# SenseTime-FVG/OpenDWM

Hardware: AMD Instinct MI355X
Metric: denoise-steps/sec (6-view x16f 448x256), SD-3.5 CTSD (higher is better)
Workload: dtype bf16; 1 GPU; CTSD SD-3.5 MMDiT (24 joint blocks, 13 dual, 6 cross-view + 12 temporal VT blocks, point-wise temporal + ImageAdapter), 6 views x 16 frames x 448x256 px (latents [1,16,6,16,32,56]), CFG g=4 -> model batch 2, 154 text tokens, FlowMatch-Euler; one replica per GPU; layers=24, finite=True, residual_stream=fp32 (GEMM operands and activations bf16), variant=text+layout (ImageAdapter recomputed every step, pointwise temporal)

## Files before the change

include/dwm_hip.h:

```cpp
#ifndef DWM_HIP_H
#define DWM_HIP_H

#include <stdint.h>

#ifdef __cplusplus
extern "C" {
#endif

#define DWM_OK 0
#define DWM_EINVAL (-1)
#define DWM_EALIGN (-2)
#define DWM_EUNSUPPORTED (-3)

#define DWM_ABI_VERSION 18
int dwm_abi_version(void);
const char* dwm_source_hash(void);

enum {
    DWM_EPI_PLAIN = 0,
    DWM_EPI_GEGLU = 1,
    DWM_EPI_RESID = 2,
    DWM_EPI_RMSHEAD = 3
};
enum { DWM_ACT_NONE = 0, DWM_ACT_GELU_TANH = 1, DWM_ACT_SILU = 2, DWM_ACT_RELU = 3 };

typedef struct dwm_rowmap2d {
    int64_t rw, rh;
    int64_t rpitch, ipitch;
    int64_t origin;
    int64_t xstep;
} dwm_rowmap2d;

typedef struct dwm_gemm_args {
    const void* A;  int64_t lda;
    const void* W;
    const void* bias;
    void* C;        int64_t ldc;
    int64_t M, N, K;
    int32_t epilogue;
    int32_t act;
    const void* gate; int64_t ld_gate; int64_t rows_per_gate;
    const void* res;  int64_t ld_res;  int64_t res_mod;
    const void* blend; int64_t ld_blend;
    const float* alpha; int64_t rows_per_alpha;
    const void* rms_w; int64_t rms_ncols; float rms_eps;
    int32_t reserved;
    dwm_rowmap2d a_map;
    dwm_rowmap2d c_map;
    int32_t ntaps; int32_t k_per_tap;
    int64_t tap_shift[27];
    void* workspace; int64_t workspace_bytes; int32_t split_k;
    void* C32; int64_t ldc32;
    int32_t tile;
} dwm_gemm_args;

int dwm_gemm_bf16(const dwm_gemm_args* args, void* stream);
int64_t dwm_gemm4w_launches(void);
int64_t dwm_gemm4w_launches_general(void);

typedef struct dwm_gemm_tn_args {
    const void* A; int64_t lda;
    const void* B; int64_t ldb; int64_t b_rows;
    void* out; int64_t ldo;
    int64_t M, N, C;
    int32_t ntaps; int32_t split_k;
    int64_t tap_shift[27];
    void* workspace; int64_t workspace_bytes;
} dwm_gemm_tn_args;
int dwm_gemm_tn(const dwm_gemm_tn_args* args, void* stream);

typedef struct dwm_attn_args {
    const void *q0, *k0, *v0; int64_t ld0;
    const void *q1, *k1, *v1; int64_t ld1;
    void* o0; int64_t ldo0;
    void* o1; int64_t ldo1;
    int64_t L0, L1;
    int64_t n_problems;
    int32_t heads; int32_t head_dim;
    float scale;
    int32_t mask_mode;
    int64_t pdiv[3], pmod[3], pstride[3];
    int64_t ldiv[2], lstride[3];
    const uint8_t* mask; int64_t mask_G; int64_t group_size; int64_t p_per_mask;
    int32_t variant;
    int32_t cross;
    float* lse;
} dwm_attn_args;

int dwm_attention_fwd(const dwm_attn_args* args, void* stream);
int64_t dwm_attn_stream_launches(void);

typedef struct dwm_attn_bwd_args {
    dwm_attn_args fwd;
    const void *do0, *do1;
    void *dq0, *dk0, *dv0; int64_t ld_d0;
    void *dq1, *dk1, *dv1; int64_t ld_d1;
    float* delta;
} dwm_attn_bwd_args;
int dwm_attention_bwd(const dwm_attn_bwd_args* args, void* stream);

int dwm_debug_tr_probe(const int32_t* offs, int16_t* out, void* stream);

typedef struct dwm_layernorm_args {
    const void* x; int64_t ldx;
    void* y;       int64_t ldy;
    void* y2;      int64_t ldy2;
    void* xsum;    int64_t ldxsum;
    int64_t rows; int32_t D; float eps;
    const void* weight; const void* bias;
    const void* scale;  const void* shift;  int64_t ld_mod;  int64_t rows_per_mod;
    const void* scale2; const void* shift2;
    const void* addvec; int64_t ld_add; int64_t rows_per_add;
} dwm_layernorm_args;

int dwm_layernorm(const dwm_layernorm_args* args, void* stream);
int dwm_layernorm_x32(const dwm_layernorm_args* args, void* stream);

int dwm_rmsnorm_heads(void* x, int64_t ldx, int64_t rows, int64_t ncols,
                      const void* w, float eps, void* stream);

int dwm_silu(const void* x, void* y, int64_t n, void* stream);

int dwm_timestep_sinusoid(const float* t, int64_t n, int32_t C, void* out, void* stream);

int dwm_patchify(const void* x, int32_t x_is_f32, int64_t I, int32_t C, int32_t H, int32_t W,
                 int32_t p, void* out, int64_t ldo, void* stream);

int dwm_unpatchify(const void* x, int64_t ldx, int64_t I, int32_t C, int32_t h, int32_t w,
                   int32_t p, void* out, void* stream);

int dwm_cfg_euler_step(const void* pred, float* latents, void* model_in, int64_t n,
                       float guidance, float dsigma, void* stream);

int dwm_cfg_euler_step_grouped(const void* pred, float* latents, void* model_in, int64_t n, float guidance,
                               const float* dsigma, int64_t group_elems, void* stream);

int dwm_unshuffle_tokens(const void* x, int32_t x_is_f32, int64_t I, int32_t C, int32_t H, int32_t W,
                         int32_t r, void* out, int64_t ldo, void* stream);

int dwm_avgpool2_tokens(const void* x, int64_t I, int32_t h, int32_t w, int32_t C, void* out, void* stream);

int dwm_add_inplace(void* y, const void* x, int64_t n, void* stream);
int dwm_add_f32_inplace(void* y, const float* x, int64_t n, void* stream);
int dwm_add_f32_f32_inplace(float* y, const float* x, int64_t n, void* stream);

int dwm_groupnorm_silu(const void* x, void* y, int64_t I, int64_t P, int32_t C, int32_t G, float eps,
                       const void* gamma, const void* beta, int32_t silu, float* stats,
                       const dwm_rowmap2d* out_map, void* stream);

typedef struct dwm_gn_imgmap { int64_t iv, pn, s_ihi, s_ilo, s_phi; } dwm_gn_imgmap;
int64_t dwm_groupnorm_stats_floats(int64_t I, int64_t P, int32_t G);
int dwm_groupnorm_silu_mapped(const void* x, void* y, int64_t I, int64_t P, int32_t C, int32_t G, float eps,
                              const void* gamma, const void* beta, int32_t silu, float* stats,
                              const dwm_rowmap2d* out_map, const dwm_gn_imgmap* img_map, void* stream);

typedef struct dwm_gn_zmap {
    const void* mod; int64_t ld_mod;
    int32_t frames, videos, h, w, shift;
    int32_t zt[32];
} dwm_gn_zmap;
int dwm_groupnorm_spatial(const void* x, void* y, int64_t I, int64_t P, int32_t C, int32_t G, float eps,
                          const void* gamma, const void* beta, int32_t silu, float* stats,
                          const dwm_rowmap2d* out_map, const dwm_gn_imgmap* img_map, const dwm_gn_zmap* zmap, void* stream);
int dwm_groupnorm_spatial_f32(const float* x, float* y, int64_t I, int64_t P, int32_t C, int32_t G, float eps,
                              const float* gamma, const float* beta, int32_t silu, float* stats,
                              const dwm_rowmap2d* out_map, const dwm_gn_imgmap* img_map, const dwm_gn_zmap* zmap, void* stream);

typedef struct dwm_frame_mix { int32_t n_out; int32_t f0[64], f1[64]; float w0[64], w1[64]; } dwm_frame_mix;
int dwm_frame_mix_bf16(const void* x, void* y, int64_t frame_elems, const dwm_frame_mix* mix, void* stream);
int dwm_frame_mix_f32(const float* x, float* y, int64_t frame_elems, const dwm_frame_mix* mix, void* stream);

int dwm_upsample2_padded(const void* x, void* y, int64_t I, int32_t h, int32_t w, int32_t C, void* stream);

int dwm_pad_tokens(const void* x, void* y, int64_t rows, int32_t C, const dwm_rowmap2d* map, void* stream);

int dwm_softmax_rows(const void* x, void* y, int64_t rows, int32_t L, int64_t ld, float scale, void* stream);

typedef struct dwm_vae_attn_args {
    const void* q; const void* k; const void* v; void* out;
    int64_t ldq, ldk, ldv, ldo;
    int64_t I, P;
    int32_t C; float scale;
} dwm_vae_attn_args;
int dwm_vae_attention(const dwm_vae_attn_args* args, void* stream);
int dwm_vae_attention_f32(const dwm_vae_attn_args* args, void* stream);

int dwm_ray_features(const float* cam, int64_t I, int32_t h, int32_t w, void* out, int64_t ldo, void* stream);
int dwm_ray_features_f32(const float* cam, int64_t I, int32_t h, int32_t w, float* out, int64_t ldo, void* stream);

int dwm_frame_affine(const float* x, const float* y, const float* coef, float* out, void* out_bf16, int64_t n,
                     int64_t group_elems, void* stream);

int dwm_cfg_ddim_step(const void* pred, int32_t pred_is_f32, int32_t cfg, float* latents, void* model_in, float* x0_out,
                      const float* noise, const float* coef, int64_t n, int64_t group_elems, float guidance,
                      int32_t prediction_type, float clip_range, int32_t use_clipped_model_output, void* stream);

int dwm_cfg_ddim_step_masked(const void* pred, int32_t pred_is_f32, int32_t cfg, float* latents, void* model_in, float* x0_out,
                             const float* noise, const float* coef, int64_t n, int64_t group_elems, float guidance,
                             int32_t prediction_type, float clip_range, int32_t use_clipped_model_output, const int32_t* skip,
                             void* stream);

int dwm_cfg_multistep(const void* pred, float* latents, float* x0_prev, void* model_in, int64_t n, float guidance,
                      float kx, float ko, float A, float B, float C, void* stream);

int dwm_cfg_multistep_grouped(const void* pred, float* latents, float* x0_prev, void* model_in, int64_t n, float guidance,
                              const float* coef, int64_t coef_rows, const int32_t* keep_model_in, int64_t group_elems, void* stream);
int dwm_cfg_multistep_grouped_f32(const float* pred, float* latents, float* x0_prev, float* model_in, int64_t n, float guidance,
                                  const float* coef, int64_t coef_rows, const int32_t* keep_model_in, int64_t group_elems,
                                  void* stream);

int dwm_cast_f32_to_bf16(const float* src, void* dst, int64_t n, void* stream);

int dwm_transpose_bf16(const void* in, int64_t ld_in, int64_t rows, int64_t cols,
                       void* out, int64_t ld_out, int64_t rows_pad, void* stream);

int dwm_segsum(const void* a, int64_t lda, const void* b, int64_t ldb, int64_t rows, int64_t ncols,
               int64_t rows_per_group, float* out, int64_t ld_out, void* stream);
int dwm_segsum_diff(const void* a, int64_t lda, const void* b, int64_t ldb, const void* b2, int64_t ldb2, int64_t rows,
                    int64_t ncols, int64_t rows_per_group, float* out, int64_t ld_out, void* stream);

int dwm_act_fwd(const void* x, void* y, int64_t n, int32_t act, void* stream);
int dwm_act_bwd(const void* x, const void* dy, void* dx, int64_t n, int32_t act, void* stream);
int dwm_act_bwd_recompute(const void* x, const void* dy, void* y_out, void* dx, int64_t n, int32_t act, void* stream);

int dwm_geglu_fwd(const void* u, int64_t ldu, int64_t rows, int64_t inner, void* g, int64_t ldg, void* stream);
int dwm_geglu_bwd(const void* u, int64_t ldu, const void* dg, int64_t lddg, int64_t rows, int64_t inner,
                  void* du, int64_t lddu, void* stream);
int dwm_geglu_bwd_recompute(const void* u, int64_t ldu, const void* dg, int64_t lddg, int64_t rows, int64_t inner,
                            void* g_out, int64_t ldg, void* du, int64_t lddu, void* stream);

typedef struct dwm_rowcombine_args {
    const void* a; int64_t lda;
    const void* gate_a; int64_t ld_gate_a; int64_t rows_per_gate_a;
    const float* coef_a; int64_t rows_per_coef_a;
    const void* b; int64_t ldb;
    const float* coef_b; int64_t rows_per_coef_b;
    void* out; int64_t ldo;
    int64_t rows; int64_t ncols;
} dwm_rowcombine_args;
int dwm_rowcombine(const dwm_rowcombine_args* args, void* stream);

typedef struct dwm_layernorm_bwd_args {
    const void* x; int64_t ldx;
    const void* addvec; int64_t ld_add; int64_t rows_per_add;
    const void* dy; int64_t lddy;
    const void* dy2; int64_t lddy2;
    void* dx; int64_t lddx; int32_t accumulate;
    int64_t rows; int32_t D; float eps;
    const void* weight;
    const void* scale; const void* scale2; int64_t ld_mod; int64_t rows_per_mod;
    float* dgamma; float* dbeta; float* dgamma2; float* dbeta2; int64_t ld_grad; int32_t grad_per_group;
} dwm_layernorm_bwd_args;
int dwm_layernorm_bwd(const dwm_layernorm_bwd_args* args, void* stream);

int dwm_rmsnorm_heads_train(void* x, int64_t ldx, int64_t rows, int64_t ncols, const void* w, float eps,
                            float* rinv, void* stream);
int dwm_rmsnorm_heads_bwd(const void* y, int64_t ldy, const float* rinv, const void* w, void* dy, int64_t lddy,
                          int64_t rows, int64_t ncols, float* dw, void* stream);

int dwm_adamw(float* p, const float* g, float* m, float* v, void* p_bf16, int64_t n, float lr, float beta1,
              float beta2, float eps, float weight_decay, float bias_corr1, float bias_corr2, float grad_scale,
              void* stream);

typedef struct dwm_adamw_item {
    float* p; const float* g; float* m; float* v; void* p_bf16; int64_t n;
} dwm_adamw_item;
int dwm_adamw_multi(const dwm_adamw_item* items, const int32_t* block_item, const int64_t* block_start, int64_t n_blocks,
                    int64_t chunk, float lr, float beta1, float beta2, float eps, float weight_decay, float bias_corr1,
                    float bias_corr2, float grad_scale, void* stream);

int dwm_quantize_blockwise8(const float* x, int64_t n, const float* code, int32_t floor_positive, uint8_t* q, float* absmax,
                            void* stream);
int dwm_dequantize_blockwise8(const uint8_t* q, const float* absmax, int64_t n, const float* code, float* x, void* stream);

typedef struct dwm_adamw8_item {
    float* p; const float* g; uint8_t* m_q; float* m_absmax; uint8_t* v_q; float* v_absmax; void* p_bf16; int64_t n;
} dwm_adamw8_item;
int dwm_adamw8_multi(const dwm_adamw8_item* items, const int32_t* block_item, const int64_t* block_start, int64_t n_blocks,
                     int64_t chunk, const float* code_m, const float* code_v, float lr, float beta1, float beta2, float eps,
                     float weight_decay, float bias_corr1, float bias_corr2, float grad_scale, void* stream);

typedef struct dwm_grad_item { float* g; int64_t n; } dwm_grad_item;
int dwm_grad_sumsq_multi(const dwm_grad_item* items, const int32_t* block_item, const int64_t* block_start, int64_t n_blocks,
                         int64_t chunk, float pre_scale, float max_norm, double* partials, uint32_t* flags, float* out,
                         void* stream);
int dwm_grad_scale_multi(const dwm_grad_item* items, const int32_t* block_item, const int64_t* block_start, int64_t n_blocks,
                         int64_t chunk, float coef, void* stream);

int dwm_groupnorm_bwd(const void* x, const void* dz, void* dx, int64_t I, int64_t P, int32_t C, int32_t G, float eps,
                      const void* gamma, const void* beta, int32_t silu, int32_t accumulate, float* stats,
                      float* dgamma, float* dbeta, const dwm_rowmap2d* dz_map, const dwm_gn_imgmap* img_map, void* stream);

int64_t dwm_segsum_ordered_floats(int64_t rows, int64_t ncols, int64_t rows_per_group);
int64_t dwm_segsum_diff_ordered_floats(int64_t rows, int64_t ncols, int64_t rows_per_group);
int64_t dwm_layernorm_bwd_ordered_floats(const dwm_layernorm_bwd_args* args);
int64_t dwm_rmsnorm_heads_bwd_ordered_floats(int64_t rows, int64_t ncols);
int64_t dwm_groupnorm_bwd_ordered_floats(int64_t I, int64_t P, int32_t C);
int dwm_segsum_ordered(const void* a, int64_t lda, const void* b, int64_t ldb, int64_t rows, int64_t ncols,
                       int64_t rows_per_group, float* out, int64_t ld_out, float* workspace, int64_t workspace_floats, void* stream);
int dwm_segsum_diff_ordered(const void* a, int64_t lda, const void* b, int64_t ldb, const void* b2, int64_t ldb2, int64_t rows,
                            int64_t ncols, int64_t rows_per_group, float* out, int64_t ld_out, float* workspace,
                            int64_t workspace_floats, void* stream);
int dwm_layernorm_bwd_ordered(const dwm_layernorm_bwd_args* args, float* workspace, int64_t workspace_floats, void* stream);
int dwm_rmsnorm_heads_bwd_ordered(const void* y, int64_t ldy, const float* rinv, const void* w, void* dy, int64_t lddy,
                                  int64_t rows, int64_t ncols, float* dw, float* workspace, int64_t workspace_floats, void* stream);
int dwm_groupnorm_bwd_ordered(const void* x, const void* dz, void* dx, int64_t I, int64_t P, int32_t C, int32_t G, float eps,
                              const void* gamma, const void* beta, int32_t silu, int32_t accumulate, float* stats,
                              float* dgamma, float* dbeta, const dwm_rowmap2d* dz_map, const dwm_gn_imgmap* img_map,
                              float* workspace, int64_t workspace_floats, void* stream);

typedef struct dwm_block_permute_args {
    const void* src;
    void* dst;
    int64_t block_bytes;
    int64_t n[4];
    int64_t sstride[4];
} dwm_block_permute_args;
int dwm_block_permute(const dwm_block_permute_args* args, void* stream);

int dwm_head_exchange(const void* src, void* dst, int64_t rows, int32_t S, int32_t R, int64_t Dr, int32_t elem_size, int64_t ld,
                      int32_t dir, void* stream);

typedef struct dwm_fifo_item {
    void* buf; const void* fresh; int64_t outer; int64_t T; int64_t inner_bytes; int64_t fresh_outer; int64_t convert; int64_t n;
} dwm_fifo_item;
int dwm_fifo_slide_multi(const dwm_fifo_item* host_items, int64_t n_items, const dwm_fifo_item* items, const int32_t* block_item,
                         const int64_t* block_start, int64_t n_blocks, int64_t chunk, void* stream);

int dwm_cast_bf16_to_f32(const void* x, int64_t ldx, float* y, int64_t ldy, int64_t rows, int64_t cols,
                         int32_t accumulate, void* stream);

int dwm_gemm_f32(const dwm_gemm_args* args, void* stream);
int dwm_groupnorm_silu_f32(const float* x, float* y, int64_t I, int64_t P, int32_t C, int32_t G, float eps,
                           const float* gamma, const float* beta, int32_t silu, float* stats,
                           const dwm_rowmap2d* out_map, const dwm_gn_imgmap* img_map, void* stream);
int dwm_upsample2_padded_f32(const float* x, float* y, int64_t I, int32_t h, int32_t w, int32_t C, void* stream);
int dwm_pad_tokens_f32(const float* x, float* y, int64_t rows, int32_t C, const dwm_rowmap2d* map, void* stream);
int dwm_softmax_rows_f32(const float* x, float* y, int64_t rows, int32_t L, int64_t ld, float scale, void* stream);
int dwm_unshuffle_tokens_f32(const float* x, int64_t I, int32_t C, int32_t H, int32_t W, int32_t r, float* out, int64_t ldo,
                             void* stream);
int dwm_avgpool2_tokens_f32(const float* x, int64_t I, int32_t h, int32_t w, int32_t C, float* out, void* stream);
int dwm_cfg_multistep_f32(const float* pred, float* latents, float* x0_prev, float* model_in, int64_t n, float guidance,
                          float kx, float ko, float A, float B, float C, void* stream);
int dwm_layernorm_f32(const dwm_layernorm_args* args, void* stream);
int dwm_attention_f32(const dwm_attn_args* args, void* stream);
int dwm_silu_f32(const float* x, float* y, int64_t n, void* stream);
int dwm_timestep_sinusoid_f32(const float* t, int64_t n, int32_t C, float* out, void* stream);
int dwm_patchify_f32(const float* x, int64_t I, int32_t C, int32_t H, int32_t W, int32_t p, float* out, int64_t ldo, void* stream);
int dwm_unpatchify_f32(const float* x, int64_t ldx, int64_t I, int32_t C, int32_t h, int32_t w, int32_t p, float* out, void* stream);
int dwm_cfg_euler_step_f32(const float* pred, float* latents, float* model_in, int64_t n, float guidance, float dsigma,
                           const float* dsigma_group, int64_t group_elems, void* stream);

typedef struct dwm_text_attn_args {
    const void* q; const void* k; const void* v; int64_t ld;
    void* out; int64_t ldo;
    int64_t n_seq, L;
// ... 18 lines not shown
```

opendwm_amd/_lib.py:

```python
from __future__ import annotations

import ctypes as C
import os

HERE = os.path.dirname(os.path.abspath(__file__))
LIB_PATH = os.environ.get("DWM_HIP_LIB") or os.path.join(HERE, "libdwm_hip.so")
ABI_VERSION = 18

EPI_PLAIN, EPI_GEGLU, EPI_RESID, EPI_RMSHEAD = 0, 1, 2, 3
ACT_NONE, ACT_GELU_TANH, ACT_SILU, ACT_RELU = 0, 1, 2, 3

_i64, _i32, _f32, _vp = C.c_int64, C.c_int32, C.c_float, C.c_void_p


class RowMap2D(C.Structure):
    _fields_ = [("rw", _i64), ("rh", _i64), ("rpitch", _i64), ("ipitch", _i64), ("origin", _i64), ("xstep", _i64)]


class GemmTnArgs(C.Structure):
    _fields_ = [
        ("A", _vp), ("lda", _i64), ("B", _vp), ("ldb", _i64), ("b_rows", _i64), ("out", _vp), ("ldo", _i64),
        ("M", _i64), ("N", _i64), ("C", _i64), ("ntaps", _i32), ("split_k", _i32), ("tap_shift", _i64 * 27),
        ("workspace", _vp), ("workspace_bytes", _i64),
    ]


class GemmArgs(C.Structure):
    _fields_ = [
        ("A", _vp), ("lda", _i64), ("W", _vp), ("bias", _vp), ("C", _vp), ("ldc", _i64),
        ("M", _i64), ("N", _i64), ("K", _i64), ("epilogue", _i32), ("act", _i32),
        ("gate", _vp), ("ld_gate", _i64), ("rows_per_gate", _i64),
        ("res", _vp), ("ld_res", _i64), ("res_mod", _i64),
        ("blend", _vp), ("ld_blend", _i64), ("alpha", _vp), ("rows_per_alpha", _i64),
        ("rms_w", _vp), ("rms_ncols", _i64), ("rms_eps", _f32), ("reserved", _i32),
        ("a_map", RowMap2D), ("c_map", RowMap2D), ("ntaps", _i32), ("k_per_tap", _i32),
        ("tap_shift", _i64 * 27),
        ("workspace", _vp), ("workspace_bytes", _i64), ("split_k", _i32),
        ("C32", _vp), ("ldc32", _i64),
        ("tile", _i32),
    ]


class AttnArgs(C.Structure):
    _fields_ = [
        ("q0", _vp), ("k0", _vp), ("v0", _vp), ("ld0", _i64),
        ("q1", _vp), ("k1", _vp), ("v1", _vp), ("ld1", _i64),
        ("o0", _vp), ("ldo0", _i64), ("o1", _vp), ("ldo1", _i64),
        ("L0", _i64), ("L1", _i64), ("n_problems", _i64),
        ("heads", _i32), ("head_dim", _i32), ("scale", _f32), ("mask_mode", _i32),
        ("pdiv", _i64 * 3), ("pmod", _i64 * 3), ("pstride", _i64 * 3),
        ("ldiv", _i64 * 2), ("lstride", _i64 * 3),
        ("mask", _vp), ("mask_G", _i64), ("group_size", _i64), ("p_per_mask", _i64),
        ("variant", _i32), ("cross", _i32), ("lse", _vp),
    ]


class AttnBwdArgs(C.Structure):
    _fields_ = [
        ("fwd", AttnArgs), ("do0", _vp), ("do1", _vp),
        ("dq0", _vp), ("dk0", _vp), ("dv0", _vp), ("ld_d0", _i64),
        ("dq1", _vp), ("dk1", _vp), ("dv1", _vp), ("ld_d1", _i64), ("delta", _vp),
    ]


class LayerNormArgs(C.Structure):
    _fields_ = [
        ("x", _vp), ("ldx", _i64), ("y", _vp), ("ldy", _i64), ("y2", _vp), ("ldy2", _i64),
        ("xsum", _vp), ("ldxsum", _i64), ("rows", _i64), ("D", _i32), ("eps", _f32),
        ("weight", _vp), ("bias", _vp),
        ("scale", _vp), ("shift", _vp), ("ld_mod", _i64), ("rows_per_mod", _i64),
        ("scale2", _vp), ("shift2", _vp),
        ("addvec", _vp), ("ld_add", _i64), ("rows_per_add", _i64),
    ]


class GnImgMap(C.Structure):
    _fields_ = [("iv", _i64), ("pn", _i64), ("s_ihi", _i64), ("s_ilo", _i64), ("s_phi", _i64)]


class GnZMap(C.Structure):
    _fields_ = [("mod", _vp), ("ld_mod", _i64), ("frames", _i32), ("videos", _i32), ("h", _i32), ("w", _i32),
                ("shift", _i32), ("zt", _i32 * 32)]


class FrameMix(C.Structure):
    _fields_ = [("n_out", _i32), ("f0", _i32 * 64), ("f1", _i32 * 64), ("w0", _f32 * 64), ("w1", _f32 * 64)]


class BlockPermuteArgs(C.Structure):
    _fields_ = [("src", C.c_void_p), ("dst", C.c_void_p), ("block_bytes", C.c_int64), ("n", C.c_int64 * 4), ("sstride", C.c_int64 * 4)]


class RowCombineArgs(C.Structure):
    _fields_ = [
        ("a", _vp), ("lda", _i64), ("gate_a", _vp), ("ld_gate_a", _i64), ("rows_per_gate_a", _i64),
        ("coef_a", _vp), ("rows_per_coef_a", _i64), ("b", _vp), ("ldb", _i64),
        ("coef_b", _vp), ("rows_per_coef_b", _i64), ("out", _vp), ("ldo", _i64), ("rows", _i64), ("ncols", _i64),
    ]


class LayerNormBwdArgs(C.Structure):
    _fields_ = [
        ("x", _vp), ("ldx", _i64), ("addvec", _vp), ("ld_add", _i64), ("rows_per_add", _i64),
        ("dy", _vp), ("lddy", _i64), ("dy2", _vp), ("lddy2", _i64),
        ("dx", _vp), ("lddx", _i64), ("accumulate", _i32),
        ("rows", _i64), ("D", _i32), ("eps", _f32), ("weight", _vp),
        ("scale", _vp), ("scale2", _vp), ("ld_mod", _i64), ("rows_per_mod", _i64),
        ("dgamma", _vp), ("dbeta", _vp), ("dgamma2", _vp), ("dbeta2", _vp), ("ld_grad", _i64), ("grad_per_group", _i32),
    ]


class AdamW8Item(C.Structure):
    _fields_ = [("p", _vp), ("g", _vp), ("m_q", _vp), ("m_absmax", _vp), ("v_q", _vp), ("v_absmax", _vp), ("p_bf16", _vp), ("n", _i64)]


class FifoItem(C.Structure):
    _fields_ = [("buf", _vp), ("fresh", _vp), ("outer", _i64), ("T", _i64), ("inner_bytes", _i64), ("fresh_outer", _i64),
                ("convert", _i64), ("n", _i64)]


class VaeAttnArgs(C.Structure):
    _fields_ = [("q", _vp), ("k", _vp), ("v", _vp), ("out", _vp), ("ldq", _i64), ("ldk", _i64), ("ldv", _i64), ("ldo", _i64),
                ("I", _i64), ("P", _i64), ("C", _i32), ("scale", _f32)]


class TextAttnArgs(C.Structure):
    _fields_ = [("q", _vp), ("k", _vp), ("v", _vp), ("ld", _i64), ("out", _vp), ("ldo", _i64), ("n_seq", _i64), ("L", _i64),
                ("heads", _i32), ("scale", _f32), ("causal", _i32), ("bias", _vp)]


SIGNATURES = {
    "dwm_abi_version": (_i32, []),
    "dwm_source_hash": (C.c_char_p, []),
    "dwm_gemm_bf16": (_i32, [C.POINTER(GemmArgs), _vp]),
    "dwm_gemm4w_launches": (_i64, []),
    "dwm_gemm4w_launches_general": (_i64, []),
    "dwm_attn_stream_launches": (_i64, []),
    "dwm_gemm_tn": (_i32, [C.POINTER(GemmTnArgs), _vp]),
    "dwm_attention_fwd": (_i32, [C.POINTER(AttnArgs), _vp]),
    "dwm_attention_bwd": (_i32, [C.POINTER(AttnBwdArgs), _vp]),
    "dwm_debug_tr_probe": (_i32, [_vp, _vp, _vp]),
    "dwm_layernorm": (_i32, [C.POINTER(LayerNormArgs), _vp]),
    "dwm_layernorm_x32": (_i32, [C.POINTER(LayerNormArgs), _vp]),
    "dwm_rmsnorm_heads": (_i32, [_vp, _i64, _i64, _i64, _vp, _f32, _vp]),
    "dwm_silu": (_i32, [_vp, _vp, _i64, _vp]),
    "dwm_timestep_sinusoid": (_i32, [_vp, _i64, _i32, _vp, _vp]),
    "dwm_patchify": (_i32, [_vp, _i32, _i64, _i32, _i32, _i32, _i32, _vp, _i64, _vp]),
    "dwm_unpatchify": (_i32, [_vp, _i64, _i64, _i32, _i32, _i32, _i32, _vp, _vp]),
    "dwm_cfg_euler_step": (_i32, [_vp, _vp, _vp, _i64, _f32, _f32, _vp]),
    "dwm_cfg_euler_step_grouped": (_i32, [_vp, _vp, _vp, _i64, _f32, _vp, _i64, _vp]),
    "dwm_cast_f32_to_bf16": (_i32, [_vp, _vp, _i64, _vp]),
    "dwm_gemm_f32": (_i32, [C.POINTER(GemmArgs), _vp]),
    "dwm_layernorm_f32": (_i32, [C.POINTER(LayerNormArgs), _vp]),
    "dwm_groupnorm_silu_f32": (_i32, [_vp, _vp, _i64, _i64, _i32, _i32, _f32, _vp, _vp, _i32, _vp, C.POINTER(RowMap2D), C.POINTER(GnImgMap), _vp]),
    "dwm_upsample2_padded_f32": (_i32, [_vp, _vp, _i64, _i32, _i32, _i32, _vp]),
    "dwm_pad_tokens_f32": (_i32, [_vp, _vp, _i64, _i32, C.POINTER(RowMap2D), _vp]),
    "dwm_softmax_rows_f32": (_i32, [_vp, _vp, _i64, _i32, _i64, _f32, _vp]),
    "dwm_unshuffle_tokens_f32": (_i32, [_vp, _i64, _i32, _i32, _i32, _i32, _vp, _i64, _vp]),
    "dwm_avgpool2_tokens_f32": (_i32, [_vp, _i64, _i32, _i32, _i32, _vp, _vp]),
    "dwm_cfg_multistep_f32": (_i32, [_vp, _vp, _vp, _vp, _i64, _f32, _f32, _f32, _f32, _f32, _f32, _vp]),
    "dwm_attention_f32": (_i32, [C.POINTER(AttnArgs), _vp]),
    "dwm_silu_f32": (_i32, [_vp, _vp, _i64, _vp]),
    "dwm_timestep_sinusoid_f32": (_i32, [_vp, _i64, _i32, _vp, _vp]),
    "dwm_patchify_f32": (_i32, [_vp, _i64, _i32, _i32, _i32, _i32, _vp, _i64, _vp]),
    "dwm_unpatchify_f32": (_i32, [_vp, _i64, _i64, _i32, _i32, _i32, _i32, _vp, _vp]),
    "dwm_cfg_euler_step_f32": (_i32, [_vp, _vp, _vp, _i64, _f32, _f32, _vp, _i64, _vp]),
    "dwm_ray_features": (_i32, [_vp, _i64, _i32, _i32, _vp, _i64, _vp]),
    "dwm_ray_features_f32": (_i32, [_vp, _i64, _i32, _i32, _vp, _i64, _vp]),
    "dwm_frame_affine": (_i32, [_vp, _vp, _vp, _vp, _vp, _i64, _i64, _vp]),
    "dwm_cfg_ddim_step": (_i32, [_vp, _i32, _i32, _vp, _vp, _vp, _vp, _vp, _i64, _i64, _f32, _i32, _f32, _i32, _vp]),
    "dwm_cfg_multistep": (_i32, [_vp, _vp, _vp, _vp, _i64, _f32, _f32, _f32, _f32, _f32, _f32, _vp]),
    "dwm_cfg_ddim_step_masked": (_i32, [_vp, _i32, _i32, _vp, _vp, _vp, _vp, _vp, _i64, _i64, _f32, _i32, _f32, _i32, _vp, _vp]),
    "dwm_cfg_multistep_grouped": (_i32, [_vp, _vp, _vp, _vp, _i64, _f32, _vp, _i64, _vp, _i64, _vp]),
    "dwm_cfg_multistep_grouped_f32": (_i32, [_vp, _vp, _vp, _vp, _i64, _f32, _vp, _i64, _vp, _i64, _vp]),
    "dwm_unshuffle_tokens": (_i32, [_vp, _i32, _i64, _i32, _i32, _i32, _i32, _vp, _i64, _vp]),
    "dwm_avgpool2_tokens": (_i32, [_vp, _i64, _i32, _i32, _i32, _vp, _vp]),
    "dwm_add_inplace": (_i32, [_vp, _vp, _i64, _vp]),
    "dwm_add_f32_inplace": (_i32, [_vp, _vp, _i64, _vp]),
    "dwm_add_f32_f32_inplace": (_i32, [_vp, _vp, _i64, _vp]),
    "dwm_groupnorm_silu": (_i32, [_vp, _vp, _i64, _i64, _i32, _i32, _f32, _vp, _vp, _i32, _vp, C.POINTER(RowMap2D), _vp]),
    "dwm_groupnorm_silu_mapped": (_i32, [_vp, _vp, _i64, _i64, _i32, _i32, _f32, _vp, _vp, _i32, _vp, C.POINTER(RowMap2D), C.POINTER(GnImgMap), _vp]),
    "dwm_upsample2_padded": (_i32, [_vp, _vp, _i64, _i32, _i32, _i32, _vp]),
    "dwm_pad_tokens": (_i32, [_vp, _vp, _i64, _i32, C.POINTER(RowMap2D), _vp]),
    "dwm_groupnorm_stats_floats": (_i64, [_i64, _i64, _i32]),
    "dwm_groupnorm_spatial": (_i32, [_vp, _vp, _i64, _i64, _i32, _i32, _f32, _vp, _vp, _i32, _vp, C.POINTER(RowMap2D),
                                     C.POINTER(GnImgMap), C.POINTER(GnZMap), _vp]),
    "dwm_frame_mix_bf16": (_i32, [_vp, _vp, _i64, C.POINTER(FrameMix), _vp]),
    "dwm_frame_mix_f32": (_i32, [_vp, _vp, _i64, C.POINTER(FrameMix), _vp]),
    "dwm_groupnorm_spatial_f32": (_i32, [_vp, _vp, _i64, _i64, _i32, _i32, _f32, _vp, _vp, _i32, _vp, C.POINTER(RowMap2D),
                                         C.POINTER(GnImgMap), C.POINTER(GnZMap), _vp]),
    "dwm_softmax_rows": (_i32, [_vp, _vp, _i64, _i32, _i64, _f32, _vp]),
    "dwm_vae_attention": (_i32, [C.POINTER(VaeAttnArgs), _vp]),
    "dwm_vae_attention_f32": (_i32, [C.POINTER(VaeAttnArgs), _vp]),
    "dwm_transpose_bf16": (_i32, [_vp, _i64, _i64, _i64, _vp, _i64, _i64, _vp]),
    "dwm_segsum": (_i32, [_vp, _i64, _vp, _i64, _i64, _i64, _i64, _vp, _i64, _vp]),
    "dwm_segsum_diff": (_i32, [_vp, _i64, _vp, _i64, _vp, _i64, _i64, _i64, _i64, _vp, _i64, _vp]),
    "dwm_act_fwd": (_i32, [_vp, _vp, _i64, _i32, _vp]),
    "dwm_act_bwd": (_i32, [_vp, _vp, _vp, _i64, _i32, _vp]),
    "dwm_geglu_fwd": (_i32, [_vp, _i64, _i64, _i64, _vp, _i64, _vp]),
    "dwm_geglu_bwd": (_i32, [_vp, _i64, _vp, _i64, _i64, _i64, _vp, _i64, _vp]),
    "dwm_act_bwd_recompute": (_i32, [_vp, _vp, _vp, _vp, _i64, _i32, _vp]),
    "dwm_geglu_bwd_recompute": (_i32, [_vp, _i64, _vp, _i64, _i64, _i64, _vp, _i64, _vp, _i64, _vp]),
    "dwm_rowcombine": (_i32, [C.POINTER(RowCombineArgs), _vp]),
    "dwm_layernorm_bwd": (_i32, [C.POINTER(LayerNormBwdArgs), _vp]),
    "dwm_rmsnorm_heads_train": (_i32, [_vp, _i64, _i64, _i64, _vp, _f32, _vp, _vp]),
    "dwm_rmsnorm_heads_bwd": (_i32, [_vp, _i64, _vp, _vp, _vp, _i64, _i64, _i64, _vp, _vp]),
    "dwm_adamw": (_i32, [_vp, _vp, _vp, _vp, _vp, _i64, _f32, _f32, _f32, _f32, _f32, _f32, _f32, _f32, _vp]),
    "dwm_adamw_multi": (_i32, [_vp, _vp, _vp, _i64, _i64, _f32, _f32, _f32, _f32, _f32, _f32, _f32, _f32, _vp]),
    "dwm_quantize_blockwise8": (_i32, [_vp, _i64, _vp, _i32, _vp, _vp, _vp]),
    "dwm_dequantize_blockwise8": (_i32, [_vp, _vp, _i64, _vp, _vp, _vp]),
    "dwm_adamw8_multi": (_i32, [_vp, _vp, _vp, _i64, _i64, _vp, _vp, _f32, _f32, _f32, _f32, _f32, _f32, _f32, _f32, _vp]),
    "dwm_grad_sumsq_multi": (_i32, [_vp, _vp, _vp, _i64, _i64, _f32, _f32, _vp, _vp, _vp, _vp]),
    "dwm_grad_scale_multi": (_i32, [_vp, _vp, _vp, _i64, _i64, _f32, _vp]),
    "dwm_block_permute": (_i32, [C.POINTER(BlockPermuteArgs), _vp]),
    "dwm_head_exchange": (_i32, [_vp, _vp, _i64, _i32, _i32, _i64, _i32, _i64, _i32, _vp]),
    "dwm_fifo_slide_multi": (_i32, [C.POINTER(FifoItem), _i64, _vp, _vp, _vp, _i64, _i64, _vp]),
    "dwm_cast_bf16_to_f32": (_i32, [_vp, _i64, _vp, _i64, _i64, _i64, _i32, _vp]),
    "dwm_groupnorm_bwd": (_i32, [_vp, _vp, _vp, _i64, _i64, _i32, _i32, _f32, _vp, _vp, _i32, _i32, _vp, _vp, _vp,
                                 C.POINTER(RowMap2D), C.POINTER(GnImgMap), _vp]),
    "dwm_segsum_ordered": (_i32, [_vp, _i64, _vp, _i64, _i64, _i64, _i64, _vp, _i64, _vp, _i64, _vp]),
    "dwm_segsum_diff_ordered": (_i32, [_vp, _i64, _vp, _i64, _vp, _i64, _i64, _i64, _i64, _vp, _i64, _vp, _i64, _vp]),
    "dwm_layernorm_bwd_ordered": (_i32, [C.POINTER(LayerNormBwdArgs), _vp, _i64, _vp]),
    "dwm_rmsnorm_heads_bwd_ordered": (_i32, [_vp, _i64, _vp, _vp, _vp, _i64, _i64, _i64, _vp, _vp, _i64, _vp]),
    "dwm_groupnorm_bwd_ordered": (_i32, [_vp, _vp, _vp, _i64, _i64, _i32, _i32, _f32, _vp, _vp, _i32, _i32, _vp, _vp, _vp,
                                         C.POINTER(RowMap2D), C.POINTER(GnImgMap), _vp, _i64, _vp]),
    "dwm_segsum_ordered_floats": (_i64, [_i64, _i64, _i64]),
    "dwm_segsum_diff_ordered_floats": (_i64, [_i64, _i64, _i64]),
    "dwm_layernorm_bwd_ordered_floats": (_i64, [C.POINTER(LayerNormBwdArgs)]),
    "dwm_rmsnorm_heads_bwd_ordered_floats": (_i64, [_i64, _i64]),
    "dwm_groupnorm_bwd_ordered_floats": (_i64, [_i64, _i64, _i32]),
    "dwm_text_attention": (_i32, [C.POINTER(TextAttnArgs), _vp]),
    "dwm_rmsnorm_rows": (_i32, [_vp, _i64, _i64, _i64, _vp, _f32, _vp, _i64, _vp]),
    "dwm_text_embed": (_i32, [_vp, _i64, _vp, _i64, _i64, _vp, _i64, _vp, _i64, _vp]),
    "dwm_text_act": (_i32, [_vp, _i64, _i64, _i64, _i32, _i32, _vp, _i64, _vp]),
}

_ERR = {-1: "DWM_EINVAL (bad shape / null pointer)", -2: "DWM_EALIGN (alignment)",
        -3: "DWM_EUNSUPPORTED (shape not supported by the kernel)"}

_lib = None


def load():
    global _lib
    if _lib is not None:
        return _lib
    import torch
    if torch.cuda.is_available():
        torch.cuda.init()
    if not os.path.exists(LIB_PATH):
        raise RuntimeError(
            f"{LIB_PATH} is missing: build it with `python -m opendwm_amd.build` "
            "(there is no CPU / PyTorch fallback for the HIP path)")
    lib = C.CDLL(LIB_PATH)
    for name, (res, args) in SIGNATURES.items():
        fn = getattr(lib, name)
        fn.restype = res
        fn.argtypes = args
    v = lib.dwm_abi_version()
    if v != ABI_VERSION:
        raise RuntimeError(f"libdwm_hip.so ABI {v} != binding ABI {ABI_VERSION}; rebuild")
    if os.environ.get("DWM_SKIP_SOURCE_HASH") != "1":
        from .build import source_hash
        try:
            want = source_hash()
        except OSError:
            want = None
        have = (lib.dwm_source_hash() or b"").decode()
        if want is not None and have != want:
            msg = (f"{LIB_PATH} was built from other sources (hash {have[:12]}..., tree {want[:12]}...): "
                   "run `python -m opendwm_amd.build`")
            if os.environ.get("DWM_HIP_LIB"):
                import warnings
                warnings.warn(msg)
            else:
                raise RuntimeError(msg)
    _lib = lib
    return lib


def check(rc: int, what: str) -> None:
    if rc != 0:
        msg = _ERR.get(rc, f"hipError_t {rc}" if rc > 0 else f"error {rc}")
        raise RuntimeError(f"{what} failed: {msg}")
```

opendwm_amd/blocks.py:

```python
from __future__ import annotations

from typing import Optional

import torch
from torch import nn

from . import ops
from .ops import ACT_GELU_TANH, ACT_SILU, EPI_GEGLU, EPI_RESID, EPI_RMSHEAD

bf16 = torch.bfloat16


class ParamStore:

    def __init__(self):
        self.step = 0
        self._shadow = {}
        self._derived = {}
        self.precision = bf16

    def set_precision(self, dtype: torch.dtype) -> None:
        if dtype not in (bf16, torch.float32):
            raise ValueError("compute dtype must be torch.bfloat16 or torch.float32")
        self.precision = dtype

    def cached(self, owner, make):
        slot = getattr(owner, "_pk", None)
        if not isinstance(slot, dict) or "_by_precision" not in slot:
            slot = {"_by_precision": {}}
            owner._pk = slot
        hit = slot["_by_precision"].get(self.precision)
        if hit is None or hit[0] != self.step:
            hit = (self.step, make())
            slot["_by_precision"][self.precision] = hit
        return hit[1]

    def bf(self, t: torch.Tensor) -> torch.Tensor:
        if self.precision == torch.float32:
            d = t.detach()
            if d.dtype == torch.float32:
                return d if d.is_contiguous() else d.contiguous()
            key = (t.data_ptr(), t._version, tuple(t.shape), "f32")
            hit = self._shadow.get(id(t))
            if hit is None or hit[0] != key:
                hit = (key, d.float().contiguous())
                self._shadow[id(t)] = hit
            return hit[1]
        if t.dtype == bf16:
            d = t.detach()
            return d if d.is_contiguous() else d.contiguous()
        key = (t.data_ptr(), t._version, tuple(t.shape))
        hit = self._shadow.get(id(t))
        if hit is None or hit[0] != key:
            d = t.detach()
            if d.is_cuda and d.dtype == torch.float32 and d.is_contiguous() and d.numel() % 4 == 0:
                sh = ops.cast_bf16(d)
            else:
                sh = d.to(bf16).contiguous()
            hit = (key, sh)
            self._shadow[id(t)] = hit
        return hit[1]

    def derived(self, t: torch.Tensor, tag: str, make):
        k = (id(t), tag, self.precision)
        hit = self._derived.get(k)
        if hit is None or hit[0] != (self.step, t.data_ptr(), t._version):
            hit = ((self.step, t.data_ptr(), t._version), make())
            self._derived[k] = hit
        return hit[1]

    def bump(self, keep_shadows: bool = False) -> None:
        self.step += 1
        self._derived.clear()
        ops.clear_split_weights()
        if not keep_shadows:
            self._shadow.clear()


STORE = ParamStore()
PRESCALE_Q = True
ATTN_VARIANT = 0


def _bf(t: Optional[torch.Tensor]) -> Optional[torch.Tensor]:
    return None if t is None else STORE.bf(t)


def stream32(h: torch.Tensor) -> bool:
    return h.dtype == torch.float32 and STORE.precision == bf16


def _act_like(h: torch.Tensor) -> torch.Tensor:
    return torch.empty(h.shape, dtype=bf16 if stream32(h) else h.dtype, device=h.device)


def _resid_into(stream: torch.Tensor, a: torch.Tensor, w: torch.Tensor, b: Optional[torch.Tensor], **kw) -> torch.Tensor:
    if stream32(stream):
        return ops.gemm(a, w, b, epilogue=EPI_RESID, res=stream, out32=stream, mirror=False, **kw)
    return ops.gemm(a, w, b, epilogue=EPI_RESID, res=stream, out=stream, **kw)


def geglu_pack(w: torch.Tensor) -> torch.Tensor:
    n2 = w.shape[0] // 2
    if n2 % 32 != 0:
        raise RuntimeError("GEGLU inner dim must be a multiple of 32")
    tail = w.shape[1:]
    v = w[:n2].reshape(n2 // 32, 32, *tail)
    g = w[n2:].reshape(n2 // 32, 32, *tail)
    return torch.stack([v, g], dim=1).reshape(w.shape).contiguous()


class RMSNorm(nn.Module):

    def __init__(self, dim: int, eps: float):
        super().__init__()
        self.eps = eps
        self.weight = nn.Parameter(torch.ones(dim))


class _ActProj(nn.Module):

    def __init__(self, dim_in: int, dim_out: int):
        super().__init__()
        self.proj = nn.Linear(dim_in, dim_out)


class FeedForward(nn.Module):

    def __init__(self, dim: int, dim_out: Optional[int] = None, activation_fn: str = "geglu"):
        super().__init__()
        inner = dim * 4
        self.activation_fn = activation_fn
        proj_out = inner * 2 if activation_fn == "geglu" else inner
        self.net = nn.ModuleList([_ActProj(dim, proj_out), nn.Identity(), nn.Linear(inner, dim_out or dim)])


class TimestepEmbedding(nn.Module):

    def __init__(self, in_channels: int, time_embed_dim: int, out_dim: Optional[int] = None):
        super().__init__()
        self.linear_1 = nn.Linear(in_channels, time_embed_dim)
        self.linear_2 = nn.Linear(time_embed_dim, out_dim or time_embed_dim)

    def run(self, x: torch.Tensor, res: Optional[torch.Tensor] = None) -> torch.Tensor:
        h = ops.gemm(x, _bf(self.linear_1.weight), _bf(self.linear_1.bias), act=ACT_SILU)
        if res is None:
            return ops.gemm(h, _bf(self.linear_2.weight), _bf(self.linear_2.bias))
        return ops.gemm(h, _bf(self.linear_2.weight), _bf(self.linear_2.bias), epilogue=EPI_RESID, res=res)


class CombinedTimestepTextProjEmbeddings(nn.Module):

    def __init__(self, embedding_dim: int, pooled_projection_dim: int):
        super().__init__()
        self.timestep_embedder = TimestepEmbedding(256, embedding_dim)
        self.text_embedder = TimestepEmbedding(pooled_projection_dim, embedding_dim)

    def run(self, timestep: torch.Tensor, pooled: torch.Tensor) -> torch.Tensor:
        t_emb = self.timestep_embedder.run(ops.timestep_sinusoid(timestep, 256, dtype=STORE.precision))
        return self.text_embedder.run(pooled, res=t_emb)


class _AdaNorm(nn.Module):

    def __init__(self, dim: int, chunks: int):
        super().__init__()
        self.linear = nn.Linear(dim, chunks * dim)


class Attention(nn.Module):

    def __init__(self, dim: int, heads: int, dim_head: int, bias: bool, out_bias: bool = True,
                 added_kv: bool = False, context_pre_only: Optional[bool] = None,
                 qk_norm: Optional[str] = None, eps: float = 1e-5):
        super().__init__()
        self.heads, self.dim_head, self.eps = heads, dim_head, eps
        inner = heads * dim_head
        self.to_q = nn.Linear(dim, inner, bias=bias)
        self.to_k = nn.Linear(dim, inner, bias=bias)
        self.to_v = nn.Linear(dim, inner, bias=bias)
        self.to_out = nn.ModuleList([nn.Linear(inner, dim, bias=out_bias), nn.Identity()])
        self.has_qk_norm = qk_norm == "rms_norm"
        if self.has_qk_norm:
            self.norm_q = RMSNorm(dim_head, eps)
            self.norm_k = RMSNorm(dim_head, eps)
        self.added_kv = added_kv
        if added_kv:
            self.add_q_proj = nn.Linear(dim, inner, bias=True)
            self.add_k_proj = nn.Linear(dim, inner, bias=True)
            self.add_v_proj = nn.Linear(dim, inner, bias=True)
            if not context_pre_only:
                self.to_add_out = nn.Linear(inner, dim, bias=True)
            if self.has_qk_norm:
                self.norm_added_q = RMSNorm(dim_head, eps)
                self.norm_added_k = RMSNorm(dim_head, eps)
        self._pk = None
        self._pk_step = -1

    def packed(self) -> dict:
        def make():
            def fuse(q, k, v):
                w = torch.cat([_bf(q.weight), _bf(k.weight), _bf(v.weight)], 0).contiguous()
                b = None if q.bias is None else torch.cat([_bf(q.bias), _bf(k.bias), _bf(v.bias)]).contiguous()
                return w, b
            pk = {}
            pk["wqkv"], pk["bqkv"] = fuse(self.to_q, self.to_k, self.to_v)
            def rms_cols(nq, nk, fold):
                wq = _bf(nq.weight)
                if fold:
                    wq = (nq.weight.detach().float() * (self.dim_head ** -0.5 * 1.4426950408889634)).to(wq.dtype)
                return torch.cat([wq.repeat(self.heads), _bf(nk.weight).repeat(self.heads)]).contiguous()
            if self.has_qk_norm:
                pk["rms"] = rms_cols(self.norm_q, self.norm_k, False)
                pk["rms_ps"] = rms_cols(self.norm_q, self.norm_k, True)
            if self.added_kv:
                pk["wadd"], pk["badd"] = fuse(self.add_q_proj, self.add_k_proj, self.add_v_proj)
                if self.has_qk_norm:
                    pk["rms_add"] = rms_cols(self.norm_added_q, self.norm_added_k, False)
                    pk["rms_add_ps"] = rms_cols(self.norm_added_q, self.norm_added_k, True)
            return pk
        return STORE.cached(self, make)

    @property
    def attn_variant(self) -> int:
        return ops.ATTN_Q_PRESCALED if (self.has_qk_norm and PRESCALE_Q) else 0

    def project_qkv(self, x: torch.Tensor, added: bool = False, out: Optional[torch.Tensor] = None) -> torch.Tensor:
        pk = self.packed()
        ps = "_ps" if self.attn_variant else ""
        w, b, rms = (pk["wadd"], pk["badd"], pk.get("rms_add" + ps)) if added else (pk["wqkv"], pk["bqkv"], pk.get("rms" + ps))
        if rms is None:
            return ops.gemm(x, w, b, out=out)
        if self.dim_head != 64:
            raise RuntimeError("qk RMSNorm is implemented for head_dim 64 only")
        return ops.gemm(x, w, b, epilogue=EPI_RMSHEAD, rms_w=rms, rms_ncols=rms.numel(), rms_eps=self.eps, out=out)


class JointTransformerBlock(nn.Module):

    def __init__(self, dim: int, num_attention_heads: int, attention_head_dim: int,
                 context_pre_only: bool = False, qk_norm: Optional[str] = None,
                 use_dual_attention: bool = False):
        super().__init__()
        self.dim, self.heads = dim, num_attention_heads
        self.context_pre_only = context_pre_only
        self.use_dual_attention = use_dual_attention
        self.norm1 = _AdaNorm(dim, 9 if use_dual_attention else 6)
        self.norm1_context = _AdaNorm(dim, 2 if context_pre_only else 6)
        self.attn = Attention(dim, num_attention_heads, attention_head_dim, bias=True, added_kv=True,
                              context_pre_only=context_pre_only, qk_norm=qk_norm, eps=1e-6)
        if use_dual_attention:
            self.attn2 = Attention(dim, num_attention_heads, attention_head_dim, bias=True,
                                   qk_norm=qk_norm, eps=1e-6)
        self.ff = FeedForward(dim, dim, activation_fn="gelu-approximate")
        if not context_pre_only:
            self.ff_context = FeedForward(dim, dim, activation_fn="gelu-approximate")

    def run(self, h: torch.Tensor, c: torch.Tensor, silu_temb: torch.Tensor, n_img: int, mod=None, cmod=None):
        D = self.dim
        N, Lc = h.shape[0] // n_img, c.shape[0] // n_img
        x32 = stream32(h)
        if mod is None:
            mod = ops.gemm(silu_temb, _bf(self.norm1.linear.weight), _bf(self.norm1.linear.bias))
        if cmod is None:
            cmod = ops.gemm(silu_temb, _bf(self.norm1_context.linear.weight), _bf(self.norm1_context.linear.bias))
        sl = lambda m, i: m[:, i * D:(i + 1) * D]
        nh2 = _act_like(h) if self.use_dual_attention else None
        nh = ops.layernorm(h, eps=1e-6, scale=sl(mod, 1), shift=sl(mod, 0), rows_per_mod=N,
                           scale2=sl(mod, 7) if nh2 is not None else None,
                           shift2=sl(mod, 6) if nh2 is not None else None, out2=nh2, x32=x32)
        if self.context_pre_only:
            nc = ops.layernorm(c, eps=1e-6, scale=sl(cmod, 0), shift=sl(cmod, 1), rows_per_mod=Lc, x32=x32)
        else:
            nc = ops.layernorm(c, eps=1e-6, scale=sl(cmod, 1), shift=sl(cmod, 0), rows_per_mod=Lc, x32=x32)

        rows_h, rows_c = nh.shape[0], nc.shape[0]
        both = torch.empty(rows_h + rows_c, 3 * D, dtype=nh.dtype, device=nh.device)
        qkv = self.attn.project_qkv(nh, out=both[:rows_h])
        cqkv = self.attn.project_qkv(nc, added=True, out=both[rows_h:])
        ao_both = torch.empty(rows_h + rows_c, D, dtype=nh.dtype, device=nh.device)
        ao, cao = ao_both[:rows_h], ao_both[rows_h:]
        ops.attention(qkv[:, :D], qkv[:, D:2 * D], qkv[:, 2 * D:], ao, ops.rowmap_identity(n_img, N), self.heads,
                      q1=cqkv[:, :D], k1=cqkv[:, D:2 * D], v1=cqkv[:, 2 * D:], out1=cao, variant=self.attn.attn_variant | ATTN_VARIANT)
        to_out = self.attn.to_out[0]
        _resid_into(h, ao, _bf(to_out.weight), _bf(to_out.bias), gate=sl(mod, 2), rows_per_gate=N)
        if self.use_dual_attention:
            qkv2 = self.attn2.project_qkv(nh2)
            ops.attention(qkv2[:, :D], qkv2[:, D:2 * D], qkv2[:, 2 * D:], ao, ops.rowmap_identity(n_img, N), self.heads,
                          variant=self.attn2.attn_variant | ATTN_VARIANT)
            to_out2 = self.attn2.to_out[0]
            _resid_into(h, ao, _bf(to_out2.weight), _bf(to_out2.bias), gate=sl(mod, 8), rows_per_gate=N)
        nh = ops.layernorm(h, eps=1e-6, scale=sl(mod, 4), shift=sl(mod, 3), rows_per_mod=N, out=nh, x32=x32)
        f1, f2 = self.ff.net[0].proj, self.ff.net[2]
        ffh = ops.gemm(nh, _bf(f1.weight), _bf(f1.bias), act=ACT_GELU_TANH)
        _resid_into(h, ffh, _bf(f2.weight), _bf(f2.bias), gate=sl(mod, 5), rows_per_gate=N)

        if self.context_pre_only:
            return None, h
        ta = self.attn.to_add_out
        _resid_into(c, cao, _bf(ta.weight), _bf(ta.bias), gate=sl(cmod, 2), rows_per_gate=Lc)
        nc = ops.layernorm(c, eps=1e-6, scale=sl(cmod, 4), shift=sl(cmod, 3), rows_per_mod=Lc, out=nc, x32=x32)
        c1, c2 = self.ff_context.net[0].proj, self.ff_context.net[2]
        cff = ops.gemm(nc, _bf(c1.weight), _bf(c1.bias), act=ACT_GELU_TANH)
        _resid_into(c, cff, _bf(c2.weight), _bf(c2.bias), gate=sl(cmod, 5), rows_per_gate=Lc)
        return c, h


class AlphaBlender(nn.Module):

    strategies = ["fixed", "learned", "learned_with_images"]

    def __init__(self, alpha: float, merge_strategy: str = "learned_with_images"):
        super().__init__()
        if merge_strategy not in AlphaBlender.strategies:
            raise ValueError("merge_strategy needs to be in {}".format(AlphaBlender.strategies))
        self.merge_strategy = merge_strategy
        if merge_strategy == "fixed":
            self.register_buffer("mix_factor", torch.tensor([float(alpha)]))
        else:
            self.register_parameter("mix_factor", nn.Parameter(torch.tensor([float(alpha)])))

    def get_alpha(self, image_only_indicator: Optional[torch.Tensor], batch: int) -> torch.Tensor:
        mfp, ind = self.mix_factor, image_only_indicator
        if mfp.is_cuda and torch.cuda.is_current_stream_capturing():
            return self._alpha(ind, batch)
        key = (mfp.data_ptr(), mfp._version, STORE.step, batch, None if ind is None else ind._version)
        c = getattr(self, "_alpha_cache", None)
        if c is not None and c[0] == key and c[1] is ind:
            return c[2]
        a = self._alpha(ind, batch)
        self._alpha_cache = (key, ind, a)
        return a

    def _alpha(self, image_only_indicator: Optional[torch.Tensor], batch: int) -> torch.Tensor:
        mf = self.mix_factor.detach().float()
        if self.merge_strategy == "fixed":
            return mf.expand(batch).contiguous()
        if self.merge_strategy == "learned":
            return torch.sigmoid(mf).expand(batch).contiguous()
        if image_only_indicator is None:
            raise ValueError("Please provide image_only_indicator to use learned_with_images merge strategy")
        flag = image_only_indicator.reshape(batch).to(device=mf.device, dtype=torch.bool)
        return torch.where(flag, torch.ones((), device=mf.device), torch.sigmoid(mf)).contiguous()


class VTSelfAttentionBlock(nn.Module):

    def __init__(self, dim: int, time_mix_inner_dim: int, num_attention_heads: int,
                 attention_head_dim: int, qk_norm=None):
        super().__init__()
        if dim != time_mix_inner_dim:
            raise NotImplementedError("VTSelfAttentionBlock: dim != time_mix_inner_dim is never used by the reference")
        self.dim, self.heads = dim, num_attention_heads
        self.is_res = True
        self.norm_in = nn.LayerNorm(dim)
        self.ff_in = FeedForward(dim, dim_out=time_mix_inner_dim, activation_fn="geglu")
        self.norm1 = nn.LayerNorm(time_mix_inner_dim)
        self.attn1 = Attention(time_mix_inner_dim, num_attention_heads, attention_head_dim, bias=False,
                               qk_norm=qk_norm, eps=1e-5)
        self.norm3 = nn.LayerNorm(time_mix_inner_dim)
        self.ff = FeedForward(time_mix_inner_dim, activation_fn="geglu")
        self._pk = None
        self._pk_step = -1

    def packed(self) -> dict:
        def make():
            pk = {}
            for name, ff in (("ff_in", self.ff_in), ("ff", self.ff)):
                pk[name + "_w"] = geglu_pack(_bf(ff.net[0].proj.weight))
                pk[name + "_b"] = geglu_pack(_bf(ff.net[0].proj.bias))
            return pk
        return STORE.cached(self, make)

    def run(self, h: torch.Tensor, rowmap: ops.RowMap, *, emb: Optional[torch.Tensor] = None,
            rows_per_emb: int = 1, group_mask: Optional[torch.Tensor] = None,
            dense_mask: Optional[torch.Tensor] = None,
            blend_alpha: Optional[torch.Tensor] = None, rows_per_alpha: int = 1,
            blend_into: Optional[torch.Tensor] = None, head_exchange=None) -> torch.Tensor:
        D = self.dim
        pk = self.packed()
        x32 = stream32(h)
        ln = lambda x, n, **kw: ops.layernorm(x, eps=1e-5, weight=_bf(n.weight), bias=_bf(n.bias), x32=stream32(x), **kw)
        if emb is not None:
            xs = torch.empty_like(h)
            y = ln(h, self.norm_in, addvec=emb, rows_per_add=rows_per_emb, xsum=xs)
        else:
            xs = h.clone()
            y = ln(h, self.norm_in)
        g = ops.gemm(y, pk["ff_in_w"], pk["ff_in_b"], epilogue=EPI_GEGLU)
        l2 = self.ff_in.net[2]
        _resid_into(xs, g, _bf(l2.weight), _bf(l2.bias))

        y = ln(xs, self.norm1, out=y)
        qkv = self.attn1.project_qkv(y)
        ao = y
        if head_exchange is None:
            ops.attention(qkv[:, :D], qkv[:, D:2 * D], qkv[:, 2 * D:], ao, rowmap, self.heads,
                          group_mask=group_mask, dense_mask=dense_mask, variant=self.attn1.attn_variant | ATTN_VARIANT)
        else:
            fs, rows = head_exchange, qkv.shape[0]
            if group_mask is not None or dense_mask is not None or self.heads % fs.size:
                raise RuntimeError("VTSelfAttentionBlock.run: the head exchange takes no mask and needs heads % ranks == 0")
            Dr = D // fs.size
            rx = fs.heads_gather(qkv, rows, 3)
            ox = torch.empty(fs.size * rows, Dr, dtype=rx.dtype, device=rx.device)
            ops.attention(rx[:, :Dr], rx[:, Dr:2 * Dr], rx[:, 2 * Dr:], ox, rowmap, self.heads // fs.size,
                          variant=self.attn1.attn_variant | ATTN_VARIANT)
            fs.heads_scatter(ox, rows, out=ao)
        to_out = self.attn1.to_out[0]
        _resid_into(xs, ao, _bf(to_out.weight), _bf(to_out.bias))

        y = ln(xs, self.norm3, out=y)
        g = ops.gemm(y, pk["ff_w"], pk["ff_b"], epilogue=EPI_GEGLU, out=g)
        l2 = self.ff.net[2]
        if blend_alpha is None:
            return _resid_into(xs, g, _bf(l2.weight), _bf(l2.bias))
        if x32:
            if not stream32(blend_into):
                raise RuntimeError("VTSelfAttentionBlock.run: an fp32 stream blends into an fp32 stream")
            ops.gemm(g, _bf(l2.weight), _bf(l2.bias), epilogue=EPI_RESID, res=xs, blend=blend_into,
                     alpha=blend_alpha, rows_per_alpha=rows_per_alpha, out32=blend_into, mirror=False)
            return blend_into
        ops.gemm(g, _bf(l2.weight), _bf(l2.bias), epilogue=EPI_RESID, res=xs, blend=blend_into,
                 alpha=blend_alpha, rows_per_alpha=rows_per_alpha, out=blend_into)
        return blend_into

    def forward(self, hidden_states: torch.Tensor, self_attention_mask: Optional[torch.Tensor] = None):
        with torch.no_grad():
            bp, L, c = hidden_states.shape
            h = ops.cast_bf16(hidden_states.reshape(bp * L, c).contiguous()) \
                if hidden_states.dtype != bf16 else hidden_states.reshape(bp * L, c).contiguous()
            out = self.run(h, ops.rowmap_identity(bp, L), dense_mask=self_attention_mask)
            return out.view(bp, L, c)
```

opendwm_amd/build.py:

```python
from __future__ import annotations

import os
import shutil
import subprocess
import sys
from concurrent.futures import ThreadPoolExecutor

HERE = os.path.dirname(os.path.abspath(__file__))
CSRC = os.path.join(HERE, "csrc")
INCLUDE = os.path.join(os.path.dirname(HERE), "include")
LIB = os.path.join(HERE, "libdwm_hip.so")
SOURCES = ["gemm_bf16.hip", "gemm_bf16_4w.hip", "gemm_tn.hip", "attention.hip", "attention_stream.hip", "attention_bwd.hip", "norm.hip",
           "elementwise.hip", "vae.hip", "vae_attention.hip", "train.hip", "fp32path.hip", "gradnorm.hip", "fifo.hip", "text.hip"]
AGPR_SOURCES: set = {"gemm_bf16_4w.hip", "attention_stream.hip"}
FILE_FLAGS: dict = {"attention_stream.hip": ["-fno-slp-vectorize"]}
VGPR_FORM = ["-mllvm", "-amdgpu-mfma-vgpr-form"]
ARCH = "gfx950"


def _hipcc() -> str:
    for c in (os.environ.get("HIPCC"), "/opt/rocm/bin/hipcc", shutil.which("hipcc")):
        if c and os.path.exists(c):
            return c
    raise RuntimeError("hipcc not found (need ROCm to build libdwm_hip.so)")


def _stale(target: str, deps) -> bool:
    if not os.path.exists(target):
        return True
    t = os.path.getmtime(target)
    return any(os.path.getmtime(d) > t for d in deps)


def source_hash() -> str:
    import hashlib
    h = hashlib.sha256()
    files = sorted(os.path.join(CSRC, f) for f in os.listdir(CSRC) if f.endswith((".hip", ".h"))) + [os.path.join(INCLUDE, "dwm_hip.h")]
    for f in files:
        h.update(os.path.basename(f).encode())
        h.update(open(f, "rb").read())
    return h.hexdigest()


def build(force: bool = False, verbose: bool = False) -> str:
    hipcc = _hipcc()
    headers = [os.path.join(CSRC, "common.h"), os.path.join(CSRC, "attention_common.h"), os.path.join(CSRC, "gemm_common.h"),
               os.path.join(INCLUDE, "dwm_hip.h")]
    shash = source_hash()
    stamp = os.path.join(CSRC, "build", ".source_hash")
    objdir = os.path.join(CSRC, "build")
    os.makedirs(objdir, exist_ok=True)
    base = [f"--offload-arch={ARCH}", "-O3", "-std=c++17", "-fPIC", "-fno-gpu-rdc", f"-I{INCLUDE}", f"-I{CSRC}"]
    user = os.environ.get("DWM_EXTRA_FLAGS", "").split()
    jobs = []
    extra = " ".join(os.environ.get("DWM_EXTRA_FLAGS", "").split())
    old_hash, old_extra = "", ""
    if os.path.exists(stamp):
        lines = open(stamp).read().split("\n")
        old_hash, old_extra = lines[0].strip(), (lines[1].strip() if len(lines) > 1 else "")
    force = force or old_extra != extra
    for src in SOURCES:
        s = os.path.join(CSRC, src)
        o = os.path.join(objdir, src.replace(".hip", ".o"))
        if force or _stale(o, [s] + headers) or (src == "elementwise.hip" and old_hash != shash):
            jobs.append((s, o))

    def compile_one(job):
        s, o = job
        name = os.path.basename(s)
        fl = base + ([] if name in AGPR_SOURCES else VGPR_FORM) + FILE_FLAGS.get(name, []) + user
        if name == "elementwise.hip":
            fl = fl + [f'-DDWM_SOURCE_HASH="{shash}"']
        cmd = [hipcc] + fl + ["-c", s, "-o", o]
        r = subprocess.run(cmd, capture_output=True, text=True)
        if r.returncode != 0:
            raise RuntimeError(f"hipcc failed for {s}:\n{r.stderr}")
        if verbose and r.stderr:
            print(r.stderr, file=sys.stderr)
        return o

    if jobs:
        with ThreadPoolExecutor(max_workers=len(jobs)) as ex:
            list(ex.map(compile_one, jobs))
    objs = [os.path.join(objdir, s.replace(".hip", ".o")) for s in SOURCES]
    if force or jobs or _stale(LIB, objs):
        cmd = [hipcc, f"--offload-arch={ARCH}", "-shared", "-fPIC", "-o", LIB] + objs
        r = subprocess.run(cmd, capture_output=True, text=True)
        if r.returncode != 0:
            raise RuntimeError(f"link failed:\n{r.stderr}")
    with open(stamp, "w") as f:
        f.write(shash + "\n" + extra)
    return LIB


def ensure_built() -> str:
    if os.path.exists(LIB):
        return LIB
    import fcntl
    with open(os.path.join(HERE, ".build.lock"), "w") as lk:
        fcntl.flock(lk, fcntl.LOCK_EX)
        try:
            if not os.path.exists(LIB):
                build()
        finally:
            fcntl.flock(lk, fcntl.LOCK_UN)
    return LIB


if __name__ == "__main__":
    print(build(force="--force" in sys.argv, verbose=True))
```

opendwm_amd/csrc/gemm_bf16.hip:

```cpp
#include <cstdlib>
#include <type_traits>

#include "gemm_common.h"

namespace {

using namespace dwm_gemm;

#ifdef DWM_DEV_HOOKS
#define DWM_RESERVED(x_) (x_)
#define DWM_DEV_LDS_PAD 16384
#else
#define DWM_RESERVED(x_) 0
#define DWM_DEV_LDS_PAD 0
#endif

constexpr int BM = 256, BN = 256, BK = 64;
constexpr int TILE_BYTES = BM * BK * 2;
constexpr int A_STAGES = 3, W_STAGES = 2;
constexpr int W_BASE = A_STAGES * TILE_BYTES;
constexpr int LDS_BYTES = (A_STAGES + W_STAGES) * TILE_BYTES;

template <int TC> struct TileCfg;
template <> struct TileCfg<0> { static constexpr int bm = 256, bn = 256, bk = 64, nwn = 4, nwaves = 8, ast = A_STAGES, wst = W_STAGES; };
// ... 606 lines not shown
    float t[8];
    if (p.bias) {
        unpack8(*(const uint4*)((const bf16_t*)p.bias + n), t);
#pragma unroll
        for (int j = 0; j < 8; ++j) v[j] += t[j];
    }
    if (p.act != DWM_ACT_NONE) {
#pragma unroll
        for (int j = 0; j < 8; j += 2) {
            const f32x2 x = {v[j], v[j + 1]};
            const f32x2 y = p.act == DWM_ACT_GELU_TANH ? gelu_tanh2(x) : p.act == DWM_ACT_SILU ? silu2(x) : relu2(x);
            v[j] = y[0]; v[j + 1] = y[1];
        }
    }
    const int64_t mr = map_row(cp.c, m);
    if (p.epilogue == DWM_EPI_RESID) {
        if (p.gate) {
            unpack8(*(const uint4*)((const bf16_t*)p.gate + (int64_t)fdiv((uint32_t)m, cp.fd_rpg) * p.ld_gate + n), t);
#pragma unroll
            for (int j = 0; j < 8; ++j) v[j] *= t[j];
        }
        if (p.res) {
            const int64_t rr = p.res_mod > 0 ? (int64_t)fmod_u((uint32_t)m, cp.fd_rmod) : p.res_mod < 0 ? (int64_t)fdiv((uint32_t)m, cp.fd_rmod) : mr;
            unpack8(*(const uint4*)((const bf16_t*)p.res + rr * p.ld_res + n), t);
#pragma unroll
            for (int j = 0; j < 8; ++j) v[j] += t[j];
        }
        if (p.blend) {
            unpack8(*(const uint4*)((const bf16_t*)p.blend + mr * p.ld_blend + n), t);
            const float al = p.alpha[fdiv((uint32_t)m, cp.fd_rpa)];
#pragma unroll
            for (int j = 0; j < 8; ++j) v[j] = al * t[j] + (1.f - al) * v[j];
        }
    }
    *(uint4*)((bf16_t*)p.C + mr * p.ldc + n) = pack8(v);
}

__global__ void __launch_bounds__(256)
split_planes_kernel(const float* __restrict__ x, int64_t ldx, int64_t M, int64_t K, bf16_t* __restrict__ planes) {
    const int64_t k8 = K >> 3;
    const int64_t i = (int64_t)blockIdx.x * 256 + threadIdx.x;
    if (i >= M * k8) return;
    const int64_t m = i / k8, k = (i - m * k8) << 3;
    const float4 a = *(const float4*)(x + m * ldx + k), b = *(const float4*)(x + m * ldx + k + 4);
    const float v[8] = {a.x, a.y, a.z, a.w, b.x, b.y, b.z, b.w};
    float hi[8], lo[8];
    const uint4 ph = pack8(v);
    unpack8(ph, hi);
#pragma unroll
    for (int j = 0; j < 8; ++j) lo[j] = v[j] - hi[j];
    *(uint4*)(planes + m * K + k) = ph;
    *(uint4*)(planes + (M + m) * K + k) = pack8(lo);
}

DWM_DEVINL float act_f32(float x, int act) {
    if (act == DWM_ACT_GELU_TANH) return 0.5f * x * (1.f + tanhf(0.7978845608028654f * (x + 0.044715f * x * x * x)));
    if (act == DWM_ACT_SILU) return x / (1.f + expf(-x));
    if (act == DWM_ACT_RELU) return fmaxf(x, 0.f);
    return x;
}

template <int EPI>
__global__ void __launch_bounds__(256)
f32_finish_kernel(const dwm_gemm_args p, const ConvParams cp) {
    constexpr bool kGeglu = EPI == DWM_EPI_GEGLU;
    const int64_t Nout = kGeglu ? (p.N >> 1) : p.N;
    const int64_t n8 = Nout >> 3;
    const int64_t i = (int64_t)blockIdx.x * 256 + threadIdx.x;
    const bool live = i < p.M * n8;
    const int64_t m = live ? i / n8 : 0, n = live ? (i - m * n8) << 3 : 0;
    const int64_t nv = kGeglu ? ((n >> 5) << 6) + (n & 31) : n;
    auto load8 = [&](int64_t col, float* v) {
#pragma unroll
        for (int j = 0; j < 8; ++j) v[j] = 0.f;
        const float* w = cp.ws + m * p.N + col;
        for (int s = 0; s < cp.ksplit; ++s) {
            const float4 a = *(const float4*)(w + s * cp.ws_slice), b = *(const float4*)(w + s * cp.ws_slice + 4);
            v[0] += a.x; v[1] += a.y; v[2] += a.z; v[3] += a.w;
            v[4] += b.x; v[5] += b.y; v[6] += b.z; v[7] += b.w;
        }
        if (p.bias) {
            const float* bp = (const float*)p.bias + col;
#pragma unroll
            for (int j = 0; j < 8; ++j) v[j] += bp[j];
        }
    };
    float v[8];
    load8(nv, v);
    if constexpr (kGeglu) {
        float g[8];
        load8(nv + 32, g);
#pragma unroll
        for (int j = 0; j < 8; ++j) v[j] *= 0.5f * g[j] * (1.f + erff(g[j] * 0.7071067811865476f));
    } else if constexpr (EPI == DWM_EPI_RMSHEAD) {
        float ss = 0.f;
#pragma unroll
        for (int j = 0; j < 8; ++j) ss += v[j] * v[j];
        ss += __shfl_xor(ss, 1, 64);
        ss += __shfl_xor(ss, 2, 64);
        ss += __shfl_xor(ss, 4, 64);
        if (n < p.rms_ncols) {
            const float rinv = 1.f / sqrtf(ss * (1.f / 64.f) + p.rms_eps);
            const float* rw = (const float*)p.rms_w + n;
#pragma unroll
            for (int j = 0; j < 8; ++j) v[j] = v[j] * rinv * rw[j];
        }
    } else {
#pragma unroll
        for (int j = 0; j < 8; ++j) v[j] = act_f32(v[j], p.act);
    }
    if (!live) return;
    const int64_t mr = map_row(cp.c, m);
    if constexpr (EPI == DWM_EPI_RESID) {
        if (p.gate) {
            const float* t = (const float*)p.gate + (int64_t)fdiv((uint32_t)m, cp.fd_rpg) * p.ld_gate + n;
#pragma unroll
            for (int j = 0; j < 8; ++j) v[j] *= t[j];
        }
        if (p.res) {
            const int64_t rr = p.res_mod > 0 ? (int64_t)fmod_u((uint32_t)m, cp.fd_rmod) : p.res_mod < 0 ? (int64_t)fdiv((uint32_t)m, cp.fd_rmod) : mr;
            const float* t = (const float*)p.res + rr * p.ld_res + n;
#pragma unroll
            for (int j = 0; j < 8; ++j) v[j] += t[j];
        }
        if (p.blend) {
            const float* t = (const float*)p.blend + mr * p.ld_blend + n;
            const float al = p.alpha[fdiv((uint32_t)m, cp.fd_rpa)];
#pragma unroll
            for (int j = 0; j < 8; ++j) v[j] = al * t[j] + (1.f - al) * v[j];
        }
    }
    float* o = (float*)p.C + mr * p.ldc + n;
    *(float4*)o = make_float4(v[0], v[1], v[2], v[3]);
    *(float4*)(o + 4) = make_float4(v[4], v[5], v[6], v[7]);
}


struct GemmFlavor {
    int quantum;
    int64_t m_limit;
    int too_many_taps;
    bool fp32;
};
constexpr GemmFlavor kBf16 = {8, 1ll << 31, DWM_EINVAL, false};
constexpr GemmFlavor kFp32 = {4, 1ll << 30, DWM_EUNSUPPORTED, true};

int check_sizes(const dwm_gemm_args& a, const GemmFlavor& fl) {
    if (a.M <= 0 || a.N <= 0 || a.K <= 0 || a.M >= fl.m_limit || a.N >= (1ll << 31)) return DWM_EINVAL;
    if (a.K % BK != 0 || a.N % 8 != 0) return DWM_EUNSUPPORTED;
    return DWM_OK;
}
int check_epilogue(const dwm_gemm_args& a, const GemmFlavor& fl) {
    const int q = fl.quantum, q_stream = a.C32 ? 4 : q;
    switch (a.epilogue) {
        case DWM_EPI_PLAIN: return DWM_OK;
        case DWM_EPI_GEGLU: return a.N % 64 != 0 ? DWM_EUNSUPPORTED : DWM_OK;
        case DWM_EPI_RESID:
            if (a.gate && (a.rows_per_gate <= 0 || a.ld_gate % q != 0 || !dwm_aligned16(a.gate))) return DWM_EINVAL;
            if (a.res && (a.ld_res % q_stream != 0 || !dwm_aligned16(a.res))) return DWM_EALIGN;
            if (a.blend && (a.alpha == nullptr || a.rows_per_alpha <= 0 || a.ld_blend % q_stream != 0 || !dwm_aligned16(a.blend))) return DWM_EINVAL;
            if (a.gate && a.blend) return DWM_EUNSUPPORTED;
            if (!fl.fp32 && a.C32 != nullptr && (a.ldc32 % 4 != 0 || a.ldc32 < a.N || !dwm_aligned16(a.C32) || a.res_mod != 0 || a.split_k > 1))
                return DWM_EINVAL;
            return DWM_OK;
        case DWM_EPI_RMSHEAD: return a.rms_w == nullptr || a.rms_ncols % 64 != 0 || a.N % 64 != 0 ? DWM_EINVAL : DWM_OK;
        default: return DWM_EINVAL;
    }
}
int check_taps(const dwm_gemm_args& a, const GemmFlavor& fl) {
    const int ntaps = gemm_ntaps(a);
    if (ntaps > 27) return fl.too_many_taps;
    const int64_t kpt = gemm_k_per_tap(a);
    return kpt <= 0 || kpt % BK != 0 || kpt * ntaps != a.K ? DWM_EINVAL : DWM_OK;
}
int check_row_divisors(const dwm_gemm_args& a) {
    return a.rows_per_gate > (1ll << 30) || a.res_mod > (1ll << 30) || a.res_mod < -(1ll << 30) || a.rows_per_alpha > (1ll << 30) ? DWM_EINVAL : DWM_OK;
}
bool valid_rowmaps(const dwm_gemm_args& a) {
    DevRowMap d;
    return make_dev_rowmap(a.a_map, d) && make_dev_rowmap(a.c_map, d);
}

int plan_gemm(const dwm_gemm_args& a, int tile_asked, GemmPlan& plan) {
    const int knobs = DWM_RESERVED(a.reserved);
    if ((tile_asked == 3 || tile_asked == 4) && !knobs && a.lda % 64 == 0 && dwm_gemm4w_covers(a, tile_asked == 4, plan)) return DWM_OK;

    if (!valid_rowmaps(a)) return DWM_EINVAL;
    int rc = check_taps(a, kBf16);
    if (rc == DWM_OK) rc = check_row_divisors(a);
    if (rc != DWM_OK) return rc;
    if (a.lda < gemm_k_per_tap(a)) return DWM_EINVAL;
    if (a.tile < 0 || a.tile > 2) return DWM_EINVAL;

    plan = GemmPlan();
    plan.epi = a.epilogue;
    plan.ntm = (int)((a.M + BM - 1) / BM); plan.ntn = (int)((a.N + BN - 1) / BN);
    plan.block = 512; plan.lds = LDS_BYTES;
    plan.gm = (knobs >> 4) & 31;
    if (plan.gm == 0) plan.gm = raster_group_height(a.K);

    const int64_t tiles = (int64_t)plan.ntm * plan.ntn, nk = a.K / BK;
    const bool ws_usable = dwm_aligned16(a.workspace) && !(knobs & 3);
    int ksplit = 1;
    if (a.split_k > 1) {
        if (!((a.epilogue == DWM_EPI_PLAIN || a.epilogue == DWM_EPI_RESID) && a.workspace != nullptr && a.C32 == nullptr && ws_usable))
            return DWM_EUNSUPPORTED;
        ksplit = a.split_k;
    } else if (auto_splitk(a, tiles) && ws_usable) {
        ksplit = (int)(256 / tiles);
    }
    if (ksplit > 1) {
        ksplit = clamp_ksplit(ksplit, nk, 32, a.M * a.N * 4, a.workspace_bytes);
        if (ksplit < 2) {
            if (a.split_k > 1) return DWM_EUNSUPPORTED;
            ksplit = 1;
        }
    }
    plan.ksplit = ksplit;
    if (ksplit > 1) {
        plan.family = GemmFamily::W8_SPLITK;
        plan.epi = EPI_SPLITK;
        plan.grid = (unsigned)(plan.ntm * plan.ntn * ksplit);
        return DWM_OK;
    }

    plan.tc = a.tile == 2 ? 1 : 0;
    if (a.tile == 0 && a.C32 == nullptr) {
        const int64_t c256 = (a.N + 255) / 256 * 256, c128 = (a.N + 127) / 128 * 128;
        if (c128 < c256 && a.K <= 640) plan.tc = 1;
    }
    if (knobs & 0x200) plan.tc = 1;
    if (plan.tc == 1) {
        if (a.C32 != nullptr) return DWM_EUNSUPPORTED;
        plan.ntn = (int)((a.N + TileCfg<1>::bn - 1) / TileCfg<1>::bn);
        plan.block = TileCfg<1>::nwaves * 64;
        plan.lds = tile_lds_bytes<1>() + ((knobs & 0x400) ? DWM_DEV_LDS_PAD : 0);
    }
    plan.grid = (unsigned)(plan.ntm * plan.ntn);

    const int64_t lim = 1ll << 31;
    const int rs16 = (a.gate ? 1 : 0) | (a.res ? 2 : 0) | (a.blend ? 4 : 0) | ((a.res && a.res_mod < 0) ? 16 : 0);
    plan.fast = a.c_map.rw <= 0 && a.ldc < lim && !(knobs & 4);
    if (a.epilogue == DWM_EPI_RESID)
        plan.fast = plan.fast && (a.res_mod == 0 || (rs16 == 18 && a.C32 == nullptr)) && a.act == DWM_ACT_NONE &&
                    (a.gate == nullptr || a.ld_gate < lim) && (a.res == nullptr || a.ld_res < lim) && (a.blend == nullptr || a.ld_blend < lim);
    if (a.C32 != nullptr) {
        plan.family = GemmFamily::W8_C32;
        plan.rf32 = true;
        plan.fast = plan.fast && a.ldc32 < lim;
        const int rs = rs16 | (a.C ? 8 : 0);
        plan.rs = plan.fast && (rs == 2 || rs == 3 || rs == 6) ? rs : 0;
        return DWM_OK;
    }
    plan.family = plan.tc == 1 ? GemmFamily::W8_128 : GemmFamily::W8_256;
    plan.rs = a.epilogue == DWM_EPI_RESID && plan.fast && (rs16 == 2 || rs16 == 3 || rs16 == 6 || rs16 == 18) ? rs16 : 0;
    return DWM_OK;
}

void fill_conv_params(const dwm_gemm_args& a, const GemmPlan& pl, ConvParams& cp) {
    make_dev_rowmap(a.a_map, cp.a);
    make_dev_rowmap(a.c_map, cp.c);
    cp.steps_per_tap = (int)(gemm_k_per_tap(a) / (pl.tc == 1 ? TileCfg<1>::bk : BK));
    cp.fd_steps = make_fastdiv((uint32_t)cp.steps_per_tap);
    cp.fd_rpg = make_fastdiv((uint32_t)(a.rows_per_gate > 0 ? a.rows_per_gate : 1));
    cp.fd_rmod = make_fastdiv((uint32_t)(a.res_mod > 0 ? a.res_mod : a.res_mod < 0 ? -a.res_mod : 1));
    cp.fd_rpa = make_fastdiv((uint32_t)(a.rows_per_alpha > 0 ? a.rows_per_alpha : 1));
    for (int t = 0; t < 27; ++t) cp.tap_shift[t] = t < a.ntaps ? a.tap_shift[t] : 0;
    cp.ksplit = pl.ksplit;
    cp.ws = (float*)a.workspace;
    cp.ws_slice = a.M * a.N;
    cp.gm = pl.gm;
    cp.fd_pergroup = make_fastdiv((uint32_t)(pl.gm * pl.ntn));
    cp.fd_gm = make_fastdiv((uint32_t)pl.gm);
}

template <int EPI, bool FAST, bool RF32, int TC, int RS>
hipError_t allow8w() {
    return dwm_allow_dynamic_lds<gemm_bf16_kernel<EPI, FAST, RF32, TC, RS>>(tile_lds_bytes<TC>() + (TC ? DWM_DEV_LDS_PAD : 0));
}
template <int EPI, bool FAST, bool RF32, int TC, int RS>
void enqueue8w(const dwm_gemm_args& a, const ConvParams& cp, const GemmPlan& pl, hipStream_t s) {
    hipLaunchKernelGGL((gemm_bf16_kernel<EPI, FAST, RF32, TC, RS>), dim3(pl.grid), dim3(pl.block), pl.lds, s, a, cp, pl.ntm, pl.ntn);
}
template <int EPI, bool FAST, bool RF32, int TC, int RS>
int launch8w(const dwm_gemm_args& a, const ConvParams& cp, const GemmPlan& pl, hipStream_t s) {
    const hipError_t e = allow8w<EPI, FAST, RF32, TC, RS>();
    if (e != hipSuccess) return (int)e;
    enqueue8w<EPI, FAST, RF32, TC, RS>(a, cp, pl, s);
    return dwm_launch_status();
}

int launch_splitk(const dwm_gemm_args& a, const ConvParams& cp, const GemmPlan& pl, hipStream_t s) {
    const hipError_t e = allow8w<EPI_SPLITK, false, false, 0, 0>();
    if (e != hipSuccess) return (int)e;
    enqueue8w<EPI_SPLITK, false, false, 0, 0>(a, cp, pl, s);
    const int64_t nthr = a.M * (a.N >> 3);
    hipLaunchKernelGGL(splitk_finish_kernel, dim3((unsigned)((nthr + 255) / 256)), dim3(256), 0, s, a, cp);
    return dwm_launch_status();
}
}

extern "C" int dwm_gemm_f32(const dwm_gemm_args* a, void* stream) {
    if (a == nullptr || a->A == nullptr || a->W == nullptr || a->C == nullptr || a->workspace == nullptr) return DWM_EINVAL;
    int rc = check_sizes(*a, kFp32);
    if (rc != DWM_OK) return rc;
    rc = check_taps(*a, kFp32);
    if (rc != DWM_OK) return rc;
    const int ctaps = gemm_ntaps(*a), ngroups = (ctaps + 8) / 9;
    const int64_t kpt = gemm_k_per_tap(*a);
    int64_t a_rows = a->M;
    if (a->a_map.rw > 0) {
        const int64_t ppi = a->a_map.rw * a->a_map.rh;
        if (a->a_map.rh <= 0 || a->M % ppi != 0) return DWM_EINVAL;
        int64_t reach = 0;
        for (int t = 0; t < a->ntaps; ++t) reach = a->tap_shift[t] > reach ? a->tap_shift[t] : reach;
        a_rows = a->a_map.origin + (a->M / ppi - 1) * a->a_map.ipitch + (a->a_map.rh - 1) * a->a_map.rpitch +
                 (a->a_map.rw - 1) * (a->a_map.xstep > 0 ? a->a_map.xstep : 1) + reach + 1;
        if (a_rows <= 0) return DWM_EINVAL;
    } else if (a->ntaps > 0) return DWM_EUNSUPPORTED;
    if (a->lda % 4 != 0 || a->ldc % 4 != 0 || !dwm_aligned16(a->A) || !dwm_aligned16(a->W) || !dwm_aligned16(a->C) ||
        !dwm_aligned16(a->workspace)) return DWM_EALIGN;
    const int64_t nout = gemm_nout(*a);
    if (a->ldc < nout || a->lda < kpt) return DWM_EINVAL;
    rc = check_epilogue(*a, kFp32);
    if (rc == DWM_OK) rc = check_row_divisors(*a);
    if (rc != DWM_OK) return rc;
    if (!valid_rowmaps(*a)) return DWM_EINVAL;
    GemmPlan pl = GemmPlan();
    pl.family = GemmFamily::W8_SPLITK; pl.epi = EPI_SPLITK;
    pl.ntm = (int)((a->M + BM - 1) / BM); pl.ntn = (int)((a->N + BN - 1) / BN);
    const int64_t plane_bytes = ((2 * a_rows * kpt * 2 + 255) / 256) * 256;
    const int last_taps = ctaps - 9 * (ngroups - 1);
    const int64_t tiles = (int64_t)pl.ntm * pl.ntn, nk = 3 * kpt * last_taps / BK, slice_bytes = a->M * a->N * 4;
    pl.ksplit = 1;
    if (splitk_pays(tiles * ngroups, nk))
        pl.ksplit = clamp_ksplit((int)(256 / (tiles * ngroups)), nk, 32 / ngroups, ngroups * slice_bytes, a->workspace_bytes - plane_bytes);
    if (pl.ksplit < 1) pl.ksplit = 1;
    if (plane_bytes + (int64_t)ngroups * slice_bytes > a->workspace_bytes) return DWM_EINVAL;
    pl.grid = (unsigned)(pl.ntm * pl.ntn * pl.ksplit); pl.block = 512; pl.lds = LDS_BYTES;

    const hipError_t e = allow8w<EPI_SPLITK, false, false, 0, 0>();
    if (e != hipSuccess) return (int)e;
    hipStream_t s = (hipStream_t)stream;
    bf16_t* planes = (bf16_t*)a->workspace;
    {
        const int64_t nthr = a_rows * (kpt >> 3);
        hipLaunchKernelGGL(split_planes_kernel, dim3((unsigned)((nthr + 255) / 256)), dim3(256), 0, s, (const float*)a->A, a->lda, a_rows,
                           kpt, planes);
    }
    dwm_gemm_args g = *a;
    g.A = planes; g.lda = kpt;
    g.reserved = 0;
    float* const ws_base = (float*)((char*)a->workspace + plane_bytes);
    ConvParams cp;
    for (int gi = 0; gi < ngroups; ++gi) {
        const int tg = gi + 1 < ngroups ? 9 : last_taps;
        g.K = 3 * kpt * tg;
        g.W = (const bf16_t*)a->W + (int64_t)a->N * (3 * kpt * 9) * gi;
        pl.gm = raster_group_height(g.K);
        fill_conv_params(*a, pl, cp);
        for (int t = 0; t < 27; ++t) cp.tap_shift[t] = 0;
        for (int t = 0; t < tg; ++t) {
            const int64_t sh = a->ntaps > 0 ? a->tap_shift[9 * gi + t] : 0;
            cp.tap_shift[3 * t] = sh; cp.tap_shift[3 * t + 1] = sh; cp.tap_shift[3 * t + 2] = sh + a_rows;
        }
        cp.ws = ws_base + (int64_t)gi * pl.ksplit * cp.ws_slice;
        enqueue8w<EPI_SPLITK, false, false, 0, 0>(g, cp, pl, s);
    }
    cp.ws = ws_base;
    cp.ksplit = ngroups * pl.ksplit;
    const int64_t nthr = a->M * (nout >> 3);
    const dim3 fg((unsigned)((nthr + 255) / 256));
    switch (a->epilogue) {
        case DWM_EPI_PLAIN: hipLaunchKernelGGL(f32_finish_kernel<DWM_EPI_PLAIN>, fg, dim3(256), 0, s, *a, cp); break;
        case DWM_EPI_GEGLU: hipLaunchKernelGGL(f32_finish_kernel<DWM_EPI_GEGLU>, fg, dim3(256), 0, s, *a, cp); break;
        case DWM_EPI_RESID: hipLaunchKernelGGL(f32_finish_kernel<DWM_EPI_RESID>, fg, dim3(256), 0, s, *a, cp); break;
        default: hipLaunchKernelGGL(f32_finish_kernel<DWM_EPI_RMSHEAD>, fg, dim3(256), 0, s, *a, cp); break;
    }
    return dwm_launch_status();
}

namespace {

int launch_c32(const dwm_gemm_args& a, const ConvParams& cp, const GemmPlan& pl, hipStream_t s) {
    if (!pl.fast) return launch8w<DWM_EPI_RESID, false, true, 0, 0>(a, cp, pl, s);
    switch (pl.rs) {
        case 0: return launch8w<DWM_EPI_RESID, true, true, 0, 0>(a, cp, pl, s);
        case 3: return launch8w<DWM_EPI_RESID, true, true, 0, 3>(a, cp, pl, s);
        case 2: return launch8w<DWM_EPI_RESID, true, true, 0, 2>(a, cp, pl, s);
        default: return launch8w<DWM_EPI_RESID, true, true, 0, 6>(a, cp, pl, s);
    }
}
template <int TC>
int launch_resid_rs(const dwm_gemm_args& a, const ConvParams& cp, const GemmPlan& pl, hipStream_t s) {
    switch (pl.rs) {
        case 2: return launch8w<DWM_EPI_RESID, true, false, TC, 2>(a, cp, pl, s);
        case 3: return launch8w<DWM_EPI_RESID, true, false, TC, 3>(a, cp, pl, s);
        case 6: return launch8w<DWM_EPI_RESID, true, false, TC, 6>(a, cp, pl, s);
        default: return launch8w<DWM_EPI_RESID, true, false, TC, 18>(a, cp, pl, s);
    }
}
template <int EPI>
int launch_epi(const dwm_gemm_args& a, const ConvParams& cp, const GemmPlan& pl, hipStream_t s) {
    if (pl.fast) return pl.tc == 1 ? launch8w<EPI, true, false, 1, 0>(a, cp, pl, s) : launch8w<EPI, true, false, 0, 0>(a, cp, pl, s);
    return pl.tc == 1 ? launch8w<EPI, false, false, 1, 0>(a, cp, pl, s) : launch8w<EPI, false, false, 0, 0>(a, cp, pl, s);
}
int launch_tile(const dwm_gemm_args& a, const ConvParams& cp, const GemmPlan& pl, hipStream_t s) {
    if (pl.rs != 0) return pl.tc == 1 ? launch_resid_rs<1>(a, cp, pl, s) : launch_resid_rs<0>(a, cp, pl, s);
    switch (pl.epi) {
        case DWM_EPI_PLAIN: return launch_epi<DWM_EPI_PLAIN>(a, cp, pl, s);
        case DWM_EPI_GEGLU: return launch_epi<DWM_EPI_GEGLU>(a, cp, pl, s);
        case DWM_EPI_RESID: return launch_epi<DWM_EPI_RESID>(a, cp, pl, s);
        default: return launch_epi<DWM_EPI_RMSHEAD>(a, cp, pl, s);
    }
}

}

extern "C" int dwm_gemm_bf16(const dwm_gemm_args* a_in, void* stream) {
    if (a_in == nullptr) return DWM_EINVAL;
    const int tile_asked = a_in->tile;
    dwm_gemm_args a_copy;
    if (tile_asked == 3 || tile_asked == 4) { a_copy = *a_in; a_copy.tile = 0; }
    const dwm_gemm_args& a = tile_asked == 3 || tile_asked == 4 ? a_copy : *a_in;

    if (a.A == nullptr || a.W == nullptr || (a.C == nullptr && a.C32 == nullptr)) return DWM_EINVAL;
    int rc = check_sizes(a, kBf16);
    if (rc != DWM_OK) return rc;
    if (a.lda % 8 != 0 || (a.C != nullptr && a.ldc % 8 != 0)) return DWM_EALIGN;
    if (!dwm_aligned16(a.A) || !dwm_aligned16(a.W) || !dwm_aligned16(a.C)) return DWM_EALIGN;
    if (a.bias && (((uintptr_t)a.bias) & 7u)) return DWM_EALIGN;
    if (a.C != nullptr && a.ldc < gemm_nout(a)) return DWM_EINVAL;
    rc = check_epilogue(a, kBf16);
    if (rc != DWM_OK) return rc;
    if (a.C32 != nullptr && a.epilogue != DWM_EPI_RESID) return DWM_EUNSUPPORTED;

    GemmPlan plan;
    rc = plan_gemm(a, tile_asked, plan);
    if (rc != DWM_OK) return rc;
    hipStream_t s = (hipStream_t)stream;
    if (plan.family == GemmFamily::W4_FAST || plan.family == GemmFamily::W4_GENERAL) return dwm_gemm4w_launch(a, plan, s);
    ConvParams cp;
    fill_conv_params(a, plan, cp);
    switch (plan.family) {
        case GemmFamily::W8_SPLITK: return launch_splitk(a, cp, plan, s);
        case GemmFamily::W8_C32: return launch_c32(a, cp, plan, s);
        default: return launch_tile(a, cp, plan, s);
    }
}
```

opendwm_amd/csrc/gemm_bf16_4w.hip:

```cpp
#include <atomic>

#include "gemm_common.h"

namespace {

using namespace dwm_gemm;

typedef __attribute__((ext_vector_type(8))) __bf16 hbf16x8;
typedef __attribute__((ext_vector_type(4))) int i32x4;

constexpr int BM = 256, BN = 256, BK = 64;
constexpr int TILE = BM * BK * 2;
constexpr int AST = 3, WST = 2;
constexpr int W_BASE = AST * TILE;
constexpr int LDS_BYTES = (AST + WST) * TILE;
constexpr int NJ = TILE / (4 * 1024);

struct G4Params {
    int ntm, ntn, gm;
    FastDiv fd_rpg, fd_rpa;
    FastDiv fd_rmod;
    DevRowMap amap;
    int steps_per_tap;
    int64_t a_base_rows;
    uint32_t tap_off[27];
};

template <int EPI, bool RF32, int RS, bool GEN = false>
__global__ void __launch_bounds__(256, 1)
gemm4w_kernel(const dwm_gemm_args p, const G4Params gp) {
    static_assert(EPI == DWM_EPI_RESID || (!RF32 && RS == 0), "RF32 / RS belong to RESID");
    static_assert(EPI != DWM_EPI_RESID || RS == 2 || RS == 3 || RS == 6 || (GEN && !RF32 && RS == 18),
                  "RESID: residual / gate + residual / residual + blend / (general form) residual row per image");
    extern __shared__ __attribute__((aligned(16))) char smem[];
    const int tid = threadIdx.x, lane = tid & 63;
    const int wave = __builtin_amdgcn_readfirstlane(tid >> 6);
    const int wm = wave >> 1, wn = wave & 1;
    const int l15 = lane & 15, lg = lane >> 4;
    const int64_t M = p.M, N = p.N, K = p.K;
    uint32_t tapv = 0;
    if constexpr (GEN) tapv = gp.tap_off[lane < 27 ? lane : 0];

    const int ntm = gp.ntm, ntn = gp.ntn, gm = gp.gm;
    const int id = xcd_remap(blockIdx.x, ntm * ntn);
    const int per_group = gm * ntn;
    const int grp = id / per_group, in_grp = id - grp * per_group;
    const int first_m = grp * gm;
    const int gsize = ntm - first_m < gm ? ntm - first_m : gm;
    const int tn = in_grp / gsize, tm = first_m + in_grp % gsize;
    const int64_t m0 = (int64_t)tm * BM, n0 = (int64_t)tn * BN;

    const bf16_t* __restrict__ Ap = (const bf16_t*)p.A;
    const bf16_t* __restrict__ Wp = (const bf16_t*)p.W;
    auto make_rsrc = [](const void* ptr) {
        const uint64_t a = (uint64_t)ptr;
        i32x4 r;
        r[0] = __builtin_amdgcn_readfirstlane((int)(uint32_t)a);
        r[1] = __builtin_amdgcn_readfirstlane((int)(uint32_t)((a >> 32) & 0xffffu));
        r[2] = -1;
        r[3] = 0x00020000;
        return r;
    };
    const i32x4 rs_a = make_rsrc(GEN ? Ap + gp.a_base_rows * p.lda : Ap + m0 * p.lda), rs_w = make_rsrc(GEN ? Wp : Wp + n0 * K);
    const int row0 = wave * (NJ * 8) + (lane >> 3);
    const uint32_t ch0 = (uint32_t)((lane & 7) ^ ((row0 >> 1) & 7)) * 16u;
    const uint32_t voff_a = (uint32_t)row0 * (uint32_t)(p.lda * 2) + ch0, voff_w = (uint32_t)row0 * (uint32_t)(K * 2) + ch0;
    const uint32_t step_a = 8u * (uint32_t)(p.lda * 2), step_w = 8u * (uint32_t)(K * 2);
    uint32_t va[NJ], vw[NJ];
    if constexpr (GEN) {
#pragma unroll
        for (int j = 0; j < NJ; ++j) {
            const int row = row0 + j * 8;
            const uint32_t ch = (uint32_t)((lane & 7) ^ ((row >> 1) & 7)) * 16u;
            int64_t gmr = m0 + row; gmr = gmr < M ? gmr : M - 1;
            int64_t gnr = n0 + row; gnr = gnr < N ? gnr : N - 1;
            va[j] = (uint32_t)map_row(gp.amap, gmr) * (uint32_t)(p.lda * 2) + ch;
            vw[j] = (uint32_t)gnr * (uint32_t)(K * 2) + ch;
        }
        asm volatile("" : "+v"(tapv));
    }
    int walk_left = 0, walk_tap = 0;
    uint32_t walk_a = 0;
    auto walk_next = [&]() {
        if (--walk_left == 0) {
            ++walk_tap;
            walk_left = gp.steps_per_tap;
            walk_a = (uint32_t)__builtin_amdgcn_readlane((int)tapv, walk_tap);
        } else {
            walk_a += BK * 2;
        }
    };
    const uint32_t lds0 = (uint32_t)(uintptr_t)(const __attribute__((address_space(3))) char*)smem;
    auto bufld = [&](const i32x4& rs, uint32_t vo, uint32_t so) {
        asm volatile("buffer_load_dwordx4 %0, %1, %2 offen lds\n\ts_add_u32 m0, m0, 0x400" ::"v"(vo), "s"(rs), "s"(so) : "memory", "m0");
    };
    auto set_m0 = [&](uint32_t lds_off) { asm volatile("s_mov_b32 m0, %0\n\ts_nop 0" ::"s"(lds0 + lds_off) : "memory", "m0"); };
    auto stage_a = [&](int buf, int kt, int j, uint32_t wa) {
        if (j == 0) set_m0((uint32_t)(buf * TILE + wave * NJ * 1024));
        if constexpr (GEN) bufld(rs_a, va[j], wa);
        else bufld(rs_a, (j & 1) ? (voff_a ^ 64u) : voff_a, (uint32_t)kt * (BK * 2) + (uint32_t)j * step_a);
    };
    auto stage_w = [&](int buf, int kt, int j) {
        if (j == 0) set_m0((uint32_t)(W_BASE + buf * TILE + wave * NJ * 1024));
        if constexpr (GEN) bufld(rs_w, vw[j], (uint32_t)kt * (BK * 2));
        else bufld(rs_w, (j & 1) ? (voff_w ^ 64u) : voff_w, (uint32_t)kt * (BK * 2) + (uint32_t)j * step_w);
    };

    const int swz = (l15 >> 1) & 7;
    const int a_row = (wm * 128 + l15) * 128, w_row = (wn * 128 + l15) * 128;
    int coff[2];
#pragma unroll
    for (int kh = 0; kh < 2; ++kh) coff[kh] = ((4 * kh + lg) ^ swz) << 4;

    f32x4 acc[8][8];
#pragma unroll
    for (int i = 0; i < 8; ++i)
#pragma unroll
        for (int j = 0; j < 8; ++j) acc[i][j] = (f32x4){0.f, 0.f, 0.f, 0.f};

    const int nk = (int)(K / BK);
    hbf16x8 af[2][8], wf[2][8];
    if constexpr (GEN) {
        walk_left = gp.steps_per_tap;
        walk_a = gp.tap_off[0];
    }
#pragma unroll
    for (int j = 0; j < NJ; ++j) stage_a(0, 0, j, walk_a);
#pragma unroll
    for (int j = 0; j < NJ; ++j) stage_w(0, 0, j);
    if (nk > 1) {
        if constexpr (GEN) walk_next();
#pragma unroll
        for (int j = 0; j < NJ; ++j) stage_a(1, 1, j, walk_a);
#pragma unroll
        for (int j = 0; j < NJ; ++j) stage_w(1, 1, j);
    }
#pragma unroll
    for (int i = 0; i < 8; ++i)
#pragma unroll
        for (int j = 0; j < 8; ++j) asm volatile("" : "+a"(acc[i][j]));
    if (nk > 1) asm volatile("s_waitcnt vmcnt(%0)" ::"n"(2 * NJ) : "memory");
    else asm volatile("s_waitcnt vmcnt(0)" ::: "memory");
    __builtin_amdgcn_s_barrier();
    asm volatile("" ::: "memory");
#pragma unroll
    for (int f = 0; f < 8; ++f) {
        af[0][f] = *(const hbf16x8*)(smem + a_row + f * 2048 + coff[0]);
        wf[0][f] = *(const hbf16x8*)(smem + W_BASE + w_row + f * 2048 + coff[0]);
    }

    int sa = 0, kt = 0;
    auto k_step = [&](auto mode_tag) {
        constexpr int MODE = decltype(mode_tag)::value;
        const int sa1 = sa == AST - 1 ? 0 : sa + 1, sa2 = sa1 == AST - 1 ? 0 : sa1 + 1;
        const char* la = smem + sa * TILE;
        const char* lw = smem + W_BASE + (kt & 1) * TILE;
        const char* lan = smem + sa1 * TILE;
        const char* lwn = smem + W_BASE + ((kt + 1) & 1) * TILE;
        if constexpr (GEN && MODE == 0) walk_next();
        const uint32_t wa2 = walk_a;
#pragma unroll
        for (int kh = 0; kh < 2; ++kh) {
            if (kh == 1 && MODE != 2) {
                if constexpr (MODE == 0) asm volatile("s_waitcnt vmcnt(%0) lgkmcnt(0)" ::"n"(NJ) : "memory");
                else asm volatile("s_waitcnt vmcnt(0) lgkmcnt(0)" ::: "memory");
                __builtin_amdgcn_s_barrier();
                asm volatile("" ::: "memory");
            }
#pragma unroll
            for (int i = 0; i < 8; ++i) {
#pragma unroll
                for (int j = 0; j < 8; ++j) {
                    acc[i][j] = __builtin_amdgcn_mfma_f32_16x16x32_bf16(wf[kh][j], af[kh][i], acc[i][j], 0, 0, 0);
                    const int idx = i * 8 + j;
                    if (!(MODE == 2 && kh == 1)) {
                        const char* fa = kh == 0 ? la : lan;
                        const char* fw = kh == 0 ? lw : lwn;
                        const int khn = kh ^ 1;
                        if (idx >= 8 && idx < 24 && ((idx & 1) == 0)) {
                            const int f = (idx - 8) >> 1;
                            wf[khn][f] = *(const hbf16x8*)(fw + w_row + f * 2048 + coff[khn]);
                        }
                        if (idx >= 9 && idx < 25 && ((idx & 1) == 1)) {
                            const int f = (idx - 9) >> 1;
                            af[khn][f] = *(const hbf16x8*)(fa + a_row + f * 2048 + coff[khn]);
                        }
                    }
                    if (MODE == 0 && idx >= 28 && idx < 28 + 4 * NJ && ((idx - 28) & 3) == 0) {
                        const int r = (idx - 28) >> 2;
                        if (kh == 0) stage_a(sa2, kt + 2, r, wa2);
                        else stage_w(kt & 1, kt + 2, r);
                    }
                    __builtin_amdgcn_sched_barrier(0);
                }
            }
        }
        sa = sa1;
        ++kt;
    };
    while (kt + 2 < nk) k_step(std::integral_constant<int, 0>{});
    if (nk > 1) k_step(std::integral_constant<int, 1>{});
    k_step(std::integral_constant<int, 2>{});

    constexpr bool kGeglu = EPI == DWM_EPI_GEGLU, kResid = EPI == DWM_EPI_RESID;
    constexpr int OW = kGeglu ? 64 : 128;
    constexpr int ESZ = kResid ? 4 : 2;
    constexpr int RB = OW * ESZ;
    constexpr int NCH = RB / 16;
    constexpr int LPR = OW / 8;
    constexpr int RPS = 64 / LPR;
    constexpr int NST = 16 / RPS;
    const int64_t Nout = kGeglu ? (N >> 1) : N;
    const int64_t ocol0 = (kGeglu ? (n0 >> 1) + wn * 64 : n0 + wn * 128);
    float bv[8][4];
    float rw[8][4];
    bool do_norm[2] = {false, false};
    if constexpr (!kResid) {
        const bf16_t* __restrict__ bias = (const bf16_t*)p.bias;
#pragma unroll
        for (int j = 0; j < 8; ++j) {
            int64_t n = n0 + wn * 128 + j * 16 + lg * 4;
            if constexpr (GEN) n = n < N ? n : 0;
            if (bias != nullptr) unpack4(*(const uint2*)(bias + n), bv[j]);
            else { bv[j][0] = bv[j][1] = bv[j][2] = bv[j][3] = 0.f; }
        }
        if constexpr (EPI == DWM_EPI_RMSHEAD) {
#pragma unroll
            for (int s = 0; s < 2; ++s) do_norm[s] = n0 + wn * 128 + s * 64 < p.rms_ncols;
#pragma unroll
            for (int j = 0; j < 8; ++j) {
                int64_t n = n0 + wn * 128 + j * 16 + lg * 4;
                if constexpr (GEN) n = n < N ? n : 0;
                if (do_norm[j >> 2]) unpack4(*(const uint2*)((const bf16_t*)p.rms_w + n), rw[j]);
                else { rw[j][0] = rw[j][1] = rw[j][2] = rw[j][3] = 1.f; }
            }
        }
    }
    const int rrow = lane / LPR, rc8 = lane % LPR;
    const int64_t ocol_raw = ocol0 + rc8 * 8;
    const bool nok = !GEN || ocol_raw < Nout;
    const int64_t ocol = nok ? ocol_raw : 0;
    float b8[8] = {0.f, 0.f, 0.f, 0.f, 0.f, 0.f, 0.f, 0.f};
    if constexpr (kResid) {
        if (p.bias != nullptr) unpack8(*(const uint4*)((const bf16_t*)p.bias + ocol), b8);
    }
    constexpr bool f_gate = (RS & 1) != 0, f_blend = (RS & 4) != 0;
    constexpr bool f_rowdiv = (RS & 16) != 0;

    asm volatile("s_waitcnt vmcnt(0)" ::: "memory");
    __syncthreads();
    char* const scr = smem + wave * 8192;

    uint4 gA[NST], rA[NST], rB[NST], blA[NST], blB[NST];
    float alA[NST];
    auto issue_resid = [&](int i) {
        if constexpr (kResid) {
#pragma unroll
            for (int st = 0; st < NST; ++st) {
                uint32_t m = (uint32_t)(m0 + wm * 128 + i * 16 + st * RPS + rrow);
                if constexpr (GEN) m = m < (uint32_t)M ? m : (uint32_t)(M - 1);
                if constexpr (f_gate) gA[st] = *(const uint4*)((const bf16_t*)p.gate + ((uint64_t)fdiv(m, gp.fd_rpg) * (uint32_t)p.ld_gate + (uint32_t)ocol));
                if constexpr (RF32) {
                    const float* rp = (const float*)p.res + ((uint64_t)m * (uint32_t)p.ld_res + (uint32_t)ocol);
                    rA[st] = *(const uint4*)rp;
                    rB[st] = *(const uint4*)(rp + 4);
                    if constexpr (f_blend) {
                        const float* bp = (const float*)p.blend + ((uint64_t)m * (uint32_t)p.ld_blend + (uint32_t)ocol);
                        blA[st] = *(const uint4*)bp;
                        blB[st] = *(const uint4*)(bp + 4);
                    }
                } else {
                    rA[st] = *(const uint4*)((const bf16_t*)p.res + ((uint64_t)(f_rowdiv ? fdiv(m, gp.fd_rmod) : m) * (uint32_t)p.ld_res + (uint32_t)ocol));
                    if constexpr (f_blend) blA[st] = *(const uint4*)((const bf16_t*)p.blend + ((uint64_t)m * (uint32_t)p.ld_blend + (uint32_t)ocol));
                }
                if constexpr (f_blend) alA[st] = p.alpha[fdiv(m, gp.fd_rpa)];
            }
        }
    };
    issue_resid(0);

#pragma unroll
    for (int i = 0; i < 8; ++i) {
        if constexpr (kGeglu) {
#pragma unroll
            for (int s = 0; s < 2; ++s)
#pragma unroll
                for (int jj = 0; jj < 2; ++jj) {
                    const int jv = 4 * s + jj, jg = jv + 2;
                    float y[4];
#pragma unroll
                    for (int r = 0; r < 4; r += 2) {
                        const f32x2 hv = (f32x2){acc[i][jv][r], acc[i][jv][r + 1]} + (f32x2){bv[jv][r], bv[jv][r + 1]};
                        const f32x2 x = hv * gelu_erf2((f32x2){acc[i][jg][r], acc[i][jg][r + 1]} + (f32x2){bv[jg][r], bv[jg][r + 1]});
                        y[r] = x[0]; y[r + 1] = x[1];
                    }
                    const int b = 2 * s + jj;
                    *(uint2*)(scr + l15 * RB + (((2 * b + (lg >> 1)) ^ (l15 & (NCH - 1))) << 4) + (lg & 1) * 8) = pack4(y);
                }
        } else if constexpr (EPI == DWM_EPI_RMSHEAD) {
#pragma unroll
            for (int s = 0; s < 2; ++s) {
                float x[4][4];
                f32x2 ss2 = {0.f, 0.f};
#pragma unroll
                for (int jj = 0; jj < 4; ++jj)
#pragma unroll
                    for (int r = 0; r < 4; r += 2) {
                        const f32x2 v = (f32x2){acc[i][4 * s + jj][r], acc[i][4 * s + jj][r + 1]} + (f32x2){bv[4 * s + jj][r], bv[4 * s + jj][r + 1]};
                        x[jj][r] = v[0]; x[jj][r + 1] = v[1];
                        ss2 += v * v;
                    }
                float ss = ss2[0] + ss2[1];
                ss += __shfl_xor(ss, 16, 64);
                ss += __shfl_xor(ss, 32, 64);
                const float rinv = do_norm[s] ? rsqrtf(ss * (1.f / 64.f) + p.rms_eps) : 1.f;
#pragma unroll
                for (int jj = 0; jj < 4; ++jj) {
                    float y[4];
#pragma unroll
                    for (int r = 0; r < 4; ++r) y[r] = x[jj][r] * rinv * rw[4 * s + jj][r];
                    const int b = 4 * s + jj;
                    *(uint2*)(scr + l15 * RB + (((2 * b + (lg >> 1)) ^ (l15 & (NCH - 1))) << 4) + (lg & 1) * 8) = pack4(y);
                }
            }
        } else if constexpr (kResid) {
#pragma unroll
            for (int j = 0; j < 8; ++j)
                *(float4*)(scr + l15 * RB + (((4 * j + lg) ^ l15) << 4)) = make_float4(acc[i][j][0], acc[i][j][1], acc[i][j][2], acc[i][j][3]);
        } else {
#define DWM4_ACT_PASS(FN_)                                                                                         \
            _Pragma("unroll") for (int j = 0; j < 8; ++j) {                                                        \
                float y[4];                                                                                        \
                _Pragma("unroll") for (int r = 0; r < 4; r += 2) {                                                 \
                    const f32x2 x = FN_((f32x2){acc[i][j][r], acc[i][j][r + 1]} + (f32x2){bv[j][r], bv[j][r + 1]}); \
                    y[r] = x[0]; y[r + 1] = x[1];                                                                  \
                }                                                                                                  \
                *(uint2*)(scr + l15 * RB + (((2 * j + (lg >> 1)) ^ (l15 & (NCH - 1))) << 4) + (lg & 1) * 8) = pack4(y); \
            }
            if (p.act == DWM_ACT_GELU_TANH) { DWM4_ACT_PASS(gelu_tanh2) }
            else if (p.act == DWM_ACT_SILU) { DWM4_ACT_PASS(silu2) }
            else if (p.act == DWM_ACT_RELU) { DWM4_ACT_PASS(relu2) }
            else { DWM4_ACT_PASS() }
#undef DWM4_ACT_PASS
        }
#pragma unroll
        for (int st = 0; st < NST; ++st) {
            const int r = st * RPS + rrow;
            const int64_t m = m0 + wm * 128 + i * 16 + r;
            if constexpr (!kResid) {
                const uint4 o = *(const uint4*)(scr + r * RB + ((rc8 ^ (r & (NCH - 1))) << 4));
                if (!GEN || (m < M && nok)) *(uint4*)((bf16_t*)p.C + ((uint64_t)(uint32_t)m * (uint32_t)p.ldc + (uint32_t)ocol)) = o;
            } else {
                const float4 x0 = *(const float4*)(scr + r * RB + (((2 * rc8) ^ r) << 4));
                const float4 x1 = *(const float4*)(scr + r * RB + (((2 * rc8 + 1) ^ r) << 4));
                float v[8] = {x0.x, x0.y, x0.z, x0.w, x1.x, x1.y, x1.z, x1.w};
                float t[8];
#pragma unroll
                for (int c = 0; c < 8; ++c) v[c] += b8[c];
                if constexpr (f_gate) {
                    unpack8(gA[st], t);
#pragma unroll
                    for (int c = 0; c < 8; ++c) v[c] *= t[c];
                }
                if constexpr (RF32) {
                    const float4 ta = *reinterpret_cast<const float4*>(&rA[st]), tb = *reinterpret_cast<const float4*>(&rB[st]);
                    t[0] = ta.x; t[1] = ta.y; t[2] = ta.z; t[3] = ta.w; t[4] = tb.x; t[5] = tb.y; t[6] = tb.z; t[7] = tb.w;
                } else {
                    unpack8(rA[st], t);
                }
#pragma unroll
                for (int c = 0; c < 8; ++c) v[c] += t[c];
                if constexpr (f_blend) {
                    if constexpr (RF32) {
                        const float4 ta = *reinterpret_cast<const float4*>(&blA[st]), tb = *reinterpret_cast<const float4*>(&blB[st]);
                        t[0] = ta.x; t[1] = ta.y; t[2] = ta.z; t[3] = ta.w; t[4] = tb.x; t[5] = tb.y; t[6] = tb.z; t[7] = tb.w;
                    } else {
                        unpack8(blA[st], t);
                    }
                    const float al = alA[st];
#pragma unroll
                    for (int c = 0; c < 8; ++c) v[c] = al * t[c] + (1.f - al) * v[c];
                }
                if (!GEN || (m < M && nok)) {
                    if constexpr (RF32) {
                        float* o32 = (float*)p.C32 + ((uint64_t)(uint32_t)m * (uint32_t)p.ldc32 + (uint32_t)ocol);
                        *(float4*)o32 = make_float4(v[0], v[1], v[2], v[3]);
                        *(float4*)(o32 + 4) = make_float4(v[4], v[5], v[6], v[7]);
                    } else {
                        *(uint4*)((bf16_t*)p.C + ((uint64_t)(uint32_t)m * (uint32_t)p.ldc + (uint32_t)ocol)) = pack8(v);
                    }
                }
            }
        }
        if (i + 1 < 8) issue_resid(i + 1);
    }
}

std::atomic<int64_t> g_launches{0};
std::atomic<int64_t> g_launches_gen{0};

template <int EPI, bool RF32, int RS, bool GEN = false>
int launch4w(const dwm_gemm_args& a, const G4Params& gp, hipStream_t s) {
    const hipError_t e = dwm_allow_dynamic_lds<gemm4w_kernel<EPI, RF32, RS, GEN>>(LDS_BYTES);
    if (e != hipSuccess) return (int)e;
    hipLaunchKernelGGL((gemm4w_kernel<EPI, RF32, RS, GEN>), dim3((unsigned)(gp.ntm * gp.ntn)), dim3(256), LDS_BYTES, s, a, gp);
    g_launches.fetch_add(1, std::memory_order_relaxed);
    if (GEN) g_launches_gen.fetch_add(1, std::memory_order_relaxed);
    return dwm_launch_status();
}
template <int EPI, bool RF32, int RS>
int launch4w_form(const dwm_gemm_args& a, const G4Params& gp, bool gen, hipStream_t s) {
    return gen ? launch4w<EPI, RF32, RS, true>(a, gp, s) : launch4w<EPI, RF32, RS, false>(a, gp, s);
}

void tap_span(const dwm_gemm_args& a, int64_t& smin, int64_t& smax) {
    smin = smax = 0;
    for (int t = 0; t < a.ntaps; ++t) {
        smin = a.tap_shift[t] < smin ? a.tap_shift[t] : smin;
        smax = a.tap_shift[t] > smax ? a.tap_shift[t] : smax;
    }
}

void fill_g4(const dwm_gemm_args& a, const GemmPlan& plan, G4Params& gp) {
    gp.ntm = plan.ntm; gp.ntn = plan.ntn;
    gp.gm = plan.gm;
    gp.fd_rpg = make_fastdiv((uint32_t)(a.rows_per_gate > 0 ? a.rows_per_gate : 1));
    gp.fd_rpa = make_fastdiv((uint32_t)(a.rows_per_alpha > 0 ? a.rows_per_alpha : 1));
    gp.fd_rmod = make_fastdiv((uint32_t)(a.res_mod < 0 ? -a.res_mod : 1));
    const dwm_rowmap2d identity = {};
    make_dev_rowmap(a.a_map.rw > 0 ? a.a_map : identity, gp.amap);
    gp.steps_per_tap = (int)(a.K / BK);
    gp.a_base_rows = 0;
    for (int t = 0; t < 27; ++t) gp.tap_off[t] = 0;
    if (plan.family != GemmFamily::W4_GENERAL) return;
    gp.steps_per_tap = (int)(gemm_k_per_tap(a) / BK);
    int64_t smin, smax;
    tap_span(a, smin, smax);
    gp.a_base_rows = smin;
    for (int t = 0; t < a.ntaps; ++t) gp.tap_off[t] = (uint32_t)((a.tap_shift[t] - smin) * a.lda * 2);
}

}

bool dwm_gemm4w_covers(const dwm_gemm_args& a, bool fast_only, GemmPlan& plan) {
    const int64_t lim = 1ll << 31;
    if (a.c_map.rw > 0 || a.split_k > 1 || a.K < 2 * BK) return false;
    const bool row_div = a.epilogue == DWM_EPI_RESID && a.res_mod < 0;
    const bool gen = a.a_map.rw > 0 || a.ntaps > 0 || a.M % BM != 0 || a.N % BN != 0 || row_div;
    if (gen && fast_only) return false;
    if (a.ldc >= lim || a.ldc32 >= lim || a.ld_res >= lim || a.ld_blend >= lim || a.ld_gate >= lim) return false;
    const int ntm = (int)((a.M + BM - 1) / BM), ntn = (int)((a.N + BN - 1) / BN);
    if (auto_splitk(a, (int64_t)ntm * ntn)) return false;
    int rs = 0;
    if (a.epilogue == DWM_EPI_RESID) {
        if (a.res_mod > 0 || a.act != DWM_ACT_NONE || a.res == nullptr) return false;
        rs = (a.gate ? 1 : 0) | 2 | (a.blend ? 4 : 0) | (row_div ? 16 : 0);
        if (a.C32 != nullptr && (a.C != nullptr || row_div)) return false;
        if (rs != 2 && rs != 3 && rs != 6 && !(rs == 18 && a.C32 == nullptr)) return false;
    } else if (a.C32 != nullptr) {
        return false;
    }
    if (!gen) {
        if (a.lda * 2 * BM >= lim || a.K * 2 * BN >= lim || a.lda * 2 >= (1ll << 28)) return false;
    } else {
        if (a.M >= (1ll << 30) || a.res_mod < -(1ll << 30) || a.rows_per_gate > (1ll << 30) || a.rows_per_alpha > (1ll << 30)) return false;
        const int ntaps = gemm_ntaps(a);
        const int64_t kpt = gemm_k_per_tap(a);
        if (ntaps > 27 || kpt <= 0 || kpt % BK != 0 || kpt * ntaps != a.K || a.lda < kpt) return false;
        DevRowMap amap;
        if (!make_dev_rowmap(a.a_map, amap)) return false;
        int64_t smin, smax;
        tap_span(a, smin, smax);
        int64_t last = a.M - 1;
        if (a.a_map.rw > 0) {
            const dwm_rowmap2d& r = a.a_map;
            const int64_t q = last / r.rw, x = last % r.rw, img = q / r.rh, y = q % r.rh;
            last = img * r.ipitch + y * r.rpitch + x * (r.xstep > 0 ? r.xstep : 1) + r.origin;
        }
        if (last < 0 || (last + smax - smin + 1) * a.lda * 2 + a.K * 2 >= lim || a.N * a.K * 2 >= lim) return false;
    }
    plan.family = gen ? GemmFamily::W4_GENERAL : GemmFamily::W4_FAST;
    plan.epi = a.epilogue; plan.rs = rs;
    plan.fast = !gen; plan.rf32 = a.C32 != nullptr;
    plan.tc = 0;
    plan.ntm = ntm; plan.ntn = ntn;
    plan.grid = (unsigned)(ntm * ntn); plan.block = 256; plan.lds = LDS_BYTES;
    plan.ksplit = 1;
    plan.gm = raster_group_height(a.K);
    return true;
}

int dwm_gemm4w_launch(const dwm_gemm_args& a, const GemmPlan& plan, hipStream_t s) {
    G4Params gp;
    fill_g4(a, plan, gp);
    const bool gen = plan.family == GemmFamily::W4_GENERAL;
    switch (plan.epi) {
        case DWM_EPI_PLAIN: return launch4w_form<DWM_EPI_PLAIN, false, 0>(a, gp, gen, s);
        case DWM_EPI_GEGLU: return launch4w_form<DWM_EPI_GEGLU, false, 0>(a, gp, gen, s);
        case DWM_EPI_RMSHEAD: return launch4w_form<DWM_EPI_RMSHEAD, false, 0>(a, gp, gen, s);
        default: break;
    }
    if (plan.rf32) {
        if (plan.rs == 2) return launch4w_form<DWM_EPI_RESID, true, 2>(a, gp, gen, s);
        if (plan.rs == 3) return launch4w_form<DWM_EPI_RESID, true, 3>(a, gp, gen, s);
        return launch4w_form<DWM_EPI_RESID, true, 6>(a, gp, gen, s);
    }
    if (plan.rs == 2) return launch4w_form<DWM_EPI_RESID, false, 2>(a, gp, gen, s);
    if (plan.rs == 3) return launch4w_form<DWM_EPI_RESID, false, 3>(a, gp, gen, s);
    if (plan.rs == 6) return launch4w_form<DWM_EPI_RESID, false, 6>(a, gp, gen, s);
    return launch4w<DWM_EPI_RESID, false, 18, true>(a, gp, s);
}

extern "C" int64_t dwm_gemm4w_launches(void) { return g_launches.load(std::memory_order_relaxed); }
extern "C" int64_t dwm_gemm4w_launches_general(void) { return g_launches_gen.load(std::memory_order_relaxed); }
```

opendwm_amd/csrc/gemm_common.h:

```cpp
#pragma once
#include "common.h"
#include "dwm_hip.h"

namespace dwm_gemm {

struct DevRowMap {
    FastDiv rw, rh;
    int64_t rpitch, ipitch, origin;
    int enabled, xstep;
};
static inline bool make_dev_rowmap(const dwm_rowmap2d& r, DevRowMap& d) {
    d.enabled = r.rw > 0;
    d.xstep = r.xstep > 0 ? (int)r.xstep : 1;
    if (!d.enabled) { d.rw = make_fastdiv(1); d.rh = make_fastdiv(1); d.rpitch = d.ipitch = d.origin = 0; return true; }
    if (r.rh <= 0 || r.rw >= (1ll << 30) || r.rh >= (1ll << 30)) return false;
    d.rw = make_fastdiv((uint32_t)r.rw); d.rh = make_fastdiv((uint32_t)r.rh);
    d.rpitch = r.rpitch; d.ipitch = r.ipitch; d.origin = r.origin;
    return true;
}
DWM_DEVINL int64_t map_row(const DevRowMap& rm, int64_t m) {
    if (!rm.enabled) return m;
    const uint32_t q = fdiv((uint32_t)m, rm.rw), x = (uint32_t)m - q * rm.rw.d;
    const uint32_t i = fdiv(q, rm.rh), y = q - i * rm.rh.d;
    return (int64_t)i * rm.ipitch + (int64_t)y * rm.rpitch + (int64_t)x * rm.xstep + rm.origin;
}

enum class GemmFamily {
    W4_FAST,
    W4_GENERAL,
    W8_SPLITK,
    W8_256,
    W8_128,
    W8_C32
};
struct GemmPlan {
    GemmFamily family;
    int epi, rs;
    bool fast, rf32;
    int tc;
    int ntm, ntn;
    unsigned grid, block;
    int lds;
    int ksplit;
    int gm;
};

static inline int raster_group_height(int64_t K) { return K >= 4096 ? 4 : 8; }

static inline int64_t gemm_nout(const dwm_gemm_args& a) { return a.epilogue == DWM_EPI_GEGLU ? a.N / 2 : a.N; }
static inline int gemm_ntaps(const dwm_gemm_args& a) { return a.ntaps > 0 ? a.ntaps : 1; }
static inline int64_t gemm_k_per_tap(const dwm_gemm_args& a) { return a.ntaps > 0 ? a.k_per_tap : a.K; }

static inline bool splitk_pays(int64_t tiles, int64_t nk) { return tiles <= 128 && nk >= 16; }
static inline bool auto_splitk(const dwm_gemm_args& a, int64_t tiles) {
    return (a.epilogue == DWM_EPI_PLAIN || a.epilogue == DWM_EPI_RESID) && a.workspace != nullptr && a.split_k == 0 &&
           a.C32 == nullptr && splitk_pays(tiles, a.K / 64);
}
static inline int clamp_ksplit(int ksplit, int64_t nk, int max_ranges, int64_t range_bytes, int64_t avail) {
    if (ksplit > nk / 8) ksplit = (int)(nk / 8);
    if (ksplit > max_ranges) ksplit = max_ranges;
    if ((int64_t)ksplit * range_bytes > avail) ksplit = (int)(avail / range_bytes);
    return ksplit;
}

}

bool dwm_gemm4w_covers(const dwm_gemm_args& a, bool fast_only, dwm_gemm::GemmPlan& plan);
int dwm_gemm4w_launch(const dwm_gemm_args& a, const dwm_gemm::GemmPlan& plan, hipStream_t s);
```

opendwm_amd/ops.py:

```python
from __future__ import annotations

import contextlib
import ctypes as C
import functools
import os
import threading
from dataclasses import dataclass
from typing import Optional, Sequence

import torch

from . import _lib
from ._lib import (ACT_GELU_TANH, ACT_NONE, ACT_RELU, ACT_SILU, EPI_GEGLU, EPI_PLAIN, EPI_RESID,
                   EPI_RMSHEAD)

BIG = 1 << 30
bf16 = torch.bfloat16
f32 = torch.float32


def _stream() -> int:
    return torch.cuda.current_stream().cuda_stream


def _call(name: str, *args) -> None:
    _lib.check(getattr(_lib.load(), name)(*args, _stream()), name)


def _dt(t: torch.Tensor):
    return f32 if t.dtype == f32 else bf16


def _p(t: Optional[torch.Tensor]):
    return None if t is None else t.data_ptr()


def _chk2d(t: torch.Tensor, name: str, dtype=bf16):
    if not t.is_cuda:
        raise RuntimeError(f"{name}: expected a device tensor (the HIP path has no CPU fallback)")
    if t.dtype != dtype:
        raise RuntimeError(f"{name}: expected {dtype}, got {t.dtype}")
    if t.dim() != 2 or t.stride(1) != 1:
        raise RuntimeError(f"{name}: expected a 2-D tensor with contiguous rows, got {tuple(t.shape)} strides {t.stride()}")


def _chkvec(t: Optional[torch.Tensor], name: str, dtype=bf16):
    if t is None:
        return
    if not t.is_cuda or t.dtype != dtype or not t.is_contiguous():
        raise RuntimeError(f"{name}: expected a contiguous {dtype} device tensor")


@dataclass
class PaddedGrid:
    I: int
    h: int
    w: int

    @property
    def rows(self) -> int:
        return self.I * (self.h + 2) * (self.w + 2)

    @property
    def pixels(self) -> int:
        return self.I * self.h * self.w

    def fill(self, m: "_lib.RowMap2D") -> None:
        m.rw, m.rh = self.w, self.h
        m.rpitch, m.ipitch = self.w + 2, (self.h + 2) * (self.w + 2)
        m.origin = self.w + 2 + 1

    def tap_shifts(self):
        return [(dy - 1) * (self.w + 2) + (dx - 1) for dy in range(3) for dx in range(3)]

    def fill_stride2(self, m: "_lib.RowMap2D") -> None:
        m.rw, m.rh = self.w // 2, self.h // 2
        m.rpitch, m.ipitch = 2 * (self.w + 2), (self.h + 2) * (self.w + 2)
        m.origin = self.w + 2 + 1
        m.xstep = 2

    def tap_shifts_stride2(self):
        return [dy * (self.w + 2) + dx for dy in range(3) for dx in range(3)]

    def fill_stride2_sym(self, m: "_lib.RowMap2D") -> None:
        self.fill_stride2(m)
        m.origin = 0

    def interior_index(self) -> torch.Tensor:
        i = torch.arange(self.I)[:, None, None]
        y = torch.arange(self.h)[None, :, None]
        x = torch.arange(self.w)[None, None, :]
        return (i * (self.h + 2) * (self.w + 2) + (y + 1) * (self.w + 2) + x + 1).reshape(-1)


@dataclass
class TimeGrid:
    B: int
    T: int
    vn: int

    @property
    def rows(self) -> int:
        return self.B * (self.T + 2) * self.vn

    @property
    def pixels(self) -> int:
        return self.B * self.T * self.vn

    def fill(self, m: "_lib.RowMap2D") -> None:
        m.rw, m.rh = self.vn, self.T
        m.rpitch, m.ipitch = self.vn, (self.T + 2) * self.vn
        m.origin = self.vn

    def tap_shifts(self):
        return [-self.vn, 0, self.vn]


@dataclass
class Grid3D:
    T: int
    B: int
    h: int
    w: int

    @property
    def frame_rows(self) -> int:
        return self.B * (self.h + 2) * (self.w + 2)

    @property
    def rows(self) -> int:
        return (self.T + 2) * self.frame_rows

    @property
    def pixels(self) -> int:
        return self.T * self.B * self.h * self.w

    def fill(self, m: "_lib.RowMap2D") -> None:
        m.rw, m.rh = self.w, self.h
        m.rpitch, m.ipitch = self.w + 2, (self.h + 2) * (self.w + 2)
        m.origin = 2 * self.frame_rows + self.w + 2 + 1

    def tap_shifts(self):
        return [(dt - 2) * self.frame_rows + (dy - 1) * (self.w + 2) + (dx - 1)
                for dt in range(3) for dy in range(3) for dx in range(3)]


def _overlaps(a: torch.Tensor, b: torch.Tensor) -> bool:
    def span(t):
        lo = t.data_ptr()
        return lo, lo + ((t.shape[0] - 1) * t.stride(0) + t.shape[1]) * t.element_size() if t.numel() else lo
    (a0, a1), (b0, b1) = span(a), span(b)
    return a0 < b1 and b0 < a1


def _gemm_dims(a, w, dt, rows, epilogue, a_grid, conv3x3, stride2, conv_taps, c_grid, fp32_checks):
    _chk2d(a, "a", dt)
    _chk2d(w, "w", dt)
    if not w.is_contiguous():
        raise RuntimeError("w must be contiguous [N, K]")
    N, K = w.shape
    taps = 9 if conv3x3 else len(conv_taps) if conv_taps is not None else 1
    if fp32_checks and taps > 27:
        raise NotImplementedError("gemm (fp32): at most 27 taps (three groups of 9, each tap walked as three plane products)")
    if a_grid is not None:
        if a.shape[0] != a_grid.rows or a.shape[1] * taps != K or (fp32_checks and not a.is_contiguous()):
            raise RuntimeError(f"gemm: padded A {tuple(a.shape)} does not match grid / weight {tuple(w.shape)}")
        if stride2 and (not conv3x3 or a_grid.h % 2 or a_grid.w % 2):
            raise RuntimeError("gemm: stride2 needs conv3x3 on an even-sized grid")
        M = a_grid.pixels // 4 if stride2 else a_grid.pixels
    else:
        if fp32_checks and (conv3x3 or conv_taps is not None or stride2):
            raise RuntimeError("gemm: convolution taps need a_grid")
        M = a.shape[0] if rows is None else rows
        if a.shape[1] != K:
            raise RuntimeError(f"gemm: K mismatch {a.shape} x {w.shape}")
    if c_grid is not None and c_grid.pixels != M:
        raise RuntimeError("gemm: c_grid pixel count != M")
    return M, N, K, taps, N // 2 if epilogue == EPI_GEGLU else N, c_grid.rows if c_grid is not None else M


def _gemm_out(out, shape, dt, device, padded):
    if out is None:
        out = (torch.zeros if padded else torch.empty)(shape, dtype=dt, device=device)
    _chk2d(out, "out", dt)
    if out.shape != shape:
        raise RuntimeError(f"gemm: out shape {tuple(out.shape)} != {shape}")
    return out


def _gemm_operands(g, dt, stream_dt, gate, rows_per_gate, res, res_mod, blend, alpha, rows_per_alpha, rms_w, rms_ncols, rms_eps):
    if gate is not None:
        _chk2d(gate, "gate", dt)
        g.gate, g.ld_gate, g.rows_per_gate = gate.data_ptr(), gate.stride(0), rows_per_gate
    if res is not None:
        _chk2d(res, "res", stream_dt)
        g.res, g.ld_res, g.res_mod = res.data_ptr(), res.stride(0), res_mod
    if blend is not None:
        _chk2d(blend, "blend", stream_dt)
        _chkvec(alpha, "alpha", f32)
        g.blend, g.ld_blend, g.alpha, g.rows_per_alpha = blend.data_ptr(), blend.stride(0), alpha.data_ptr(), rows_per_alpha
    if rms_w is not None:
        _chkvec(rms_w, "rms_w", dt)
        g.rms_w, g.rms_ncols, g.rms_eps = rms_w.data_ptr(), rms_ncols, rms_eps


def _gemm_maps(g, a, a_grid, conv3x3, stride2, conv_taps, c_grid, res, blend):
    if a_grid is not None:
        if stride2:
            (a_grid.fill_stride2_sym if stride2 == "sym" else a_grid.fill_stride2)(g.a_map)
        else:
            a_grid.fill(g.a_map)
        shifts = conv_taps
        if conv3x3:
            shifts = a_grid.tap_shifts_stride2() if stride2 else a_grid.tap_shifts()
        if shifts is not None:
            g.ntaps, g.k_per_tap = len(shifts), a.shape[1]
            for t, sh in enumerate(shifts):
                g.tap_shift[t] = sh
    if c_grid is not None:
        c_grid.fill(g.c_map)
        for name, t in (("res", res), ("blend", blend)):
            if t is not None and t.shape[0] != c_grid.rows:
                raise RuntimeError(f"gemm: {name} must be a padded grid when c_grid is given")


def gemm(a: torch.Tensor, w: torch.Tensor, bias: Optional[torch.Tensor] = None, *,
         out: Optional[torch.Tensor] = None, epilogue: int = EPI_PLAIN, act: int = ACT_NONE,
         gate: Optional[torch.Tensor] = None, rows_per_gate: int = 1,
         res: Optional[torch.Tensor] = None, res_mod: int = 0,
         blend: Optional[torch.Tensor] = None, alpha: Optional[torch.Tensor] = None,
         rows_per_alpha: int = 1,
         rms_w: Optional[torch.Tensor] = None, rms_ncols: int = 0, rms_eps: float = 1e-6,
         a_grid=None, conv3x3: bool = False, stride2=False, conv_taps: Optional[list] = None,
         c_grid=None, out32: Optional[torch.Tensor] = None, mirror: bool = True, w_is_activation: bool = False,
         rows: Optional[int] = None, split_k: int = 0, tile: int = 0, _debug: int = 0) -> torch.Tensor:
    if a.dtype == f32:
        return _gemm_f32(a, w, bias, out, rows, epilogue, act, gate, rows_per_gate, res, res_mod, blend, alpha, rows_per_alpha, rms_w,
                         rms_ncols, rms_eps, a_grid, conv3x3, stride2, conv_taps, c_grid, not w_is_activation)
    M, N, K, _, nout, orow = _gemm_dims(a, w, bf16, rows, epilogue, a_grid, conv3x3, stride2, conv_taps, c_grid, False)
    if not mirror:
        if out32 is None or out is not None:
            raise RuntimeError("gemm: mirror=False needs out32 and no `out`")
    else:
        out = _gemm_out(out, (orow, nout), bf16, a.device, c_grid is not None)
        if _overlaps(a, out):
            raise RuntimeError("gemm: `out` overlaps the A operand (a tile's output would overwrite rows other tiles still read)")
    _chkvec(bias, "bias")
    g = _lib.GemmArgs()
    g.A, g.lda, g.W, g.bias = a.data_ptr(), a.stride(0), w.data_ptr(), _p(bias)
    if out is not None:
        g.C, g.ldc = out.data_ptr(), out.stride(0)
    g.M, g.N, g.K, g.epilogue, g.act = M, N, K, epilogue, act
    if out32 is not None:
        if epilogue != EPI_RESID or res_mod != 0:
            raise RuntimeError("gemm: out32 needs the RESID epilogue (res_mod = 0; `res`, if any, in fp32)")
        _chk2d(out32, "out32", f32)
        if out32.shape != (orow, nout):
            raise RuntimeError("gemm: out32 must have the shape of the output")
        if res is not None and res.shape != out32.shape:
            raise RuntimeError("gemm: the fp32 res must have the shape of the output")
        g.C32, g.ldc32 = out32.data_ptr(), out32.stride(0)
        split_k = 1
    _gemm_operands(g, bf16, f32 if out32 is not None else bf16, gate, rows_per_gate, res, res_mod, blend, alpha, rows_per_alpha,
                   rms_w, rms_ncols, rms_eps)
    _gemm_maps(g, a, a_grid, conv3x3, stride2, conv_taps, c_grid, res, blend)
    g.reserved = _debug
    g.split_k = split_k
    g.tile = _gemm_tile_request(tile)
    if split_k != 1 and epilogue in (EPI_PLAIN, EPI_RESID) and ((M + 255) // 256) * ((N + 255) // 256) <= 128 and K >= 1024:
        ws = _gemm_workspace(a.device)
        g.workspace, g.workspace_bytes = ws.data_ptr(), ws.numel() * 4
    _call("dwm_gemm_bf16", C.byref(g))
    return out if mirror else out32


_G4W = threading.local()
_G4W_ENV = os.environ.get("DWM_GEMM4W", "")


def block_permute(src: torch.Tensor, dst: torch.Tensor, dims, src_strides, block_elems: int) -> torch.Tensor:
    if not (src.is_cuda and dst.is_cuda and src.is_contiguous() and dst.is_contiguous() and src.dtype == dst.dtype):
        raise RuntimeError("block_permute: contiguous device tensors of one dtype expected")
    a = _lib.BlockPermuteArgs()
    a.src, a.dst = src.data_ptr(), dst.data_ptr()
    a.block_bytes = block_elems * src.element_size()
    n = 1
    for i in range(4):
        a.n[i], a.sstride[i] = dims[i], src_strides[i]
        n *= dims[i]
    if n * block_elems != src.numel() or dst.numel() != src.numel():
        raise RuntimeError("block_permute: dims x block size do not cover the tensors")
    _call("dwm_block_permute", C.byref(a))
    return dst


def head_exchange(src: torch.Tensor, dst: torch.Tensor, rows: int, S: int, R: int, Dr: int, merge: bool = False) -> torch.Tensor:
    wide, dense = (dst, src) if merge else (src, dst)
    if not (src.is_cuda and dst.is_cuda and src.dtype == dst.dtype and src.element_size() in (2, 4)):
        raise RuntimeError("head_exchange: device tensors of one 2- or 4-byte dtype expected")
    if min(rows, S, R, Dr) <= 0:
        raise RuntimeError("head_exchange: rows, S, R and Dr must be positive")
    if wide.dim() != 2 or wide.stride(1) != 1 or tuple(wide.shape) != (rows, S * R * Dr) or (rows > 1 and wide.stride(0) < S * R * Dr):
        raise RuntimeError(f"head_exchange: the row-major side must be [rows, S * R * Dr] = [{rows}, {S * R * Dr}] with contiguous rows, "
                           f"got {tuple(wide.shape)} strides {wide.stride()}")
    if not dense.is_contiguous() or dense.numel() != rows * S * R * Dr:
        raise RuntimeError("head_exchange: the dense side must be contiguous with rows * S * R * Dr elements")
    ld = wide.stride(0) if rows > 1 else max(wide.stride(0), S * R * Dr)
    _call("dwm_head_exchange", src.data_ptr(), dst.data_ptr(), rows, S, R, Dr, src.element_size(), ld, 1 if merge else 0)
    return dst


FIFO_CHUNK = 1024


class FifoSlide:

    def __init__(self, pairs, chunk: int = FIFO_CHUNK):
        pairs = list(pairs)
        if not pairs:
            raise RuntimeError("fifo_slide: an empty list")
        self.chunk, self.tensors, rows = chunk, pairs, []
        dev = pairs[0][0].device
        for buf, fresh, outer, T in pairs:
            if not (torch.is_tensor(buf) and torch.is_tensor(fresh) and buf.is_cuda and fresh.is_cuda):
                raise RuntimeError("fifo_slide: expected device tensors (the HIP path has no CPU fallback)")
            if buf.device != dev or fresh.device != dev or not buf.is_contiguous() or not fresh.is_contiguous():
                raise RuntimeError("fifo_slide: contiguous tensors on one device expected")
            convert = buf.dtype == bf16 and fresh.dtype == f32
            if fresh.dtype != buf.dtype and not convert:
                raise RuntimeError(f"fifo_slide: fresh is {fresh.dtype}, the buffer {buf.dtype} (only fp32 -> bf16 is converted)")
            if outer <= 0 or T <= 0 or buf.numel() == 0 or buf.numel() % (outer * T) != 0:
                raise RuntimeError(f"fifo_slide: a buffer of {buf.numel()} elements is not [outer = {outer}][T = {T}][inner]")
            inner = buf.numel() // (outer * T)
            inner_bytes = inner * buf.element_size()
            if inner_bytes % 2 != 0:
                raise RuntimeError(f"fifo_slide: rows of {inner_bytes} bytes (a multiple of 2 is needed)")
            if fresh.numel() == 0 or fresh.numel() % inner != 0 or outer % (fresh.numel() // inner) != 0:
                raise RuntimeError(f"fifo_slide: fresh has {fresh.numel()} elements: not a number of rows of {inner} that divides outer = {outer}")
            b0, f0 = buf.data_ptr(), fresh.data_ptr()
            if f0 < b0 + buf.numel() * buf.element_size() and b0 < f0 + fresh.numel() * fresh.element_size():
                raise RuntimeError("fifo_slide: fresh overlaps the buffer it is shifted into")
            a = b0 | f0 | inner_bytes
            piece = 16 if a % 16 == 0 else 4 if a % 4 == 0 else 2
            rows.append((b0, f0, outer, T, inner_bytes, fresh.numel() // inner, int(convert), outer * (inner_bytes // piece)))
        self.bytes_moved = sum((2 * r[3] - 1) * r[2] * r[4] for r in rows)
        self.host_items = (_lib.FifoItem * len(rows))(*[_lib.FifoItem(*r) for r in rows])
        self.items = torch.tensor(rows, dtype=torch.int64).to(dev)
        bi, bs = [], []
        for i, r in enumerate(rows):
            nb = (r[-1] + chunk - 1) // chunk
            bi.append(torch.full((nb,), i, dtype=torch.int32))
            bs.append(torch.arange(nb, dtype=torch.int64) * chunk)
        self.block_item, self.block_start = torch.cat(bi).to(dev), torch.cat(bs).to(dev)

    def run(self) -> None:
        _call("dwm_fifo_slide_multi", self.host_items, len(self.host_items), _p(self.items), _p(self.block_item), _p(self.block_start),
              self.block_item.numel(), self.chunk)


def fifo_slide(bufs: Sequence[torch.Tensor], freshes: Sequence[torch.Tensor]) -> None:
    if len(bufs) != len(freshes):
        raise RuntimeError("fifo_slide: one fresh tensor per buffer")
    for b in bufs:
        if not torch.is_tensor(b) or b.dim() < 2:
            raise RuntimeError("fifo_slide: buffers are tensors [outer, T, ...]")
    FifoSlide([(b, f, b.shape[0], b.shape[1]) for b, f in zip(bufs, freshes)]).run()


ATTN_Q_PRESCALED = 1 << 15
ATTN_STREAM = 1 << 12
ATTN_RES12 = 1 << 13

_ATTN_ENV_VARIANT = int(os.environ.get("DWM_ATTN_VARIANT", "0") or "0", 0) | \
    {"1": 1 << 12, "2": (1 << 12) | (1 << 13)}.get(os.environ.get("DWM_ATTN_RES4", "")[:1], 0)


def _gemm_tile_request(tile: int) -> int:
    if tile != 0:
        return tile
    env = _G4W_ENV[:1]
    on = getattr(_G4W, "on", False)
    if env == "0":
        return 0
    if env == "f":
        return 4 if on else 0
    if env not in ("", "0"):
        return 3
    return 3 if on else 0


def gemm_4wave_enabled() -> bool:
    return bool(getattr(_G4W, "on", False))


@contextlib.contextmanager
def gemm_4wave_scope(on: bool):
    prev = gemm_4wave_enabled()
    _G4W.on = bool(on)
    try:
        yield
    finally:
        _G4W.on = prev


_ORD = threading.local()


def ordered_reductions_enabled() -> bool:
    return bool(getattr(_ORD, "on", False))


@contextlib.contextmanager
def ordered_reductions(on: bool):
    prev = ordered_reductions_enabled()
    _ORD.on = bool(on)
    try:
        yield
    finally:
        _ORD.on = prev


def opens_ordered_scope(fn):
    @functools.wraps(fn)
    def wrapped(model, *args, **kwargs):
        with ordered_reductions(getattr(model, "ordered_reductions", False)):
            return fn(model, *args, **kwargs)
    return wrapped


def carries_ordered_scope(cls):
    fwd, bwd = cls.forward, cls.backward

    def forward(ctx, *args, **kwargs):
        ctx._ordered_reductions = ordered_reductions_enabled()
        return fwd(ctx, *args, **kwargs)

    def backward(ctx, *grads):
        with ordered_reductions(getattr(ctx, "_ordered_reductions", False)):
            return bwd(ctx, *grads)

    cls.forward, cls.backward = staticmethod(forward), staticmethod(backward)
    return cls


def carries_gemm_scope(cls):
    fwd, bwd = cls.forward, cls.backward

    def forward(ctx, *args, **kwargs):
        ctx._gemm_4wave = gemm_4wave_enabled()
        return fwd(ctx, *args, **kwargs)

    def backward(ctx, *grads):
        with gemm_4wave_scope(getattr(ctx, "_gemm_4wave", False)):
            return bwd(ctx, *grads)

    cls.forward, cls.backward = staticmethod(forward), staticmethod(backward)
    return carries_ordered_scope(cls)


_SPLIT_WEIGHTS: dict = {}
SPLIT_WEIGHT_CACHE_MAX = 2048


def split_weight(w: torch.Tensor, taps: int = 1, cache: bool = True) -> torch.Tensor:
    key = (w.data_ptr(), w._version, tuple(w.shape), taps)
    hit = _SPLIT_WEIGHTS.pop(key, None) if cache else None
    if hit is None:
        hi = w.to(bf16)
        lo = (w - hi.float()).to(bf16)
        if taps > 1:
            N, K = w.shape
            h3, l3 = hi.view(N, taps, K // taps), lo.view(N, taps, K // taps)
            ws = torch.stack([h3, l3, h3], 2)
            if taps > 9:
                ws = torch.cat([ws[:, t0:t0 + 9].reshape(-1) for t0 in range(0, taps, 9)]).view(N, 3 * K)
            else:
                ws = ws.reshape(N, 3 * K).contiguous()
        else:
            ws = torch.cat([hi, lo, hi], 1).contiguous()
        hit = (ws, w)
    if not cache:
        return hit[0]
    _SPLIT_WEIGHTS[key] = hit
    while len(_SPLIT_WEIGHTS) > SPLIT_WEIGHT_CACHE_MAX:
        _SPLIT_WEIGHTS.pop(next(iter(_SPLIT_WEIGHTS)))
    return hit[0]


def clear_split_weights() -> None:
    _SPLIT_WEIGHTS.clear()


def _gemm_f32(a, w, bias, out, rows, epilogue, act, gate, rows_per_gate, res, res_mod, blend, alpha, rows_per_alpha, rms_w, rms_ncols,
              rms_eps, a_grid, conv3x3, stride2, conv_taps, c_grid, cache_w):
    M, N, K, taps, nout, orow = _gemm_dims(a, w, f32, rows, epilogue, a_grid, conv3x3, stride2, conv_taps, c_grid, True)
    out = _gemm_out(out, (orow, nout), f32, a.device, c_grid is not None)
    _chkvec(bias, "bias", f32)
    ws = split_weight(w, taps, cache=cache_w)
    g = _lib.GemmArgs()
    g.A, g.lda, g.W, g.bias, g.C, g.ldc = a.data_ptr(), a.stride(0), ws.data_ptr(), _p(bias), out.data_ptr(), out.stride(0)
    g.M, g.N, g.K, g.epilogue, g.act = M, N, K, epilogue, act
    _gemm_operands(g, f32, f32, gate, rows_per_gate, res, res_mod, blend, alpha, rows_per_alpha, rms_w, rms_ncols, rms_eps)
    _gemm_maps(g, a, a_grid, conv3x3, stride2, conv_taps, c_grid, res, blend)
    a_rows = a_grid.rows if a_grid is not None else M
    groups = (taps + 8) // 9
    need = 4 * a_rows * (K // taps) + 256 + 4 * M * N * groups
    tiles = ((M + 255) // 256) * ((N + 255) // 256)
    if tiles * groups <= 128:
        need += 4 * M * N * min(32, 256 // tiles)
    wsb = _f32_workspace(a.device, need)
    g.workspace, g.workspace_bytes = wsb.data_ptr(), wsb.numel() * 4
    _call("dwm_gemm_f32", C.byref(g))
    return out


_WORKSPACES: dict = {}
_F32_WORKSPACES: dict = {}
GEMM_WORKSPACE_BYTES = 1 << 30


def _workspace(cache: dict, device: torch.device, nbytes: int, slack: int = 0) -> torch.Tensor:
    key = (device.index, torch.cuda.current_stream(device).cuda_stream)
    ws = cache.get(key)
    if ws is None or ws.numel() * 4 < nbytes:
        ws = cache[key] = torch.empty((nbytes + slack) // 4, dtype=f32, device=device)
    return ws


def _f32_workspace(device: torch.device, nbytes: int) -> torch.Tensor:
    return _workspace(_F32_WORKSPACES, device, nbytes, 64 << 20)


def _gemm_workspace(device: torch.device) -> torch.Tensor:
    return _workspace(_WORKSPACES, device, GEMM_WORKSPACE_BYTES)


@dataclass
class RowMap:
    L0: int
    n_problems: int
    pdiv: Sequence[int] = (1, 1, 1)
    pmod: Sequence[int] = (BIG, 1, 1)
    pstride: Sequence[int] = (0, 0, 0)
    ldiv: Sequence[int] = (BIG, BIG)
    lstride: Sequence[int] = (1, 0, 0)
    p_per_mask: int = 1
    group_size: int = 1

    def rows(self) -> torch.Tensor:
        p = torch.arange(self.n_problems)[:, None]
        l = torch.arange(self.L0)[None, :]
        r = torch.zeros(self.n_problems, self.L0, dtype=torch.int64)
        for d, m, s in zip(self.pdiv, self.pmod, self.pstride):
            r = r + ((p // d) % m) * s
        r = r + (l % self.ldiv[0]) * self.lstride[0] + ((l // self.ldiv[0]) % self.ldiv[1]) * self.lstride[1] \
            + (l // (self.ldiv[0] * self.ldiv[1])) * self.lstride[2]
        return r


def rowmap_identity(n_problems: int, L0: int) -> RowMap:
    return RowMap(L0=L0, n_problems=n_problems, pstride=(L0, 0, 0))


def rowmap_crossview_rowwise(B: int, T: int, V: int, h: int, w: int) -> RowMap:
    return RowMap(L0=V * w, n_problems=B * T * h,
                  pdiv=(h, 1, 1), pmod=(BIG, h, 1), pstride=(V * h * w, w, 0),
                  ldiv=(w, BIG), lstride=(1, h * w, 0), p_per_mask=T * h, group_size=w)


def rowmap_crossview_full(B: int, T: int, V: int, h: int, w: int) -> RowMap:
    return RowMap(L0=h * V * w, n_problems=B * T,
                  pstride=(V * h * w, 0, 0),
# ... 668 lines not shown
```

Measured before the change: 2.553 denoise-steps/s.

## Pair image and context GEMMs of joint blocks into one two-segment launch

Adds a two-segment GEMM mode in which rows below seg_rows use W/bias/gate/res, and the remaining rows use a second weight set, gate and residual. In the joint blocks this fuses the image and context QKV projections, the attention out-projections and the FF2 residual GEMMs into single launches over a shared A buffer. A paired 4-wave kernel variant (W4_PAIR) handles both segments in one grid when a pair plan exists; otherwise the two segments still run as back-to-back launches. The aim is to cut launch count and fill the GPU better on the small context segment. The cost is more kernel template complexity and row buffers padded to multiples of 256. FF1 pairing is left off.

```diff
diff --git a/include/dwm_hip.h b/include/dwm_hip.h
--- a/include/dwm_hip.h
+++ b/include/dwm_hip.h
@@ -52,6 +52,12 @@
     void* workspace; int64_t workspace_bytes; int32_t split_k;
     void* C32; int64_t ldc32;
     int32_t tile;
+    int64_t seg_rows, a_rows;
+    const void* W1; const void* bias1; const void* rms_w1;
+    const void* gate1; int64_t ld_gate1; int64_t rows_per_gate1;
+    const void* res1; int64_t ld_res1;
+    void* C1; int64_t ldc1;
+    void* C32_1; int64_t ldc32_1;
 } dwm_gemm_args;
 
 int dwm_gemm_bf16(const dwm_gemm_args* args, void* stream);
diff --git a/opendwm_amd/_lib.py b/opendwm_amd/_lib.py
--- a/opendwm_amd/_lib.py
+++ b/opendwm_amd/_lib.py
@@ -38,6 +38,9 @@
         ("workspace", _vp), ("workspace_bytes", _i64), ("split_k", _i32),
         ("C32", _vp), ("ldc32", _i64),
         ("tile", _i32),
+        ("seg_rows", _i64), ("a_rows", _i64), ("W1", _vp), ("bias1", _vp), ("rms_w1", _vp),
+        ("gate1", _vp), ("ld_gate1", _i64), ("rows_per_gate1", _i64), ("res1", _vp), ("ld_res1", _i64),
+        ("C1", _vp), ("ldc1", _i64), ("C32_1", _vp), ("ldc32_1", _i64),
     ]
 
 
diff --git a/opendwm_amd/blocks.py b/opendwm_amd/blocks.py
--- a/opendwm_amd/blocks.py
+++ b/opendwm_amd/blocks.py
@@ -100,6 +100,25 @@
     return ops.gemm(a, w, b, epilogue=EPI_RESID, res=stream, out=stream, **kw)
 
 
+PAIR_GEMMS = True
+PAIR_FF1 = False
+
+
+def _pair_rows(rows: int, cols: int, dtype: torch.dtype, device) -> torch.Tensor:
+    return torch.empty((rows + 255) // 256 * 256, cols, dtype=dtype, device=device)[:rows]
+
+
+def _resid_pair_into(s0: torch.Tensor, s1: torch.Tensor, a: torch.Tensor, w0, b0, w1, b1, gate0, rows_per_gate0: int, gate1,
+                     rows_per_gate1: int) -> None:
+    on32 = stream32(s0)
+    seg = ops.GemmSegment(s0.shape[0], w1, b1, gate=gate1, rows_per_gate=rows_per_gate1, res=s1,
+                          out32=s1 if on32 else None, out=None if on32 else s1)
+    if on32:
+        ops.gemm(a, w0, b0, epilogue=EPI_RESID, res=s0, out32=s0, mirror=False, gate=gate0, rows_per_gate=rows_per_gate0, seg1=seg)
+    else:
+        ops.gemm(a, w0, b0, epilogue=EPI_RESID, res=s0, out=s0, gate=gate0, rows_per_gate=rows_per_gate0, seg1=seg)
+
+
 def geglu_pack(w: torch.Tensor) -> torch.Tensor:
     n2 = w.shape[0] // 2
     if n2 % 32 != 0:
@@ -225,15 +244,17 @@
     def attn_variant(self) -> int:
         return ops.ATTN_Q_PRESCALED if (self.has_qk_norm and PRESCALE_Q) else 0
 
-    def project_qkv(self, x: torch.Tensor, added: bool = False, out: Optional[torch.Tensor] = None) -> torch.Tensor:
+    def project_qkv(self, x: torch.Tensor, added: bool = False, out: Optional[torch.Tensor] = None,
+                    rows0: Optional[int] = None) -> torch.Tensor:
         pk = self.packed()
         ps = "_ps" if self.attn_variant else ""
         w, b, rms = (pk["wadd"], pk["badd"], pk.get("rms_add" + ps)) if added else (pk["wqkv"], pk["bqkv"], pk.get("rms" + ps))
+        seg = None if rows0 is None else ops.GemmSegment(rows0, pk["wadd"], pk["badd"], rms_w=pk.get("rms_add" + ps))
         if rms is None:
-            return ops.gemm(x, w, b, out=out)
+            return ops.gemm(x, w, b, out=out, seg1=seg)
         if self.dim_head != 64:
             raise RuntimeError("qk RMSNorm is implemented for head_dim 64 only")
-        return ops.gemm(x, w, b, epilogue=EPI_RMSHEAD, rms_w=rms, rms_ncols=rms.numel(), rms_eps=self.eps, out=out)
+        return ops.gemm(x, w, b, epilogue=EPI_RMSHEAD, rms_w=rms, rms_ncols=rms.numel(), rms_eps=self.eps, out=out, seg1=seg)
 
 
 class JointTransformerBlock(nn.Module):
@@ -266,40 +287,65 @@
             cmod = ops.gemm(silu_temb, _bf(self.norm1_context.linear.weight), _bf(self.norm1_context.linear.bias))
         sl = lambda m, i: m[:, i * D:(i + 1) * D]
         nh2 = _act_like(h) if self.use_dual_attention else None
-        nh = ops.layernorm(h, eps=1e-6, scale=sl(mod, 1), shift=sl(mod, 0), rows_per_mod=N,
-                           scale2=sl(mod, 7) if nh2 is not None else None,
-                           shift2=sl(mod, 6) if nh2 is not None else None, out2=nh2, x32=x32)
+        rows_h, rows_c = h.shape[0], c.shape[0]
+        rows = rows_h + rows_c
+        pair = PAIR_GEMMS
+        adt = bf16 if stream32(h) else h.dtype
+        nhc = _pair_rows(rows, D, adt, h.device)
+        nh, nc = nhc[:rows_h], nhc[rows_h:]
+        ops.layernorm(h, eps=1e-6, scale=sl(mod, 1), shift=sl(mod, 0), rows_per_mod=N, out=nh,
+                      scale2=sl(mod, 7) if nh2 is not None else None,
+                      shift2=sl(mod, 6) if nh2 is not None else None, out2=nh2, x32=x32)
         if self.context_pre_only:
-            nc = ops.layernorm(c, eps=1e-6, scale=sl(cmod, 0), shift=sl(cmod, 1), rows_per_mod=Lc, x32=x32)
-        else:
-            nc = ops.layernorm(c, eps=1e-6, scale=sl(cmod, 1), shift=sl(cmod, 0), rows_per_mod=Lc, x32=x32)
-
-        rows_h, rows_c = nh.shape[0], nc.shape[0]
-        both = torch.empty(rows_h + rows_c, 3 * D, dtype=nh.dtype, device=nh.device)
-        qkv = self.attn.project_qkv(nh, out=both[:rows_h])
-        cqkv = self.attn.project_qkv(nc, added=True, out=both[rows_h:])
-        ao_both = torch.empty(rows_h + rows_c, D, dtype=nh.dtype, device=nh.device)
+            ops.layernorm(c, eps=1e-6, scale=sl(cmod, 0), shift=sl(cmod, 1), rows_per_mod=Lc, out=nc, x32=x32)
+        else:
+            ops.layernorm(c, eps=1e-6, scale=sl(cmod, 1), shift=sl(cmod, 0), rows_per_mod=Lc, out=nc, x32=x32)
+
+        both = torch.empty(rows, 3 * D, dtype=nh.dtype, device=nh.device)
+        qkv, cqkv = both[:rows_h], both[rows_h:]
+        if pair:
+            self.attn.project_qkv(nhc, out=both, rows0=rows_h)
+        else:
+            self.attn.project_qkv(nh, out=qkv)
+            self.attn.project_qkv(nc, added=True, out=cqkv)
+        ao_both = _pair_rows(rows, D, adt, h.device)
         ao, cao = ao_both[:rows_h], ao_both[rows_h:]
         ops.attention(qkv[:, :D], qkv[:, D:2 * D], qkv[:, 2 * D:], ao, ops.rowmap_identity(n_img, N), self.heads,
                       q1=cqkv[:, :D], k1=cqkv[:, D:2 * D], v1=cqkv[:, 2 * D:], out1=cao, variant=self.attn.attn_variant | ATTN_VARIANT)
-        to_out = self.attn.to_out[0]
-        _resid_into(h, ao, _bf(to_out.weight), _bf(to_out.bias), gate=sl(mod, 2), rows_per_gate=N)
+        pair = pair and not self.context_pre_only
+        to_out, ta = self.attn.to_out[0], None if self.context_pre_only else self.attn.to_add_out
+        if pair:
+            _resid_pair_into(h, c, ao_both, _bf(to_out.weight), _bf(to_out.bias), _bf(ta.weight), _bf(ta.bias),
+                             sl(mod, 2), N, sl(cmod, 2), Lc)
+        else:
+            _resid_into(h, ao, _bf(to_out.weight), _bf(to_out.bias), gate=sl(mod, 2), rows_per_gate=N)
         if self.use_dual_attention:
             qkv2 = self.attn2.project_qkv(nh2)
             ops.attention(qkv2[:, :D], qkv2[:, D:2 * D], qkv2[:, 2 * D:], ao, ops.rowmap_identity(n_img, N), self.heads,
                           variant=self.attn2.attn_variant | ATTN_VARIANT)
             to_out2 = self.attn2.to_out[0]
             _resid_into(h, ao, _bf(to_out2.weight), _bf(to_out2.bias), gate=sl(mod, 8), rows_per_gate=N)
-        nh = ops.layernorm(h, eps=1e-6, scale=sl(mod, 4), shift=sl(mod, 3), rows_per_mod=N, out=nh, x32=x32)
+        ops.layernorm(h, eps=1e-6, scale=sl(mod, 4), shift=sl(mod, 3), rows_per_mod=N, out=nh, x32=x32)
         f1, f2 = self.ff.net[0].proj, self.ff.net[2]
+        if pair:
+            ops.layernorm(c, eps=1e-6, scale=sl(cmod, 4), shift=sl(cmod, 3), rows_per_mod=Lc, out=nc, x32=x32)
+            c1, c2 = self.ff_context.net[0].proj, self.ff_context.net[2]
+            ff_both = _pair_rows(rows, f1.weight.shape[0], adt, h.device)
+            if PAIR_FF1:
+                ops.gemm(nhc, _bf(f1.weight), _bf(f1.bias), act=ACT_GELU_TANH, out=ff_both,
+                         seg1=ops.GemmSegment(rows_h, _bf(c1.weight), _bf(c1.bias)))
+            else:
+                ops.gemm(nh, _bf(f1.weight), _bf(f1.bias), act=ACT_GELU_TANH, out=ff_both[:rows_h])
+                ops.gemm(nc, _bf(c1.weight), _bf(c1.bias), act=ACT_GELU_TANH, out=ff_both[rows_h:])
+            _resid_pair_into(h, c, ff_both, _bf(f2.weight), _bf(f2.bias), _bf(c2.weight), _bf(c2.bias), sl(mod, 5), N, sl(cmod, 5), Lc)
+            return c, h
         ffh = ops.gemm(nh, _bf(f1.weight), _bf(f1.bias), act=ACT_GELU_TANH)
         _resid_into(h, ffh, _bf(f2.weight), _bf(f2.bias), gate=sl(mod, 5), rows_per_gate=N)
 
         if self.context_pre_only:
             return None, h
-        ta = self.attn.to_add_out
         _resid_into(c, cao, _bf(ta.weight), _bf(ta.bias), gate=sl(cmod, 2), rows_per_gate=Lc)
-        nc = ops.layernorm(c, eps=1e-6, scale=sl(cmod, 4), shift=sl(cmod, 3), rows_per_mod=Lc, out=nc, x32=x32)
+        ops.layernorm(c, eps=1e-6, scale=sl(cmod, 4), shift=sl(cmod, 3), rows_per_mod=Lc, out=nc, x32=x32)
         c1, c2 = self.ff_context.net[0].proj, self.ff_context.net[2]
         cff = ops.gemm(nc, _bf(c1.weight), _bf(c1.bias), act=ACT_GELU_TANH)
         _resid_into(c, cff, _bf(c2.weight), _bf(c2.bias), gate=sl(cmod, 5), rows_per_gate=Lc)
diff --git a/opendwm_amd/build.py b/opendwm_amd/build.py
--- a/opendwm_amd/build.py
+++ b/opendwm_amd/build.py
@@ -45,7 +45,7 @@
 def build(force: bool = False, verbose: bool = False) -> str:
     hipcc = _hipcc()
     headers = [os.path.join(CSRC, "common.h"), os.path.join(CSRC, "attention_common.h"), os.path.join(CSRC, "gemm_common.h"),
-               os.path.join(INCLUDE, "dwm_hip.h")]
+               os.path.join(CSRC, "gemm_bf16_4w_passes.h"), os.path.join(INCLUDE, "dwm_hip.h")]
     shash = source_hash()
     stamp = os.path.join(CSRC, "build", ".source_hash")
     objdir = os.path.join(CSRC, "build")
diff --git a/opendwm_amd/csrc/gemm_bf16.hip b/opendwm_amd/csrc/gemm_bf16.hip
--- a/opendwm_amd/csrc/gemm_bf16.hip
+++ b/opendwm_amd/csrc/gemm_bf16.hip
@@ -932,6 +932,7 @@
 
 extern "C" int dwm_gemm_f32(const dwm_gemm_args* a, void* stream) {
     if (a == nullptr || a->A == nullptr || a->W == nullptr || a->C == nullptr || a->workspace == nullptr) return DWM_EINVAL;
+    if (a->seg_rows != 0) return DWM_EUNSUPPORTED;
     int rc = check_sizes(*a, kFp32);
     if (rc != DWM_OK) return rc;
     rc = check_taps(*a, kFp32);
@@ -1047,12 +1048,13 @@
 
 }
 
-extern "C" int dwm_gemm_bf16(const dwm_gemm_args* a_in, void* stream) {
-    if (a_in == nullptr) return DWM_EINVAL;
+namespace {
+
+int prepare_gemm(const dwm_gemm_args* a_in, dwm_gemm_args& a_copy, const dwm_gemm_args*& ap, GemmPlan& plan) {
     const int tile_asked = a_in->tile;
-    dwm_gemm_args a_copy;
     if (tile_asked == 3 || tile_asked == 4) { a_copy = *a_in; a_copy.tile = 0; }
     const dwm_gemm_args& a = tile_asked == 3 || tile_asked == 4 ? a_copy : *a_in;
+    ap = &a;
 
     if (a.A == nullptr || a.W == nullptr || (a.C == nullptr && a.C32 == nullptr)) return DWM_EINVAL;
     int rc = check_sizes(a, kBf16);
@@ -1065,11 +1067,12 @@
     if (rc != DWM_OK) return rc;
     if (a.C32 != nullptr && a.epilogue != DWM_EPI_RESID) return DWM_EUNSUPPORTED;
 
-    GemmPlan plan;
-    rc = plan_gemm(a, tile_asked, plan);
-    if (rc != DWM_OK) return rc;
-    hipStream_t s = (hipStream_t)stream;
-    if (plan.family == GemmFamily::W4_FAST || plan.family == GemmFamily::W4_GENERAL) return dwm_gemm4w_launch(a, plan, s);
+    return plan_gemm(a, tile_asked, plan);
+}
+
+int launch_gemm(const dwm_gemm_args& a, const GemmPlan& plan, hipStream_t s) {
+    if (plan.family == GemmFamily::W4_FAST || plan.family == GemmFamily::W4_GENERAL || plan.family == GemmFamily::W4_PAIR)
+        return dwm_gemm4w_launch(a, plan, s);
     ConvParams cp;
     fill_conv_params(a, plan, cp);
     switch (plan.family) {
@@ -1078,3 +1081,67 @@
         default: return launch_tile(a, cp, plan, s);
     }
 }
+
+void clear_segments(dwm_gemm_args& a) {
+    a.seg_rows = a.a_rows = 0;
+    a.W1 = a.bias1 = a.rms_w1 = a.gate1 = a.res1 = nullptr;
+    a.C1 = a.C32_1 = nullptr;
+    a.ld_gate1 = a.rows_per_gate1 = a.ld_res1 = a.ldc1 = a.ldc32_1 = 0;
+}
+
+int gemm_two_segments(const dwm_gemm_args& a, hipStream_t s) {
+    if (a.seg_rows < 0 || a.seg_rows >= a.M || a.W1 == nullptr || (a.a_rows != 0 && a.a_rows < a.M)) return DWM_EINVAL;
+    if (a.A == nullptr || a.lda <= 0) return DWM_EINVAL;
+    const int64_t r0 = a.seg_rows, stream_bytes = a.C32 != nullptr ? 4 : 2;
+    auto rows_on = [](const void* p, int64_t rows, int64_t ld, int64_t esz) { return p == nullptr ? nullptr : (const char*)p + rows * ld * esz; };
+    dwm_gemm_args s0 = a, s1 = a;
+    clear_segments(s0);
+    clear_segments(s1);
+    s0.M = r0;
+    s1.M = a.M - r0;
+    s1.A = rows_on(a.A, r0, a.lda, 2);
+    s1.W = a.W1; s1.bias = a.bias1; s1.rms_w = a.rms_w1;
+    s1.gate = a.gate1; s1.ld_gate = a.ld_gate1; s1.rows_per_gate = a.rows_per_gate1;
+    if (a.res1 != nullptr) { s1.res = a.res1; s1.ld_res = a.ld_res1; }
+    else s1.res = rows_on(a.res, r0, a.ld_res, stream_bytes);
+    if (a.C1 != nullptr) { s1.C = a.C1; s1.ldc = a.ldc1; }
+    else s1.C = (void*)rows_on(a.C, r0, a.ldc, 2);
+    if (a.C32_1 != nullptr) { s1.C32 = a.C32_1; s1.ldc32 = a.ldc32_1; }
+    else s1.C32 = (void*)rows_on(a.C32, r0, a.ldc32, 4);
+    if (a.blend != nullptr) {
+        s1.blend = rows_on(a.blend, r0, a.ld_blend, stream_bytes);
+        if (a.alpha != nullptr && a.rows_per_alpha > 0) s1.alpha = a.alpha + r0 / a.rows_per_alpha;
+    }
+    dwm_gemm_args c0, c1;
+    const dwm_gemm_args *p0, *p1;
+    GemmPlan plan0, plan1;
+    int rc = prepare_gemm(&s0, c0, p0, plan0);
+    if (rc == DWM_OK) rc = prepare_gemm(&s1, c1, p1, plan1);
+    if (rc != DWM_OK) return rc;
+
+    GemmPlan pair;
+    if ((a.tile == 3 || a.tile == 4) && !DWM_RESERVED(a.reserved) && a.lda % 64 == 0 && dwm_gemm4w_pair_plan(a, *p0, *p1, pair)) {
+        dwm_gemm_args both = *p0;
+        both.M = a.M; both.seg_rows = r0; both.a_rows = a.a_rows;
+        both.W1 = p1->W; both.bias1 = p1->bias; both.rms_w1 = p1->rms_w;
+        both.gate1 = p1->gate; both.ld_gate1 = p1->ld_gate; both.rows_per_gate1 = p1->rows_per_gate;
+        both.res1 = p1->res; both.ld_res1 = p1->ld_res;
+        both.C1 = p1->C; both.ldc1 = p1->ldc;
+        both.C32_1 = p1->C32; both.ldc32_1 = p1->ldc32;
+        return launch_gemm(both, pair, s);
+    }
+    rc = launch_gemm(*p0, plan0, s);
+    return rc != DWM_OK ? rc : launch_gemm(*p1, plan1, s);
+}
+
+}
+
+extern "C" int dwm_gemm_bf16(const dwm_gemm_args* a_in, void* stream) {
+    if (a_in == nullptr) return DWM_EINVAL;
+    if (a_in->seg_rows != 0) return gemm_two_segments(*a_in, (hipStream_t)stream);
+    dwm_gemm_args a_copy;
+    const dwm_gemm_args* a;
+    GemmPlan plan;
+    const int rc = prepare_gemm(a_in, a_copy, a, plan);
+    return rc != DWM_OK ? rc : launch_gemm(*a, plan, (hipStream_t)stream);
+}
diff --git a/opendwm_amd/csrc/gemm_bf16_4w.hip b/opendwm_amd/csrc/gemm_bf16_4w.hip
--- a/opendwm_amd/csrc/gemm_bf16_4w.hip
+++ b/opendwm_amd/csrc/gemm_bf16_4w.hip
@@ -24,12 +24,14 @@
     int steps_per_tap;
     int64_t a_base_rows;
     uint32_t tap_off[27];
+    FastDiv fd_rpg1;
 };
 
-template <int EPI, bool RF32, int RS, bool GEN = false>
+template <int EPI, bool RF32, int RS, bool GEN = false, bool PAIR = false>
 __global__ void __launch_bounds__(256, 1)
 gemm4w_kernel(const dwm_gemm_args p, const G4Params gp) {
     static_assert(EPI == DWM_EPI_RESID || (!RF32 && RS == 0), "RF32 / RS belong to RESID");
+    static_assert(!PAIR || (!GEN && EPI != DWM_EPI_GEGLU && (EPI != DWM_EPI_RESID || RS == 2 || RS == 3)), "paired form: fast, PLAIN / RMSHEAD / RESID 2, 3");
     static_assert(EPI != DWM_EPI_RESID || RS == 2 || RS == 3 || RS == 6 || (GEN && !RF32 && RS == 18),
                   "RESID: residual / gate + residual / residual + blend / (general form) residual row per image");
     extern __shared__ __attribute__((aligned(16))) char smem[];
@@ -49,9 +51,12 @@
     const int gsize = ntm - first_m < gm ? ntm - first_m : gm;
     const int tn = in_grp / gsize, tm = first_m + in_grp % gsize;
     const int64_t m0 = (int64_t)tm * BM, n0 = (int64_t)tn * BN;
+    const bool seg1 = PAIR && m0 >= p.seg_rows;
+    const int64_t ml0 = seg1 ? m0 - p.seg_rows : m0;
+    const int64_t Mseg = PAIR ? (seg1 ? M - p.seg_rows : p.seg_rows) : M;
 
     const bf16_t* __restrict__ Ap = (const bf16_t*)p.A;
-    const bf16_t* __restrict__ Wp = (const bf16_t*)p.W;
+    const bf16_t* __restrict__ Wp = (const bf16_t*)(seg1 ? p.W1 : p.W);
     auto make_rsrc = [](const void* ptr) {
         const uint64_t a = (uint64_t)ptr;
         i32x4 r;
@@ -212,11 +217,12 @@
     constexpr int NST = 16 / RPS;
     const int64_t Nout = kGeglu ? (N >> 1) : N;
     const int64_t ocol0 = (kGeglu ? (n0 >> 1) + wn * 64 : n0 + wn * 128);
+#define DWM4_SEG(F0_, F1_) (seg1 ? (F1_) : (F0_))
     float bv[8][4];
     float rw[8][4];
     bool do_norm[2] = {false, false};
     if constexpr (!kResid) {
-        const bf16_t* __restrict__ bias = (const bf16_t*)p.bias;
+        const bf16_t* __restrict__ bias = (const bf16_t*)DWM4_SEG(p.bias, p.bias1);
 #pragma unroll
         for (int j = 0; j < 8; ++j) {
             int64_t n = n0 + wn * 128 + j * 16 + lg * 4;
@@ -231,7 +237,7 @@
             for (int j = 0; j < 8; ++j) {
                 int64_t n = n0 + wn * 128 + j * 16 + lg * 4;
                 if constexpr (GEN) n = n < N ? n : 0;
-                if (do_norm[j >> 2]) unpack4(*(const uint2*)((const bf16_t*)p.rms_w + n), rw[j]);
+                if (do_norm[j >> 2]) unpack4(*(const uint2*)((const bf16_t*)DWM4_SEG(p.rms_w, p.rms_w1) + n), rw[j]);
                 else { rw[j][0] = rw[j][1] = rw[j][2] = rw[j][3] = 1.f; }
             }
         }
@@ -242,7 +248,7 @@
     const int64_t ocol = nok ? ocol_raw : 0;
     float b8[8] = {0.f, 0.f, 0.f, 0.f, 0.f, 0.f, 0.f, 0.f};
     if constexpr (kResid) {
-        if (p.bias != nullptr) unpack8(*(const uint4*)((const bf16_t*)p.bias + ocol), b8);
+        if (DWM4_SEG(p.bias, p.bias1) != nullptr) unpack8(*(const uint4*)((const bf16_t*)DWM4_SEG(p.bias, p.bias1) + ocol), b8);
     }
     constexpr bool f_gate = (RS & 1) != 0, f_blend = (RS & 4) != 0;
     constexpr bool f_rowdiv = (RS & 16) != 0;
@@ -251,159 +257,32 @@
     __syncthreads();
     char* const scr = smem + wave * 8192;
 
-    uint4 gA[NST], rA[NST], rB[NST], blA[NST], blB[NST];
-    float alA[NST];
-    auto issue_resid = [&](int i) {
-        if constexpr (kResid) {
-#pragma unroll
-            for (int st = 0; st < NST; ++st) {
-                uint32_t m = (uint32_t)(m0 + wm * 128 + i * 16 + st * RPS + rrow);
-                if constexpr (GEN) m = m < (uint32_t)M ? m : (uint32_t)(M - 1);
-                if constexpr (f_gate) gA[st] = *(const uint4*)((const bf16_t*)p.gate + ((uint64_t)fdiv(m, gp.fd_rpg) * (uint32_t)p.ld_gate + (uint32_t)ocol));
-                if constexpr (RF32) {
-                    const float* rp = (const float*)p.res + ((uint64_t)m * (uint32_t)p.ld_res + (uint32_t)ocol);
-                    rA[st] = *(const uint4*)rp;
-                    rB[st] = *(const uint4*)(rp + 4);
-                    if constexpr (f_blend) {
-                        const float* bp = (const float*)p.blend + ((uint64_t)m * (uint32_t)p.ld_blend + (uint32_t)ocol);
-                        blA[st] = *(const uint4*)bp;
-                        blB[st] = *(const uint4*)(bp + 4);
-                    }
-                } else {
-                    rA[st] = *(const uint4*)((const bf16_t*)p.res + ((uint64_t)(f_rowdiv ? fdiv(m, gp.fd_rmod) : m) * (uint32_t)p.ld_res + (uint32_t)ocol));
-                    if constexpr (f_blend) blA[st] = *(const uint4*)((const bf16_t*)p.blend + ((uint64_t)m * (uint32_t)p.ld_blend + (uint32_t)ocol));
-                }
-                if constexpr (f_blend) alA[st] = p.alpha[fdiv(m, gp.fd_rpa)];
-            }
-        }
-    };
-    issue_resid(0);
-
-#pragma unroll
-    for (int i = 0; i < 8; ++i) {
-        if constexpr (kGeglu) {
-#pragma unroll
-            for (int s = 0; s < 2; ++s)
-#pragma unroll
-                for (int jj = 0; jj < 2; ++jj) {
-                    const int jv = 4 * s + jj, jg = jv + 2;
-                    float y[4];
-#pragma unroll
-                    for (int r = 0; r < 4; r += 2) {
-                        const f32x2 hv = (f32x2){acc[i][jv][r], acc[i][jv][r + 1]} + (f32x2){bv[jv][r], bv[jv][r + 1]};
-                        const f32x2 x = hv * gelu_erf2((f32x2){acc[i][jg][r], acc[i][jg][r + 1]} + (f32x2){bv[jg][r], bv[jg][r + 1]});
-                        y[r] = x[0]; y[r + 1] = x[1];
-                    }
-                    const int b = 2 * s + jj;
-                    *(uint2*)(scr + l15 * RB + (((2 * b + (lg >> 1)) ^ (l15 & (NCH - 1))) << 4) + (lg & 1) * 8) = pack4(y);
-                }
-        } else if constexpr (EPI == DWM_EPI_RMSHEAD) {
-#pragma unroll
-            for (int s = 0; s < 2; ++s) {
-                float x[4][4];
-                f32x2 ss2 = {0.f, 0.f};
-#pragma unroll
-                for (int jj = 0; jj < 4; ++jj)
-#pragma unroll
-                    for (int r = 0; r < 4; r += 2) {
-                        const f32x2 v = (f32x2){acc[i][4 * s + jj][r], acc[i][4 * s + jj][r + 1]} + (f32x2){bv[4 * s + jj][r], bv[4 * s + jj][r + 1]};
-                        x[jj][r] = v[0]; x[jj][r + 1] = v[1];
-                        ss2 += v * v;
-                    }
-                float ss = ss2[0] + ss2[1];
-                ss += __shfl_xor(ss, 16, 64);
-                ss += __shfl_xor(ss, 32, 64);
-                const float rinv = do_norm[s] ? rsqrtf(ss * (1.f / 64.f) + p.rms_eps) : 1.f;
-#pragma unroll
-                for (int jj = 0; jj < 4; ++jj) {
-                    float y[4];
-#pragma unroll
-                    for (int r = 0; r < 4; ++r) y[r] = x[jj][r] * rinv * rw[4 * s + jj][r];
-                    const int b = 4 * s + jj;
-                    *(uint2*)(scr + l15 * RB + (((2 * b + (lg >> 1)) ^ (l15 & (NCH - 1))) << 4) + (lg & 1) * 8) = pack4(y);
-                }
-            }
-        } else if constexpr (kResid) {
-#pragma unroll
-            for (int j = 0; j < 8; ++j)
-                *(float4*)(scr + l15 * RB + (((4 * j + lg) ^ l15) << 4)) = make_float4(acc[i][j][0], acc[i][j][1], acc[i][j][2], acc[i][j][3]);
-        } else {
-#define DWM4_ACT_PASS(FN_)                                                                                         \
-            _Pragma("unroll") for (int j = 0; j < 8; ++j) {                                                        \
-                float y[4];                                                                                        \
-                _Pragma("unroll") for (int r = 0; r < 4; r += 2) {                                                 \
-                    const f32x2 x = FN_((f32x2){acc[i][j][r], acc[i][j][r + 1]} + (f32x2){bv[j][r], bv[j][r + 1]}); \
-                    y[r] = x[0]; y[r + 1] = x[1];                                                                  \
-                }                                                                                                  \
-                *(uint2*)(scr + l15 * RB + (((2 * j + (lg >> 1)) ^ (l15 & (NCH - 1))) << 4) + (lg & 1) * 8) = pack4(y); \
-            }
-            if (p.act == DWM_ACT_GELU_TANH) { DWM4_ACT_PASS(gelu_tanh2) }
-            else if (p.act == DWM_ACT_SILU) { DWM4_ACT_PASS(silu2) }
-            else if (p.act == DWM_ACT_RELU) { DWM4_ACT_PASS(relu2) }
-            else { DWM4_ACT_PASS() }
-#undef DWM4_ACT_PASS
-        }
-#pragma unroll
-        for (int st = 0; st < NST; ++st) {
-            const int r = st * RPS + rrow;
-            const int64_t m = m0 + wm * 128 + i * 16 + r;
-            if constexpr (!kResid) {
-                const uint4 o = *(const uint4*)(scr + r * RB + ((rc8 ^ (r & (NCH - 1))) << 4));
-                if (!GEN || (m < M && nok)) *(uint4*)((bf16_t*)p.C + ((uint64_t)(uint32_t)m * (uint32_t)p.ldc + (uint32_t)ocol)) = o;
-            } else {
-                const float4 x0 = *(const float4*)(scr + r * RB + (((2 * rc8) ^ r) << 4));
-                const float4 x1 = *(const float4*)(scr + r * RB + (((2 * rc8 + 1) ^ r) << 4));
-                float v[8] = {x0.x, x0.y, x0.z, x0.w, x1.x, x1.y, x1.z, x1.w};
-                float t[8];
-#pragma unroll
-                for (int c = 0; c < 8; ++c) v[c] += b8[c];
-                if constexpr (f_gate) {
-                    unpack8(gA[st], t);
-#pragma unroll
-                    for (int c = 0; c < 8; ++c) v[c] *= t[c];
-                }
-                if constexpr (RF32) {
-                    const float4 ta = *reinterpret_cast<const float4*>(&rA[st]), tb = *reinterpret_cast<const float4*>(&rB[st]);
-                    t[0] = ta.x; t[1] = ta.y; t[2] = ta.z; t[3] = ta.w; t[4] = tb.x; t[5] = tb.y; t[6] = tb.z; t[7] = tb.w;
-                } else {
-                    unpack8(rA[st], t);
-                }
-#pragma unroll
-                for (int c = 0; c < 8; ++c) v[c] += t[c];
-                if constexpr (f_blend) {
-                    if constexpr (RF32) {
-                        const float4 ta = *reinterpret_cast<const float4*>(&blA[st]), tb = *reinterpret_cast<const float4*>(&blB[st]);
-                        t[0] = ta.x; t[1] = ta.y; t[2] = ta.z; t[3] = ta.w; t[4] = tb.x; t[5] = tb.y; t[6] = tb.z; t[7] = tb.w;
-                    } else {
-                        unpack8(blA[st], t);
-                    }
-                    const float al = alA[st];
-#pragma unroll
-                    for (int c = 0; c < 8; ++c) v[c] = al * t[c] + (1.f - al) * v[c];
-                }
-                if (!GEN || (m < M && nok)) {
-                    if constexpr (RF32) {
-                        float* o32 = (float*)p.C32 + ((uint64_t)(uint32_t)m * (uint32_t)p.ldc32 + (uint32_t)ocol);
-                        *(float4*)o32 = make_float4(v[0], v[1], v[2], v[3]);
-                        *(float4*)(o32 + 4) = make_float4(v[4], v[5], v[6], v[7]);
-                    } else {
-                        *(uint4*)((bf16_t*)p.C + ((uint64_t)(uint32_t)m * (uint32_t)p.ldc + (uint32_t)ocol)) = pack8(v);
-                    }
-                }
-            }
-        }
-        if (i + 1 < 8) issue_resid(i + 1);
-    }
+#define DWM4_PASSES "gemm_bf16_4w_passes.h"
+    if constexpr (!PAIR) {
+#define DWM4_RAG GEN
+#include DWM4_PASSES
+#undef DWM4_RAG
+    } else if (ml0 + BM > Mseg) {
+#define DWM4_RAG true
+#include DWM4_PASSES
+#undef DWM4_RAG
+    } else {
+#define DWM4_RAG false
+#include DWM4_PASSES
+#undef DWM4_RAG
+    }
+#undef DWM4_PASSES
+#undef DWM4_SEG
 }
 
 std::atomic<int64_t> g_launches{0};
 std::atomic<int64_t> g_launches_gen{0};
 
-template <int EPI, bool RF32, int RS, bool GEN = false>
+template <int EPI, bool RF32, int RS, bool GEN = false, bool PAIR = false>
 int launch4w(const dwm_gemm_args& a, const G4Params& gp, hipStream_t s) {
-    const hipError_t e = dwm_allow_dynamic_lds<gemm4w_kernel<EPI, RF32, RS, GEN>>(LDS_BYTES);
+    const hipError_t e = dwm_allow_dynamic_lds<gemm4w_kernel<EPI, RF32, RS, GEN, PAIR>>(LDS_BYTES);
     if (e != hipSuccess) return (int)e;
-    hipLaunchKernelGGL((gemm4w_kernel<EPI, RF32, RS, GEN>), dim3((unsigned)(gp.ntm * gp.ntn)), dim3(256), LDS_BYTES, s, a, gp);
+    hipLaunchKernelGGL((gemm4w_kernel<EPI, RF32, RS, GEN, PAIR>), dim3((unsigned)(gp.ntm * gp.ntn)), dim3(256), LDS_BYTES, s, a, gp);
     g_launches.fetch_add(1, std::memory_order_relaxed);
     if (GEN) g_launches_gen.fetch_add(1, std::memory_order_relaxed);
     return dwm_launch_status();
@@ -420,6 +299,8 @@
         smax = a.tap_shift[t] > smax ? a.tap_shift[t] : smax;
     }
 }
+
+int launch4w_pair(const dwm_gemm_args& a, const GemmPlan& plan, const G4Params& gp, hipStream_t s);
 
 void fill_g4(const dwm_gemm_args& a, const GemmPlan& plan, G4Params& gp) {
     gp.ntm = plan.ntm; gp.ntn = plan.ntn;
@@ -427,6 +308,7 @@
     gp.fd_rpg = make_fastdiv((uint32_t)(a.rows_per_gate > 0 ? a.rows_per_gate : 1));
     gp.fd_rpa = make_fastdiv((uint32_t)(a.rows_per_alpha > 0 ? a.rows_per_alpha : 1));
     gp.fd_rmod = make_fastdiv((uint32_t)(a.res_mod < 0 ? -a.res_mod : 1));
+    gp.fd_rpg1 = make_fastdiv((uint32_t)(a.rows_per_gate1 > 0 ? a.rows_per_gate1 : 1));
     const dwm_rowmap2d identity = {};
     make_dev_rowmap(a.a_map.rw > 0 ? a.a_map : identity, gp.amap);
     gp.steps_per_tap = (int)(a.K / BK);
@@ -493,6 +375,7 @@
 int dwm_gemm4w_launch(const dwm_gemm_args& a, const GemmPlan& plan, hipStream_t s) {
     G4Params gp;
     fill_g4(a, plan, gp);
+    if (plan.family == GemmFamily::W4_PAIR) return launch4w_pair(a, plan, gp, s);
     const bool gen = plan.family == GemmFamily::W4_GENERAL;
     switch (plan.epi) {
         case DWM_EPI_PLAIN: return launch4w_form<DWM_EPI_PLAIN, false, 0>(a, gp, gen, s);
@@ -511,5 +394,29 @@
     return launch4w<DWM_EPI_RESID, false, 18, true>(a, gp, s);
 }
 
+namespace {
+int launch4w_pair(const dwm_gemm_args& a, const GemmPlan& plan, const G4Params& gp, hipStream_t s) {
+    if (plan.epi == DWM_EPI_PLAIN) return launch4w<DWM_EPI_PLAIN, false, 0, false, true>(a, gp, s);
+    if (plan.epi == DWM_EPI_RMSHEAD) return launch4w<DWM_EPI_RMSHEAD, false, 0, false, true>(a, gp, s);
+    if (plan.rf32) return plan.rs == 2 ? launch4w<DWM_EPI_RESID, true, 2, false, true>(a, gp, s) : launch4w<DWM_EPI_RESID, true, 3, false, true>(a, gp, s);
+    return plan.rs == 2 ? launch4w<DWM_EPI_RESID, false, 2, false, true>(a, gp, s) : launch4w<DWM_EPI_RESID, false, 3, false, true>(a, gp, s);
+}
+}
+
+bool dwm_gemm4w_pair_plan(const dwm_gemm_args& a, const dwm_gemm_args& s0, const dwm_gemm_args& s1, GemmPlan& plan) {
+    GemmPlan p1;
+    if (a.seg_rows % BM != 0 || a.N % BN != 0) return false;
+    if (!dwm_gemm4w_covers(s0, true, plan) || !dwm_gemm4w_covers(s1, false, p1)) return false;
+    if (s1.a_map.rw > 0 || s1.ntaps > 0 || s1.res_mod != 0) return false;
+    if (p1.epi != plan.epi || p1.rs != plan.rs || p1.rf32 != plan.rf32) return false;
+    if (plan.epi == DWM_EPI_GEGLU || (plan.epi == DWM_EPI_RESID && plan.rs != 2 && plan.rs != 3)) return false;
+    const int ntm = (int)((a.M + BM - 1) / BM);
+    if ((a.a_rows > 0 ? a.a_rows : a.M) < (int64_t)ntm * BM) return false;
+    plan.family = GemmFamily::W4_PAIR;
+    plan.ntm = ntm;
+    plan.grid = (unsigned)(ntm * plan.ntn);
+    return true;
+}
+
 extern "C" int64_t dwm_gemm4w_launches(void) { return g_launches.load(std::memory_order_relaxed); }
 extern "C" int64_t dwm_gemm4w_launches_general(void) { return g_launches_gen.load(std::memory_order_relaxed); }
diff --git a/opendwm_amd/csrc/gemm_bf16_4w_passes.h b/opendwm_amd/csrc/gemm_bf16_4w_passes.h
--- /dev/null
+++ b/opendwm_amd/csrc/gemm_bf16_4w_passes.h
@@ -0,0 +1,143 @@
+    uint4 gA[NST], rA[NST], rB[NST], blA[NST], blB[NST];
+    float alA[NST];
+    auto issue_resid = [&](int i) {
+        if constexpr (kResid) {
+#pragma unroll
+            for (int st = 0; st < NST; ++st) {
+                uint32_t m = (uint32_t)(ml0 + wm * 128 + i * 16 + st * RPS + rrow);
+                if constexpr (DWM4_RAG) m = m < (uint32_t)Mseg ? m : (uint32_t)(Mseg - 1);
+                if constexpr (f_gate) gA[st] = *(const uint4*)((const bf16_t*)DWM4_SEG(p.gate, p.gate1) + ((uint64_t)fdiv(m, DWM4_SEG(gp.fd_rpg, gp.fd_rpg1)) * (uint32_t)DWM4_SEG(p.ld_gate, p.ld_gate1) + (uint32_t)ocol));
+                if constexpr (RF32) {
+                    const float* rp = (const float*)DWM4_SEG(p.res, p.res1) + ((uint64_t)m * (uint32_t)DWM4_SEG(p.ld_res, p.ld_res1) + (uint32_t)ocol);
+                    rA[st] = *(const uint4*)rp;
+                    rB[st] = *(const uint4*)(rp + 4);
+                    if constexpr (f_blend) {
+                        const float* bp = (const float*)p.blend + ((uint64_t)m * (uint32_t)p.ld_blend + (uint32_t)ocol);
+                        blA[st] = *(const uint4*)bp;
+                        blB[st] = *(const uint4*)(bp + 4);
+                    }
+                } else {
+                    rA[st] = *(const uint4*)((const bf16_t*)DWM4_SEG(p.res, p.res1) + ((uint64_t)(f_rowdiv ? fdiv(m, gp.fd_rmod) : m) * (uint32_t)DWM4_SEG(p.ld_res, p.ld_res1) + (uint32_t)ocol));
+                    if constexpr (f_blend) blA[st] = *(const uint4*)((const bf16_t*)p.blend + ((uint64_t)m * (uint32_t)p.ld_blend + (uint32_t)ocol));
+                }
+                if constexpr (f_blend) alA[st] = p.alpha[fdiv(m, gp.fd_rpa)];
+            }
+        }
+    };
+    issue_resid(0);
+
+#pragma unroll
+    for (int i = 0; i < 8; ++i) {
+        if constexpr (kGeglu) {
+#pragma unroll
+            for (int s = 0; s < 2; ++s)
+#pragma unroll
+                for (int jj = 0; jj < 2; ++jj) {
+                    const int jv = 4 * s + jj, jg = jv + 2;
+                    float y[4];
+#pragma unroll
+                    for (int r = 0; r < 4; r += 2) {
+                        const f32x2 hv = (f32x2){acc[i][jv][r], acc[i][jv][r + 1]} + (f32x2){bv[jv][r], bv[jv][r + 1]};
+                        const f32x2 x = hv * gelu_erf2((f32x2){acc[i][jg][r], acc[i][jg][r + 1]} + (f32x2){bv[jg][r], bv[jg][r + 1]});
+                        y[r] = x[0]; y[r + 1] = x[1];
+                    }
+                    const int b = 2 * s + jj;
+                    *(uint2*)(scr + l15 * RB + (((2 * b + (lg >> 1)) ^ (l15 & (NCH - 1))) << 4) + (lg & 1) * 8) = pack4(y);
+                }
+        } else if constexpr (EPI == DWM_EPI_RMSHEAD) {
+#pragma unroll
+            for (int s = 0; s < 2; ++s) {
+                float x[4][4];
+                f32x2 ss2 = {0.f, 0.f};
+#pragma unroll
+                for (int jj = 0; jj < 4; ++jj)
+#pragma unroll
+                    for (int r = 0; r < 4; r += 2) {
+                        const f32x2 v = (f32x2){acc[i][4 * s + jj][r], acc[i][4 * s + jj][r + 1]} + (f32x2){bv[4 * s + jj][r], bv[4 * s + jj][r + 1]};
+                        x[jj][r] = v[0]; x[jj][r + 1] = v[1];
+                        ss2 += v * v;
+                    }
+                float ss = ss2[0] + ss2[1];
+                ss += __shfl_xor(ss, 16, 64);
+                ss += __shfl_xor(ss, 32, 64);
+                const float rinv = do_norm[s] ? rsqrtf(ss * (1.f / 64.f) + p.rms_eps) : 1.f;
+#pragma unroll
+                for (int jj = 0; jj < 4; ++jj) {
+                    float y[4];
+#pragma unroll
+                    for (int r = 0; r < 4; ++r) y[r] = x[jj][r] * rinv * rw[4 * s + jj][r];
+                    const int b = 4 * s + jj;
+                    *(uint2*)(scr + l15 * RB + (((2 * b + (lg >> 1)) ^ (l15 & (NCH - 1))) << 4) + (lg & 1) * 8) = pack4(y);
+                }
+            }
+        } else if constexpr (kResid) {
+#pragma unroll
+            for (int j = 0; j < 8; ++j)
+                *(float4*)(scr + l15 * RB + (((4 * j + lg) ^ l15) << 4)) = make_float4(acc[i][j][0], acc[i][j][1], acc[i][j][2], acc[i][j][3]);
+        } else {
+#define DWM4_ACT_PASS(FN_)                                                                                         \
+            _Pragma("unroll") for (int j = 0; j < 8; ++j) {                                                        \
+                float y[4];                                                                                        \
+                _Pragma("unroll") for (int r = 0; r < 4; r += 2) {                                                 \
+                    const f32x2 x = FN_((f32x2){acc[i][j][r], acc[i][j][r + 1]} + (f32x2){bv[j][r], bv[j][r + 1]}); \
+                    y[r] = x[0]; y[r + 1] = x[1];                                                                  \
+                }                                                                                                  \
+                *(uint2*)(scr + l15 * RB + (((2 * j + (lg >> 1)) ^ (l15 & (NCH - 1))) << 4) + (lg & 1) * 8) = pack4(y); \
+            }
+            if (p.act == DWM_ACT_GELU_TANH) { DWM4_ACT_PASS(gelu_tanh2) }
+            else if (p.act == DWM_ACT_SILU) { DWM4_ACT_PASS(silu2) }
+            else if (p.act == DWM_ACT_RELU) { DWM4_ACT_PASS(relu2) }
+            else { DWM4_ACT_PASS() }
+#undef DWM4_ACT_PASS
+        }
+#pragma unroll
+        for (int st = 0; st < NST; ++st) {
+            const int r = st * RPS + rrow;
+            const int64_t m = ml0 + wm * 128 + i * 16 + r;
+            if constexpr (!kResid) {
+                const uint4 o = *(const uint4*)(scr + r * RB + ((rc8 ^ (r & (NCH - 1))) << 4));
+                if (!(DWM4_RAG) || (m < Mseg && nok)) *(uint4*)((bf16_t*)DWM4_SEG(p.C, p.C1) + ((uint64_t)(uint32_t)m * (uint32_t)DWM4_SEG(p.ldc, p.ldc1) + (uint32_t)ocol)) = o;
+            } else {
+                const float4 x0 = *(const float4*)(scr + r * RB + (((2 * rc8) ^ r) << 4));
+                const float4 x1 = *(const float4*)(scr + r * RB + (((2 * rc8 + 1) ^ r) << 4));
+                float v[8] = {x0.x, x0.y, x0.z, x0.w, x1.x, x1.y, x1.z, x1.w};
+                float t[8];
+#pragma unroll
+                for (int c = 0; c < 8; ++c) v[c] += b8[c];
+                if constexpr (f_gate) {
+                    unpack8(gA[st], t);
+#pragma unroll
+                    for (int c = 0; c < 8; ++c) v[c] *= t[c];
+                }
+                if constexpr (RF32) {
+                    const float4 ta = *reinterpret_cast<const float4*>(&rA[st]), tb = *reinterpret_cast<const float4*>(&rB[st]);
+                    t[0] = ta.x; t[1] = ta.y; t[2] = ta.z; t[3] = ta.w; t[4] = tb.x; t[5] = tb.y; t[6] = tb.z; t[7] = tb.w;
+                } else {
+                    unpack8(rA[st], t);
+                }
+#pragma unroll
+                for (int c = 0; c < 8; ++c) v[c] += t[c];
+                if constexpr (f_blend) {
+                    if constexpr (RF32) {
+                        const float4 ta = *reinterpret_cast<const float4*>(&blA[st]), tb = *reinterpret_cast<const float4*>(&blB[st]);
+                        t[0] = ta.x; t[1] = ta.y; t[2] = ta.z; t[3] = ta.w; t[4] = tb.x; t[5] = tb.y; t[6] = tb.z; t[7] = tb.w;
+                    } else {
+                        unpack8(blA[st], t);
+                    }
+                    const float al = alA[st];
+#pragma unroll
+                    for (int c = 0; c < 8; ++c) v[c] = al * t[c] + (1.f - al) * v[c];
+                }
+                if (!(DWM4_RAG) || (m < Mseg && nok)) {
+                    if constexpr (RF32) {
+                        float* o32 = (float*)DWM4_SEG(p.C32, p.C32_1) + ((uint64_t)(uint32_t)m * (uint32_t)DWM4_SEG(p.ldc32, p.ldc32_1) + (uint32_t)ocol);
+                        *(float4*)o32 = make_float4(v[0], v[1], v[2], v[3]);
+                        *(float4*)(o32 + 4) = make_float4(v[4], v[5], v[6], v[7]);
+                    } else {
+                        *(uint4*)((bf16_t*)DWM4_SEG(p.C, p.C1) + ((uint64_t)(uint32_t)m * (uint32_t)DWM4_SEG(p.ldc, p.ldc1) + (uint32_t)ocol)) = pack8(v);
+                    }
+                }
+            }
+        }
+        if (i + 1 < 8) issue_resid(i + 1);
+    }
diff --git a/opendwm_amd/csrc/gemm_common.h b/opendwm_amd/csrc/gemm_common.h
--- a/opendwm_amd/csrc/gemm_common.h
+++ b/opendwm_amd/csrc/gemm_common.h
@@ -28,6 +28,7 @@
 enum class GemmFamily {
     W4_FAST,
     W4_GENERAL,
+    W4_PAIR,
     W8_SPLITK,
     W8_256,
     W8_128,
@@ -66,4 +67,5 @@
 }
 
 bool dwm_gemm4w_covers(const dwm_gemm_args& a, bool fast_only, dwm_gemm::GemmPlan& plan);
+bool dwm_gemm4w_pair_plan(const dwm_gemm_args& a, const dwm_gemm_args& s0, const dwm_gemm_args& s1, dwm_gemm::GemmPlan& plan);
 int dwm_gemm4w_launch(const dwm_gemm_args& a, const dwm_gemm::GemmPlan& plan, hipStream_t s);
diff --git a/opendwm_amd/ops.py b/opendwm_amd/ops.py
--- a/opendwm_amd/ops.py
+++ b/opendwm_amd/ops.py
@@ -224,6 +224,87 @@
                 raise RuntimeError(f"gemm: {name} must be a padded grid when c_grid is given")
 
 
+class GemmSegment:
+    __slots__ = ("rows0", "w", "bias", "rms_w", "gate", "rows_per_gate", "res", "out", "out32")
+
+    def __init__(self, rows0: int, w: torch.Tensor, bias: Optional[torch.Tensor] = None, *, rms_w: Optional[torch.Tensor] = None,
+                 gate: Optional[torch.Tensor] = None, rows_per_gate: int = 1, res: Optional[torch.Tensor] = None,
+                 out: Optional[torch.Tensor] = None, out32: Optional[torch.Tensor] = None):
+        self.rows0, self.w, self.bias, self.rms_w, self.gate, self.rows_per_gate = rows0, w, bias, rms_w, gate, rows_per_gate
+        self.res, self.out, self.out32 = res, out, out32
+
+    @property
+    def separate(self) -> bool:
+        return self.out is not None or self.out32 is not None
+
+
+def _rows_readable(a: torch.Tensor) -> int:
+    if a.shape[0] <= 1 or a.stride(0) <= 0:
+        return a.shape[0]
+    elems = a.untyped_storage().nbytes() // a.element_size() - a.storage_offset()
+    return max(a.shape[0], (elems - a.shape[1]) // a.stride(0) + 1)
+
+
+def _gemm_segment1(g, seg1, a, w, M, nout, dt, epilogue, out, out32, res, a_grid, c_grid, conv3x3, conv_taps, stride2, blend, res_mod, rows):
+    if a_grid is not None or c_grid is not None or conv3x3 or conv_taps is not None or stride2 or blend is not None or res_mod != 0 \
+            or rows is not None:
+        raise RuntimeError("gemm: seg1 goes with plain row-major operands (no grids, taps, blend, res_mod, rows)")
+    r0 = seg1.rows0
+    if not 0 < r0 < M:
+        raise RuntimeError(f"gemm: seg1.rows0 = {r0} must lie inside the {M} rows of a")
+    _chk2d(seg1.w, "seg1.w", dt)
+    if seg1.w.shape != w.shape or not seg1.w.is_contiguous():
+        raise RuntimeError("gemm: seg1.w must be contiguous and shaped like w")
+    _chkvec(seg1.bias, "seg1.bias")
+    g.seg_rows, g.a_rows, g.W1, g.bias1 = r0, _rows_readable(a), seg1.w.data_ptr(), _p(seg1.bias)
+    stream_dt = f32 if out32 is not None else dt
+    if (seg1.out32 is not None) != (seg1.separate and out32 is not None) or (seg1.out is not None) != (seg1.separate and out is not None):
+        raise RuntimeError("gemm: seg1.out / seg1.out32 must be given exactly where the call's out / out32 are, or both left out")
+    for name, t, tdt in (("seg1.out", seg1.out, dt), ("seg1.out32", seg1.out32, f32)):
+        if t is not None:
+            _chk2d(t, name, tdt)
+            if t.shape != (M - r0, nout):
+                raise RuntimeError(f"gemm: {name} must be [{M - r0}, {nout}]")
+    if seg1.out is not None:
+        if _overlaps(a, seg1.out):
+            raise RuntimeError("gemm: `seg1.out` overlaps the A operand")
+        g.C1, g.ldc1 = seg1.out.data_ptr(), seg1.out.stride(0)
+    if seg1.out32 is not None:
+        g.C32_1, g.ldc32_1 = seg1.out32.data_ptr(), seg1.out32.stride(0)
+    if (seg1.res is not None) != (seg1.separate and res is not None):
+        raise RuntimeError("gemm: seg1.res goes with separate outputs and a `res` of segment 0 (else `res` holds the rows of both)")
+    if seg1.res is not None:
+        _chk2d(seg1.res, "seg1.res", stream_dt)
+        if seg1.res.shape != (M - r0, nout):
+            raise RuntimeError(f"gemm: seg1.res must be [{M - r0}, {nout}]")
+        g.res1, g.ld_res1 = seg1.res.data_ptr(), seg1.res.stride(0)
+    if (seg1.gate is not None) != bool(g.gate) or (seg1.rms_w is not None) != bool(g.rms_w):
+        raise RuntimeError("gemm: seg1 takes a gate / rms_w exactly where segment 0 does")
+    if seg1.gate is not None:
+        _chk2d(seg1.gate, "seg1.gate", dt)
+        g.gate1, g.ld_gate1, g.rows_per_gate1 = seg1.gate.data_ptr(), seg1.gate.stride(0), seg1.rows_per_gate
+    if seg1.rms_w is not None:
+        _chkvec(seg1.rms_w, "seg1.rms_w", dt)
+        g.rms_w1 = seg1.rms_w.data_ptr()
+
+
+def _gemm_f32_segments(a, w, bias, out, seg1, res, gate, kw):
+    r0, M = seg1.rows0, a.shape[0]
+    if not 0 < r0 < M:
+        raise RuntimeError(f"gemm: seg1.rows0 = {r0} must lie inside the {M} rows of a")
+    if seg1.separate:
+        o0, o1, r1 = out, seg1.out, seg1.res
+    else:
+        if out is None:
+            out = torch.empty((M, w.shape[0]), dtype=f32, device=a.device)
+        o0, o1, r1 = out[:r0], out[r0:], None if res is None else res[r0:]
+        res = None if res is None else res[:r0]
+    o0 = gemm(a[:r0], w, bias, out=o0, res=res, gate=gate, **kw)
+    kw = dict(kw, rms_w=seg1.rms_w, rows_per_gate=seg1.rows_per_gate)
+    gemm(a[r0:], seg1.w, seg1.bias, out=o1, res=r1, gate=seg1.gate, **kw)
+    return o0 if seg1.separate else out
+
+
 def gemm(a: torch.Tensor, w: torch.Tensor, bias: Optional[torch.Tensor] = None, *,
          out: Optional[torch.Tensor] = None, epilogue: int = EPI_PLAIN, act: int = ACT_NONE,
          gate: Optional[torch.Tensor] = None, rows_per_gate: int = 1,
@@ -233,11 +314,21 @@
          rms_w: Optional[torch.Tensor] = None, rms_ncols: int = 0, rms_eps: float = 1e-6,
          a_grid=None, conv3x3: bool = False, stride2=False, conv_taps: Optional[list] = None,
          c_grid=None, out32: Optional[torch.Tensor] = None, mirror: bool = True, w_is_activation: bool = False,
-         rows: Optional[int] = None, split_k: int = 0, tile: int = 0, _debug: int = 0) -> torch.Tensor:
+         rows: Optional[int] = None, split_k: int = 0, tile: int = 0, _debug: int = 0,
+         seg1: Optional[GemmSegment] = None) -> torch.Tensor:
+    if a.dtype == f32 and seg1 is not None:
+        if a_grid is not None or c_grid is not None or conv3x3 or conv_taps is not None or stride2 or blend is not None or res_mod != 0 \
+                or rows is not None:
+            raise RuntimeError("gemm: seg1 goes with plain row-major operands (no grids, taps, blend, res_mod, rows)")
+        return _gemm_f32_segments(a, w, bias, out, seg1, res, gate,
+                                  dict(epilogue=epilogue, act=act, rows_per_gate=rows_per_gate, rms_w=rms_w, rms_ncols=rms_ncols,
+                                       rms_eps=rms_eps, w_is_activation=w_is_activation))
     if a.dtype == f32:
         return _gemm_f32(a, w, bias, out, rows, epilogue, act, gate, rows_per_gate, res, res_mod, blend, alpha, rows_per_alpha, rms_w,
                          rms_ncols, rms_eps, a_grid, conv3x3, stride2, conv_taps, c_grid, not w_is_activation)
     M, N, K, _, nout, orow = _gemm_dims(a, w, bf16, rows, epilogue, a_grid, conv3x3, stride2, conv_taps, c_grid, False)
+    if seg1 is not None and seg1.separate:
+        orow = seg1.rows0
     if not mirror:
         if out32 is None or out is not None:
             raise RuntimeError("gemm: mirror=False needs out32 and no `out`")
@@ -264,10 +355,15 @@
     _gemm_operands(g, bf16, f32 if out32 is not None else bf16, gate, rows_per_gate, res, res_mod, blend, alpha, rows_per_alpha,
                    rms_w, rms_ncols, rms_eps)
     _gemm_maps(g, a, a_grid, conv3x3, stride2, conv_taps, c_grid, res, blend)
+    if seg1 is not None:
+        _gemm_segment1(g, seg1, a, w, M, nout, bf16, epilogue, out, out32, res, a_grid, c_grid, conv3x3, conv_taps, stride2, blend, res_mod,
+                       rows)
     g.reserved = _debug
     g.split_k = split_k
     g.tile = _gemm_tile_request(tile)
-    if split_k != 1 and epilogue in (EPI_PLAIN, EPI_RESID) and ((M + 255) // 256) * ((N + 255) // 256) <= 128 and K >= 1024:
+    seg_rows = (M,) if seg1 is None else (seg1.rows0, M - seg1.rows0)
+    if split_k != 1 and epilogue in (EPI_PLAIN, EPI_RESID) and K >= 1024 and \
+            any(((r + 255) // 256) * ((N + 255) // 256) <= 128 for r in seg_rows):
         ws = _gemm_workspace(a.device)
         g.workspace, g.workspace_bytes = ws.data_ptr(), ws.numel() * 4
     _call("dwm_gemm_bf16", C.byref(g))
```

Measured after the change: 2.562 denoise-steps/s (median of 3 runs). No clear change (+0.4%).
